# fabian-sp/GGLasso

Hardware: AMD Instinct MI355X
Metric: ADMM iters/sec on (K=32,p=500) GGL at 1/2/4/8 GPUs; eigh HBM GB/s vs peak (higher is better)
Workload: dtype f64

## Files before the change

gglasso_amd/_lib.py:

```python
import ctypes
import os

import numpy as np

_HERE = os.path.dirname(os.path.abspath(__file__))
LIB_PATH = os.path.join(_HERE, "lib", "libggl_hip.so")
DEV_LIB_PATH = os.path.join(_HERE, "lib", "libggl_hip_dev.so")

REG_SGL, REG_GGL, REG_FGL, REG_FSGL = 0, 1, 2, 3
EIG_AUTO, EIG_JACOBI, EIG_ROCSOLVER, EIG_NEWTON_SCHULZ = 0, 1, 2, 3
CTX_STREAM_GIVEN = 1 << 16
OPTIONS = {"speculate": 1, "spec_factor": 2, "ns_mode": 3, "ns_degrees": 4, "theta_flat": 5, "rank_eig": 6, "parts": 7,
           "parts_max_tiles": 8, "symm_variant": 9, "spin_wait": 10, "fused_bounds": 11, "pipeline": 12, "fused_start": 13, "parts_small": 14, "ns_tol": 15, "cw_warm": 16, "chain": 17, "rank_l0_coarse": 18, "isolate": 19, "rank_deflate": 20, "rank_l0_deflate": 21, "fused_cw": 22, "omega_lds": 23, "early_part": 24, "part_priority": 25, "fused_w": 26, "rank_cw": 27, "bound_side": 28, "lds_pinned": 29, "join_flag": 30, "cw_rider": 31, "copy_rider": 32, "reduce_rider": 33, "parts_bias": 34, "parts_order": 35, "download_threads": 36, "group_sched": 37, "omega_poly": 38}


def eig_flags(method=EIG_AUTO, ns_mode=0, ns_degrees=0):
    return int(method) | ((int(ns_mode) & 0x3) << 8) | ((int(ns_degrees) & 0xf) << 12)

JACOBI_MAX_P = 128
NS_MIN_P = 8
BUF_S, BUF_OMEGA, BUF_THETA, BUF_L, BUF_X, BUF_GROUPSQ, BUF_NORMS, BUF_OMEGA_PREV = range(8)
E_ARG, E_HIP, E_SOLVER, E_ALLOC, E_COMM = -1, -2, -3, -4, -5
PHASES = ("form_W", "eig_omega", "recon_omega", "theta", "eig_L", "recon_L", "dual", "reduce", "eig_omega2", "bound",
          "allreduce_groupsq", "allreduce_norms")

_dp = ctypes.POINTER(ctypes.c_double)
_vp = ctypes.c_void_p
_i = ctypes.c_int
_d = ctypes.c_double
_ubp = ctypes.POINTER(ctypes.c_ubyte)
_ip = ctypes.POINTER(ctypes.c_int)

_SIGNATURES = {
    "ggl_version": ([], _i),
    "ggl_last_error": ([], ctypes.c_char_p),
    "ggl_device_count": ([], _i),
    "ggl_theta_limits": ([ctypes.POINTER(_i)], _i),
    "ggl_ctx_create": ([_i, _i, _i, _i, _vp, ctypes.POINTER(_vp)], _i),
    "ggl_ctx_destroy": ([_vp], _i),
    "ggl_ctx_sync": ([_vp], _i),
    "ggl_device_ptr": ([_vp, _i], _vp),
    "ggl_ctx_set_option": ([_vp, _i, _d], _i),
    "ggl_ctx_get_option": ([_vp, _i, _dp], _i),
    "ggl_set_S": ([_vp, _dp], _i),
    "ggl_set_state": ([_vp, _dp, _dp, _dp, _dp], _i),
    "ggl_set_state_ex": ([_vp, _dp, _dp, _dp, _dp, ctypes.POINTER(_i)], _i),
    "ggl_set_S_ex": ([_vp, _dp, _i], _i),
    "ggl_get_state": ([_vp, _dp, _dp, _dp, _dp], _i),
    "ggl_state_snapshot": ([_vp, _i], _i),
    "ggl_set_lambda1_mask": ([_vp, _dp], _i),
    "ggl_set_lambda1_mask_k": ([_vp, _dp], _i),
    "ggl_set_instance_dims": ([_vp, ctypes.POINTER(_i)], _i),
    "ggl_set_block_size": ([_vp, _i], _i),
    "ggl_fsgl_stats": ([_vp, ctypes.POINTER(ctypes.c_longlong)], _i),
    "ggl_prox_sum_frob": ([_i, _i, _dp, _d, _dp], _i),
    "ggl_frob_norm_per_block": ([_i, _i, _dp, _i, _dp], _i),
    "ggl_admm_step": ([_vp, _d, _d, _d, _i, _i, _dp, _dp, _dp], _i),
    "ggl_hint_last_step": ([_vp], _i),
    "ggl_step_omega": ([_vp, _d, _i, _dp], _i),
    "ggl_step_omega_spec": ([_vp, _d, _i, _dp], _i),
    "ggl_step_group_partial": ([_vp, _d, _d], _i),
    "ggl_step_finish": ([_vp, _d, _d, _d, _i, _i, _dp, _i, _dp], _i),
    "ggl_norms_read": ([_vp, _dp], _i),
    "ggl_comm_unique_id": ([ctypes.c_char_p], _i),
    "ggl_comm_init": ([_vp, _i, _i, ctypes.c_char_p], _i),
    "ggl_comm_destroy": ([_vp], _i),
# ... 6 lines not shown
    "ggl_sgl_batch_step": ([_vp, _dp, _dp, _i, _dp, _dp], _i),
    "ggl_mgl_batch_step": ([_vp, _i, _dp, _dp, _dp, _i, _i, _dp, _dp, _dp], _i),
    "ggl_scale_X_batch": ([_vp, _dp], _i),
    "ggl_batch_decide": ([_i, _dp, _ubp, _ubp, _dp, _dp, _d, _d, _i, _dp, _dp, _ip], _i),
    "ggl_sgl_batch_run": ([_vp, _i, _dp, _dp, _i, _dp, _dp, _d, _d, _i, _dp, _ip, _ip, _i, _vp, _ip, _i], _i),
    "ggl_mgl_batch_run": ([_vp, _i, _i, _dp, _dp, _dp, _i, _i, _dp, _dp, _dp, _d, _d, _i, _dp, _ip, _ip, _i, _vp, _ip, _i], _i),
    "ggl_snapshot_state_from": ([_vp, _i, _vp, _i], _i),
    "ggl_get_snapshots": ([_vp, _dp, _dp, _dp, _dp], _i),
    "ggl_get_state_k": ([_vp, _i, _dp, _dp, _dp, _dp], _i),
    "ggl_exit_checks": ([_vp, _i, _dp], _i),
    "ggl_exit_checks_k": ([_vp, _i, _dp], _i),
    "ggl_exit_checks_fast_k": ([_vp, _i, _d, _d, _dp], _i),
    "ggl_ext_setup": ([_vp, ctypes.POINTER(_i), ctypes.POINTER(_i), _i], _i),
    "ggl_ext_set_state": ([_vp, _dp, _dp], _i),
    "ggl_ext_get_state": ([_vp, _dp, _dp], _i),
    "ggl_ext_admm_step": ([_vp, _d, _dp, _d, _i, _dp, _dp], _i),
    "ggl_ext_kkt_residual": ([_vp, _d, _dp, _d, _i, _dp, _dp], _i),
    "ggl_ext_setup_batch": ([_vp, _i, ctypes.POINTER(_i), ctypes.POINTER(_i), _i], _i),
    "ggl_ext_batch_step": ([_vp, _d, _dp, _dp, _i, _dp, _dp], _i),
    "ggl_objective": ([_vp, _d, _d, _i, _dp], _i),
    "ggl_kkt_residual": ([_vp, _d, _d, _d, _i, _i, _dp, _dp, _dp], _i),
    "ggl_profile_enable": ([_vp, _i], _i),
    "ggl_profile_read": ([_vp, _dp, ctypes.POINTER(ctypes.c_longlong), _i], _i),
    "ggl_dev_symm": ([_i, _i, _dp, _dp, _dp, _dp, _dp, _dp, _i], _i),
    "ggl_dev_symm_bench": ([_i, _i, _i, _i, _dp], _i),
    "ggl_lds_stats": ([_vp, ctypes.POINTER(ctypes.c_longlong)], _i),
    "ggl_group_stats": ([_vp, ctypes.POINTER(ctypes.c_longlong), _dp], _i),
    "ggl_spectral_bounds": ([_vp, _dp, _dp], _i),
    "ggl_pipeline_stats": ([_vp, ctypes.POINTER(ctypes.c_longlong)], _i),
    "ggl_trace_start": ([_vp, _i], _i),
    "ggl_trace_read": ([_vp, _dp, _i], _i),
    "ggl_dev_omega_lds": ([_i, _i, _dp, _dp, _dp, _dp, _dp, _d, _i, _dp, _dp, _i, _dp], _i),
    "ggl_dev_symm_bounds": ([_i, _i, _dp, _dp, _i, _dp, _dp, _dp, _dp], _i),
    "ggl_snapshot_k": ([_vp, _i], _i),
    "ggl_snapshot_from": ([_vp, _i, _vp, _i], _i),
    "ggl_selection_stats": ([_vp, _dp], _i),
    "ggl_threshold_scan": ([_vp, _dp, _i, _dp, ctypes.POINTER(_i)], _i),
    "ggl_selection_rank": ([_vp, _d, _dp], _i),
    "ggl_finalize_L": ([_vp, _i, ctypes.POINTER(_i)], _i),
    "ggl_failed_instances": ([_vp, ctypes.POINTER(_i)], _i),
    "ggl_failed_reason": ([_vp, _i, _dp], _i),
    "ggl_debug_poison": ([_i], _i),
    "ggl_set_odd_dl": ([_i], _i),
    "ggl_reset_instance": ([_vp, _i], _i),
    "ggl_ctx_create_subset": ([_vp, ctypes.POINTER(_i), _i, ctypes.POINTER(_vp)], _i),
    "ggl_get_snapshot_k": ([_vp, _i, _dp, _dp], _i),
    "ggl_get_snapshot_state_k": ([_vp, _i, _dp, _dp], _i),
    "ggl_dev_ns_schedule": ([_d, _i, _i, ctypes.POINTER(_i), _dp, ctypes.POINTER(_i)], _i),
    "ggl_dev_ns_schedule_tol": ([_d, _i, _d, _i, ctypes.POINTER(_i), _dp, ctypes.POINTER(_i)], _i),
    "ggl_dev_group_partition": ([ctypes.POINTER(_i), _i, _i, _i, ctypes.POINTER(_i)], _i),
    "ggl_dev_ns_units": ([_d, _i, _d], _i),
    "ggl_dev_omega_poly_plan": ([_d, _d, _i, ctypes.POINTER(_i), _dp, ctypes.POINTER(_i)], _i),
    "ggl_omega_poly_stats": ([_vp, ctypes.POINTER(ctypes.c_longlong)], _i),
    "ggl_ns_stats": ([_vp, ctypes.POINTER(ctypes.c_longlong)], _i),
    "ggl_rank_stats": ([_vp, ctypes.POINTER(ctypes.c_longlong)], _i),
    "ggl_deflate_stats": ([_vp, ctypes.POINTER(ctypes.c_longlong)], _i),
    "ggl_finalize_stats": ([_vp, ctypes.POINTER(ctypes.c_longlong)], _i),
    "ggl_eig_info": ([_vp, ctypes.POINTER(_i)], _i),
    "ggl_last_dispatch": ([_vp, ctypes.POINTER(ctypes.c_longlong)], _i),
    "ggl_eigh_batched": ([_i, _i, _dp, _dp, _dp, _i], _i),
    "ggl_phiplus": ([_i, _i, _dp, _dp, _dp, _dp], _i),
    "ggl_prox_rank_norm": ([_i, _i, _dp, _dp, _dp, _dp], _i),
    "ggl_phiplus_matrix": ([_i, _i, _dp, _dp, _dp, _i], _i),
    "ggl_rank_matrix": ([_i, _i, _dp, _dp, _dp, _i], _i),
    "ggl_rank_matrix_ex": ([_i, _i, _dp, _dp, _dp, _i, _d, ctypes.POINTER(ctypes.c_longlong)], _i),
    "ggl_rank_matrix_deflate": ([_i, _i, _dp, _dp, _dp, _i, _d, ctypes.POINTER(ctypes.c_longlong)], _i),
    "ggl_prox_od_1norm": ([_i, _dp, _d, _dp, _dp], _i),
    "ggl_prox_p": ([_i, _i, _dp, _d, _d, _i, _dp], _i),
    "ggl_prox_tv": ([_i, _i, _dp, _d, _dp], _i),
    "ggl_prox_2norm": ([_i, _i, _dp, _d, _dp], _i),
    "ggl_prox_phi": ([_i, _i, _dp, _d, _d, _i, _dp], _i),
}

_DEV_SIGNATURES = {
    "ggl_dev_i8_stages": ([_i], _i),
    "ggl_dev_symm_i8": ([_i, _i, _i, _i, _dp, _dp, _d, _d, _dp, _i, _dp], _i),
    "ggl_dev_omega_i8": ([_i, _i, _dp, _dp, _dp, ctypes.POINTER(_i), _d, _dp, _i, _dp], _i),
    "ggl_dev_mfma_f64_peak": ([_dp], _i),
    "ggl_dev_symm_timeline": ([_i, _i, ctypes.POINTER(ctypes.c_longlong), _i, ctypes.POINTER(_i)], _i),
    "ggl_dev_chain_probe": ([_i, _i, _i, _i, _i, _i, _dp], _i),
    "ggl_dev_coissue_probe": ([_dp], _i),
    "ggl_dev_mfma_lds_probe": ([_dp], _i),
    "ggl_dev_chain_run": ([_i, _i, _i, _i, _dp], _i),
    "ggl_dev_switch_bench": ([_i, _i, _i, _i, _i, _dp], _i),
    "ggl_dev_vendor_bench": ([_i, _i, _i, _i, _dp], _i),
    "ggl_dev_fill_copy_probe": ([_i, _i, _i, _i, _i, ctypes.POINTER(ctypes.c_longlong)], _i),
}

ABI_VERSION = 300
EXPORTS = tuple(_SIGNATURES)
_lib = None


def load():
    global _lib
    if _lib is not None:
        return _lib
    if not os.path.exists(LIB_PATH):
        raise RuntimeError(
            f"{LIB_PATH} is missing: build it with `python -m gglasso_amd.build` "
            "(gglasso_amd has no CPU fallback)")
    import sys
    if "torch" not in sys.modules and os.environ.get("GGL_TORCH_FIRST", "1") != "0":
        try:
            import torch
        except Exception:
# ... 59 lines not shown
```

gglasso_amd/csrc/capi_batch.hip:

```cpp
#include "capi_internal.hpp"

static int sgl_fused_finish(ggl_ctx* c, const double* rho, const double* lambda1, double* out_norms);

extern "C" int ggl_sgl_batch_step(ggl_ctx* c, const double* rho, const double* lambda1, int latent, const double* mu1,
                                  double* out_norms)
{
    ARGCHK(c && rho && lambda1 && out_norms, "ctx, rho, lambda1, out_norms");
    ARGCHK(!latent || mu1, "latent needs mu1");
    HIPCHK(hipSetDevice(c->device));
    DROP_PRE(c);
    return sgl_batch_step_impl(c, rho, lambda1, latent, mu1, out_norms);
}

static int sgl_fused_finish(ggl_ctx* c, const double* rho, const double* lambda1, double* out_norms)
{
    const int K = c->K;
    c->sgl_done = false;
    c->sgl_fused_calls += 1;
    c->norms_host = true;
    double* rows = c->norms_h;
    {
        const unsigned long long want = c->seq_wait;
        const volatile unsigned long long* sq = c->seq_h;
        const auto t0 = std::chrono::steady_clock::now();
// ... 433 lines not shown
    out[0] = f ? (double)c->fail_why[k] : 0.0;
    out[1] = f ? c->fail_value[k] : 0.0;
    return GGL_OK;
}

extern "C" int ggl_failed_instances(ggl_ctx* c, int* out)
{
    ARGCHK(c, "ctx");
    int n = 0;
    for (int k = 0; k < c->K; ++k) {
        const int f = (c->failed && c->failed[k]) ? 1 : 0;
        if (out) out[k] = f;
        n += f;
    }
    return n;
}

extern "C" int ggl_reset_instance(ggl_ctx* c, int k)
{
    ARGCHK(c && k >= 0 && k < c->K, "ctx, k");
    HIPCHK(hipSetDevice(c->device));
    DROP_PRE(c);
    const size_t pp = (size_t)c->p * c->p, off = (size_t)k * pp;
    double* ident[] = {c->S + off, c->Om[0] + off, c->Om[1] + off, c->Theta + off};
    double* zero[] = {c->L + off, c->X + off, c->W + off};
    for (double* z : zero) HIPCHK(hipMemsetAsync(z, 0, pp * sizeof(double), c->stream));
    for (double* a : ident) launch_set_identity(c->stream, a, 1, c->p);
    for (double* lam : c->Lam)
        if (lam) launch_set_identity(c->stream, lam + off, 1, c->p);
    if (c->X1) HIPCHK(hipMemsetAsync(c->X1 + off, 0, pp * sizeof(double), c->stream));
    HIPCHK(hipGetLastError());
    c->spec_have = false;
    c->cw_have = false;
    c->cwL_have = false;
    return GGL_OK;
}

extern "C" int ggl_ctx_create_subset(ggl_ctx* src, const int* idx, int m, ggl_ctx** out)
{
    ARGCHK(src && idx && out, "ctx, idx, out");
    ARGCHK(m >= 1 && m <= src->K, "1 <= m <= K");
    for (int i = 0; i < m; ++i) ARGCHK(idx[i] >= 0 && idx[i] < src->K, "instance index");
    HIPCHK(hipSetDevice(src->device));
    { int rc_ = drop_prelaunch(src); if (rc_) return rc_; }
    ggl_ctx* c = nullptr;
    int rc = ggl_ctx_create(src->device, m, src->p, src->flags & ~GGL_CTX_STREAM_GIVEN, nullptr, &c);
    if (rc) return rc;
    c->spec_enable = src->spec_enable; c->spec_factor = src->spec_factor; c->ns_force = src->ns_force;
    c->ns_degrees = src->ns_degrees; c->theta_flat = src->theta_flat; c->rank_eig = src->rank_eig;
    c->rank_ns = c->omega_ns && !c->rank_eig; c->ns_parts = src->ns_parts; c->parts_max_tiles = src->parts_max_tiles;
    c->symm_variant = src->symm_variant; c->spin_wait = src->spin_wait; c->fused_bounds = src->fused_bounds;
    c->pipeline = src->pipeline; c->fused_start = src->fused_start; c->parts_small = src->parts_small; c->download_threads = src->download_threads; c->ns_tol = src->ns_tol;
    c->cw_warm = src->cw_warm; c->rank_l0 = src->rank_l0; c->rank_l0_coarse = src->rank_l0_coarse;
    c->group_sched = src->group_sched; c->omega_poly = src->omega_poly;
    c->isolate = src->isolate; c->lds_omega = src->lds_omega; c->lds_waves = src->lds_waves; c->early_part = src->early_part; c->rank_deflate = src->rank_deflate; c->rank_l0_deflate = src->rank_l0_deflate;
    int* didx = nullptr;
    hipError_t e = hipMalloc(&didx, m * sizeof(int));
    if (e == hipSuccess) e = hipMemcpyAsync(didx, idx, m * sizeof(int), hipMemcpyHostToDevice, src->stream);
    if (e != hipSuccess) { ggl_ctx_destroy(c); return fail(GGL_E_HIP, "subset: %s", hipGetErrorString(e)); }
    const size_t pp = (size_t)src->p * src->p;
    const double* from[] = {src->S, src->Om[src->cur], src->Om[src->cur ^ 1], src->Theta, src->L, src->X};
    double* to[] = {c->S, c->Om[0], c->Om[1], c->Theta, c->L, c->X};
    for (int i = 0; i < 6; ++i) launch_copy_instances(src->stream, to[i], from[i], didx, m, pp, false);
    c->cur = 0;
    c->state_symmetric = src->state_symmetric;
    c->S_symmetric = src->S_symmetric;
    c->fused_w = src->fused_w;
#ifdef GGL_DEV
    c->parts_bias = src->parts_bias; c->parts_order = src->parts_order; c->chain_mode = src->chain_mode; c->fused_cw = src->fused_cw;
    c->rank_cw = src->rank_cw; c->bound_side = src->bound_side;
#endif
    c->lds_pinned = src->lds_pinned;
    c->join_flag = src->join_flag;
    c->cw_rider = src->cw_rider;
    c->copy_rider = src->copy_rider;
    c->red_rider = src->red_rider;
    c->step_latent = src->step_latent;
    c->nk_valid = false;
    if (src->l_ns && src->Ckeep && src->Ckeep_beta) {
        e = hipMalloc(&c->Ckeep_alloc, c->n * sizeof(double) + STACK_SLACK);
        if (e != hipSuccess) { (void)hipFree(didx); ggl_ctx_destroy(c); return fail(GGL_E_HIP, "subset: %s", hipGetErrorString(e)); }
        c->Ckeep = c->Ckeep_alloc;
        c->Ckeep_beta = (double*)malloc(m * sizeof(double));
        for (int i = 0; i < m; ++i) c->Ckeep_beta[i] = src->Ckeep_beta[idx[i]];
        launch_copy_instances(src->stream, c->Ckeep, src->Ckeep, didx, m, pp, false);
        c->l_ns = true;
    }
    if (src->has_mask) {
        e = hipMemcpyAsync(c->mask, src->mask, pp * sizeof(double), hipMemcpyDeviceToDevice, src->stream);
        c->has_mask = true;
    }
    if (e == hipSuccess && src->has_maskK && src->maskK) {
        e = hipMalloc(&c->maskK, c->n * sizeof(double));
        if (e == hipSuccess) launch_copy_instances(src->stream, c->maskK, src->maskK, didx, m, pp, false);
        c->has_maskK = true;
    }
    if (e == hipSuccess && src->has_dims && src->inst_pk) {
        std::vector<int> all(src->K), sub(m);
        e = hipMemcpyAsync(all.data(), src->inst_pk, src->K * sizeof(int), hipMemcpyDeviceToHost, src->stream);
        if (e == hipSuccess) e = hipStreamSynchronize(src->stream);
        for (int i = 0; i < m; ++i) sub[i] = all[idx[i]];
        if (e == hipSuccess) e = hipMalloc(&c->inst_pk, m * sizeof(int));
        if (e == hipSuccess) e = hipMemcpy(c->inst_pk, sub.data(), m * sizeof(int), hipMemcpyHostToDevice);
        c->has_dims = true;
    }
    if (e == hipSuccess) e = hipGetLastError();
    if (e == hipSuccess) e = hipStreamSynchronize(src->stream);
// ... 11 lines not shown
```

gglasso_amd/csrc/capi_ctx.hip:

```cpp
#include "capi_internal.hpp"

static thread_local char g_err[512] = "";

int fail(int code, const char* fmt, ...)
{
    va_list ap;
    va_start(ap, fmt);
    vsnprintf(g_err, sizeof(g_err), fmt, ap);
    va_end(ap);
    return code;
}

void prof_collect(ggl_ctx* c)
{
    if (!c->prof_on) return;
    for (int ph = 0; ph < GGL_NPHASE; ++ph) {
        if (!c->ev_used[ph]) continue;
        float ms = 0.f;
        if (hipEventElapsedTime(&ms, c->ev[ph][0], c->ev[ph][1]) == hipSuccess) {
            c->ph_ms[ph] += ms;
            c->ph_cnt[ph] += 1;
        }
        c->ev_used[ph] = false;
    }
// ... 278 lines not shown
    HIPCHK(hipMemsetAsync(c->X, 0, nb, c->stream));
    HIPCHK(hipMemsetAsync(c->Om[1], 0, nb, c->stream));
    if (c->omega_ns) {
        HIPCHK(hipMemsetAsync(c->cwmax, 0, c->K * sizeof(unsigned long long), c->stream));
        HIPCHK(hipMemsetAsync(c->cwcnt, 0, c->K * sizeof(unsigned), c->stream));
        *c->seq_h = 0;
        HIPCHK(hipMemsetAsync(c->spec_flag, 0, ggl_ctx::MAX_PARTS * sizeof(int), c->stream));
        memset(c->spec_flag_h, 0, ggl_ctx::MAX_PARTS * sizeof(int));
    }
    HIPCHK(hipStreamSynchronize(c->stream));
    return GGL_OK;
}



static int set_option(ggl_ctx* c, int opt, double v)
{
    int rcd = drop_prelaunch(c);
    if (rcd) return rcd;
    switch (opt) {
        case GGL_OPT_SPECULATE: c->spec_enable = v != 0.0; break;
        case GGL_OPT_SPEC_FACTOR:
            if (!(v > 0.0)) return fail(GGL_E_ARG, "bad argument: GGL_OPT_SPEC_FACTOR must be positive");
            c->spec_factor = v;
            break;
        case GGL_OPT_NS_MODE:
            if (v != 0.0 && v != 1.0 && v != 2.0) return fail(GGL_E_ARG, "bad argument: GGL_OPT_NS_MODE is 0, 1 or 2");
            c->ns_force = (int)v;
            break;
        case GGL_OPT_NS_DEGREES: c->ns_degrees = v >= 9 ? 9 : (v >= 5 ? 5 : 3); break;
        case GGL_OPT_THETA_FLAT: c->theta_flat = (v == 2.0) ? 2 : (v != 0.0 ? 1 : 0); break;
        case GGL_OPT_RANK_EIG: c->rank_eig = v != 0.0; c->rank_ns = c->omega_ns && !c->rank_eig; break;
        case GGL_OPT_PARTS: c->ns_parts = std::min(std::max((int)v, 1), (int)ggl_ctx::MAX_PARTS); break;
        case GGL_OPT_PARTS_MAX_TILES: c->parts_max_tiles = (long)v; break;
        case GGL_OPT_SYMM_VARIANT:
            if (v >= 0 && !symm_variant_built((int)v))
                return fail(GGL_E_ARG, "bad argument: product-kernel variant not in this build");
            c->symm_variant = (int)v;
            break;
        case GGL_OPT_SPIN_WAIT: c->spin_wait = v != 0.0; break;
        case GGL_OPT_FUSED_BOUNDS: c->fused_bounds = v != 0.0; break;
        case GGL_OPT_PIPELINE: c->pipeline = v != 0.0; break;
        case GGL_OPT_FUSED_START: c->fused_start = v != 0.0; break;
        case GGL_OPT_PARTS_SMALL: c->parts_small = (int)v; break;
        case GGL_OPT_GROUP_SCHED:
            if (v != 0.0 && v != 1.0 && v != 2.0 && v != 3.0 && v != 12.0 && v != 13.0)
                return fail(GGL_E_ARG, "bad argument: GGL_OPT_GROUP_SCHED is 0, 1, 2, 3, 12 or 13");
            c->group_sched = (int)v;
            break;
        case GGL_OPT_OMEGA_POLY:
            if (v != 0.0 && v != 1.0) return fail(GGL_E_ARG, "bad argument: GGL_OPT_OMEGA_POLY is 0 or 1");
            c->omega_poly = (int)v;
            break;
#ifdef GGL_DEV
        case GGL_OPT_PARTS_BIAS: c->parts_bias = (int)v; break;
        case GGL_OPT_PARTS_ORDER: c->parts_order = (int)v; break;
        case GGL_OPT_CHAIN: c->chain_mode = (v == 2.0) ? 2 : (v != 0.0 ? 1 : 0); break;
        case GGL_OPT_FUSED_CW: c->fused_cw = v != 0.0; break;
        case GGL_OPT_RANK_CW: c->rank_cw = v != 0.0; break;
        case GGL_OPT_BOUND_SIDE: c->bound_side = (int)v; break;
#else
        case GGL_OPT_PARTS_BIAS: case GGL_OPT_PARTS_ORDER: case GGL_OPT_CHAIN: case GGL_OPT_FUSED_CW: case GGL_OPT_RANK_CW:
        case GGL_OPT_BOUND_SIDE: case GGL_OPT_PART_PRIORITY:
            if (v == 0.0) break;
            return fail(GGL_E_ARG, "bad argument: option %d is a measured-and-rejected alternative that only the development "
                        "library (libggl_hip_dev.so, python -m gglasso_amd.build --dev) carries", opt);
#endif
        case GGL_OPT_DOWNLOAD_THREADS: c->download_threads = std::min(std::max((int)v, 1), 64); break;
        case GGL_OPT_CW_WARM: c->cw_warm = v != 0.0; break;
        case GGL_OPT_ISOLATE: c->isolate = v != 0.0; break;
        case GGL_OPT_OMEGA_LDS: c->lds_omega = v != 0.0; c->lds_waves = (v == 4.0 || v == 8.0) ? (int)v : 0; break;
        case GGL_OPT_EARLY_PART: c->early_part = v != 0.0; break;
        case GGL_OPT_FUSED_W: c->fused_w = v != 0.0; break;
        case GGL_OPT_LDS_PINNED: c->lds_pinned = v != 0.0; break;
        case GGL_OPT_JOIN_FLAG: c->join_flag = v != 0.0; break;
        case GGL_OPT_CW_RIDER: c->cw_rider = (int)v; break;
        case GGL_OPT_COPY_RIDER: c->copy_rider = (int)v; break;
        case GGL_OPT_REDUCE_RIDER: c->red_rider = (int)v; break;
#ifdef GGL_DEV
        case GGL_OPT_PART_PRIORITY: {
            if (v != 0.0 && v != 1.0 && v != 2.0) return fail(GGL_E_ARG, "bad argument: GGL_OPT_PART_PRIORITY is 0, 1 or 2");
            if (!c->omega_ns || (int)v == c->part_priority) break;
            int lo = 0, hi = 0;
            HIPCHK(hipSetDevice(c->device));
            HIPCHK(hipDeviceGetStreamPriorityRange(&lo, &hi));
            HIPCHK(hipStreamSynchronize(c->stream));
            for (int i = 0; i < ggl_ctx::MAX_PARTS - 1; ++i) {
                HIPCHK(hipStreamSynchronize(c->streamx[i]));
                HIPCHK(hipStreamDestroy(c->streamx[i]));
                c->streamx[i] = nullptr;
                if (v == 0.0) HIPCHK(hipStreamCreateWithFlags(&c->streamx[i], hipStreamNonBlocking));
                else HIPCHK(hipStreamCreateWithPriority(&c->streamx[i], hipStreamNonBlocking, v == 1.0 ? hi : lo));
            }
            c->part_priority = (int)v;
            c->parts_probed = false;
            break;
        }
#endif
        case GGL_OPT_RANK_DEFLATE: c->rank_deflate = v != 0.0; break;
        case GGL_OPT_RANK_L0_DEFLATE:
            if (!(v > 0.0) || v > 0.1) return fail(GGL_E_ARG, "bad argument: GGL_OPT_RANK_L0_DEFLATE is in (0, 0.1]");
            c->rank_l0_deflate = v;
            break;
        case GGL_OPT_RANK_L0_COARSE:
            if (!(v >= 0.0) || v > 0.1) return fail(GGL_E_ARG, "bad argument: GGL_OPT_RANK_L0_COARSE is in [0, 0.1]");
            c->rank_l0_coarse = v;
            break;
        case GGL_OPT_NS_TOL:
            if (!(v >= 0.0) || v > 1e-6) return fail(GGL_E_ARG, "bad argument: GGL_OPT_NS_TOL is in [0, 1e-6]");
            c->ns_tol = std::max(v, NS_TOL_EXACT);
            break;
        default: return fail(GGL_E_ARG, "bad argument: unknown ctx option %d", opt);
    }
    c->spec_have = false;
    c->cw_have = false;
    c->cwL_have = false;
    return GGL_OK;
}

extern "C" int ggl_ctx_set_option(ggl_ctx* c, int opt, double value)
{
    ARGCHK(c, "ctx");
    return set_option(c, opt, value);
}

extern "C" int ggl_ctx_get_option(ggl_ctx* c, int opt, double* value)
{
    ARGCHK(c && value, "ctx, value");
    switch (opt) {
        case GGL_OPT_SPECULATE: *value = c->spec_enable; break;
        case GGL_OPT_SPEC_FACTOR: *value = c->spec_factor; break;
        case GGL_OPT_NS_MODE: *value = c->ns_force; break;
        case GGL_OPT_NS_DEGREES: *value = c->ns_degrees; break;
        case GGL_OPT_THETA_FLAT: *value = c->theta_flat; break;
        case GGL_OPT_RANK_EIG: *value = c->rank_eig; break;
        case GGL_OPT_PARTS: *value = c->ns_parts; break;
        case GGL_OPT_PARTS_MAX_TILES: *value = (double)c->parts_max_tiles; break;
        case GGL_OPT_SYMM_VARIANT: *value = c->symm_variant; break;
        case GGL_OPT_SPIN_WAIT: *value = c->spin_wait; break;
        case GGL_OPT_FUSED_BOUNDS: *value = c->fused_bounds; break;
        case GGL_OPT_PIPELINE: *value = c->pipeline; break;
        case GGL_OPT_FUSED_START: *value = c->fused_start; break;
        case GGL_OPT_PARTS_SMALL: *value = c->parts_small; break;
        case GGL_OPT_GROUP_SCHED: *value = c->group_sched; break;
        case GGL_OPT_OMEGA_POLY: *value = c->omega_poly; break;
        case GGL_OPT_PARTS_BIAS: *value = c->parts_bias; break;
        case GGL_OPT_PARTS_ORDER: *value = c->parts_order; break;
        case GGL_OPT_DOWNLOAD_THREADS: *value = c->download_threads; break;
        case GGL_OPT_NS_TOL: *value = c->ns_tol; break;
        case GGL_OPT_CW_WARM: *value = c->cw_warm; break;
        case GGL_OPT_CHAIN: *value = c->chain_mode; break;
        case GGL_OPT_RANK_L0_COARSE: *value = c->rank_l0_coarse; break;
        case GGL_OPT_ISOLATE: *value = c->isolate; break;
        case GGL_OPT_FUSED_CW: *value = c->fused_cw; break;
        case GGL_OPT_OMEGA_LDS: *value = c->lds_omega ? (c->lds_waves ? c->lds_waves : 1) : 0; break;
        case GGL_OPT_EARLY_PART: *value = c->early_part; break;
        case GGL_OPT_FUSED_W: *value = c->fused_w; break;
        case GGL_OPT_RANK_CW: *value = c->rank_cw; break;
        case GGL_OPT_BOUND_SIDE: *value = c->bound_side; break;
        case GGL_OPT_LDS_PINNED: *value = c->lds_pinned; break;
        case GGL_OPT_JOIN_FLAG: *value = c->join_flag; break;
        case GGL_OPT_CW_RIDER: *value = c->cw_rider; break;
        case GGL_OPT_COPY_RIDER: *value = c->copy_rider; break;
        case GGL_OPT_REDUCE_RIDER: *value = c->red_rider; break;
        case GGL_OPT_PART_PRIORITY: *value = c->part_priority; break;
        case GGL_OPT_RANK_DEFLATE: *value = c->rank_deflate; break;
        case GGL_OPT_RANK_L0_DEFLATE: *value = c->rank_l0_deflate; break;
        default: return fail(GGL_E_ARG, "bad argument: unknown ctx option %d", opt);
    }
    return GGL_OK;
}

#ifdef GGL_DEV
static void dev_env_options(ggl_ctx* c)
{
    static const struct { const char* name; int opt; } tab[] = {
        {"GGL_SPECULATE", GGL_OPT_SPECULATE}, {"GGL_SPEC_FACTOR", GGL_OPT_SPEC_FACTOR}, {"GGL_NS_MODE", GGL_OPT_NS_MODE},
        {"GGL_NS_DEGREES", GGL_OPT_NS_DEGREES}, {"GGL_THETA_FLAT", GGL_OPT_THETA_FLAT}, {"GGL_RANK_EIG", GGL_OPT_RANK_EIG},
        {"GGL_TWO_STREAM", GGL_OPT_PARTS}, {"GGL_PARTS_MAX_TILES", GGL_OPT_PARTS_MAX_TILES},
        {"GGL_SYMM_VARIANT", GGL_OPT_SYMM_VARIANT}, {"GGL_SPIN_WAIT", GGL_OPT_SPIN_WAIT},
        {"GGL_FUSED_BOUNDS", GGL_OPT_FUSED_BOUNDS}, {"GGL_PIPELINE", GGL_OPT_PIPELINE},
        {"GGL_FUSED_START", GGL_OPT_FUSED_START}, {"GGL_PARTS_SMALL", GGL_OPT_PARTS_SMALL}, {"GGL_CHAIN", GGL_OPT_CHAIN}};
    for (const auto& t : tab)
        if (const char* v = getenv(t.name)) (void)set_option(c, t.opt, atof(v));
    if (const char* v = getenv("GGL_ROCSOLVER_SYEVJ")) c->use_syevj = atoi(v) != 0;
}
#endif

extern "C" int ggl_ctx_create(int device, int K, int p, int flags, void* stream, ggl_ctx** out)
{
    ARGCHK(out != nullptr, "out");
    ARGCHK(K >= 1 && p >= 1, "K, p must be positive");
    const int eig = flags & 0xff;
    ARGCHK(eig == GGL_EIG_AUTO || eig == GGL_EIG_JACOBI || eig == GGL_EIG_ROCSOLVER || eig == GGL_EIG_NEWTON_SCHULZ,
           "eigensolver selector");
    ARGCHK(eig != GGL_EIG_JACOBI || jacobi_fits(p), "GGL_EIG_JACOBI needs p <= GGL_JACOBI_MAX_P");
    const int nsm = (flags >> 8) & 0x3, nsd = (flags >> 12) & 0xf;
    ARGCHK(nsm <= 2, "GGL_EIG_NS_MODE is 0, 1 or 2");
// ... 339 lines not shown
```

gglasso_amd/csrc/capi_internal.hpp:

```cpp
#pragma once
#include <hip/hip_runtime.h>
#include <rocblas/rocblas.h>
#include <rocsolver/rocsolver.h>

#include <algorithm>
#include <cmath>
#include <cstdarg>
#include <cstdio>
#include <cstring>
#include <numeric>
#include <atomic>
#include <thread>
#include <mutex>
#include <chrono>
#include <vector>

#include "../../include/ggl_hip.h"
#include "kernels.hpp"
#include "ggl_comm.hpp"

using namespace ggl;


#define HIPCHK(expr)                                                                                   \
// ... 60 lines not shown
    bool par0_stale = false;
    int* sgl_fail_h = nullptr;
    long long sgl_fused_calls = 0, sgl_fallback_instances = 0;
    bool nk_valid = false;
    bool omega_ns = false;
    bool dvo_valid = false;
    int symm_variant = -1;
    double *nsYP[2] = {nullptr, nullptr}, *nsT = nullptr;
#ifdef GGL_DEV
#define GGL_DEV_OPT(type, name) type name = 0
#else
#define GGL_DEV_OPT(type, name) static constexpr type name = 0
#endif
    GGL_DEV_OPT(int, chain_mode);
    double* nsNX = nullptr;
    unsigned* chain_cnt = nullptr;
    long long chain_calls = 0;
    bool flags_dirty = false;
    int step_latent = 0;
    int ns_force = 0;
    bool use_syevj = false;
    static constexpr int MAX_PARTS = 4;
    hipStream_t streamx[MAX_PARTS - 1] = {};
    hipEvent_t ev_fork = nullptr, ev_join[MAX_PARTS - 1] = {};
    GGL_DEV_OPT(int, bound_side);
    bool join_flag = true;
    int red_rider = 2;
    long long red_rides = 0;
    RedRider red_pending;
    int copy_rider = 1;
    long long copy_rides = 0;
    std::vector<double> pre0_beta;
    int cw_rider = 1;
    long long cw_rides = 0;
    bool parts_serial = false;
    unsigned long long* join_words = nullptr;
    unsigned long long join_seq = 0;
    hipEvent_t ev_bfork[MAX_PARTS] = {}, ev_bjoin[MAX_PARTS] = {};
    bool pipeline = true, pre_valid = false, pre_spec_pending = false;
    bool last_step_hint = false;
    double* pre_beta = nullptr;
    long long pre_launched = 0, pre_dropped = 0;
    int download_threads = 8;
    GGL_DEV_OPT(int, parts_order);
    GGL_DEV_OPT(int, parts_bias);
    int group_sched = 1;
    long long group_steps = 0;
    long long group_changes = 0;
    int last_groups = 1, last_group_len[MAX_PARTS] = {}, last_group_units[MAX_PARTS] = {};
    double group_units_sum[MAX_PARTS] = {};
    int omega_poly = 1;
    long long poly_seqs = 0, poly_seqs_total = 0;
    int poly_last_deg = 0;
    int parts_small = 8;
    bool fused_start = true;
    bool fused_bounds = true;
    bool lds_omega = true;
    int lds_waves = 0;
    double* lds_tab = nullptr;
    int lds_ntab = 0, lds_tab_deg = -1;
    double lds_lnq = 0.0, lds_tab_tol = -1.0;
    long long lds_calls = 0, lds_misses = 0;
    int lds_cool = 0, lds_cool_next = 4;
    bool lds_last = false;
    GGL_DEV_OPT(bool, fused_cw);
    int theta_flat = 2;
    bool state_symmetric = true;
    bool S_symmetric = false;
    bool fused_w = true, wf_ready = false;
    double* wf_beta = nullptr;
    long long wf_written = 0, wf_used = 0;
    bool spec_enable = true, spec_have = false, spec_pending = false;
    double *spec_c = nullptr, *spec_beta = nullptr;
    double *cuse = nullptr, *cuse_h = nullptr;
    double *coef_hh[2] = {nullptr, nullptr}, *cuse_hh[2] = {nullptr, nullptr};
    int plan_par = 0;
    struct EarlyA {
        bool valid = false;
        NsPlan plans[4];
        double* fused[4] = {nullptr, nullptr, nullptr, nullptr};
        double* beta = nullptr;
        int nh = 0, Kh[4] = {}, k0h[4] = {};
        bool grouped = false;
        int var_parts = -1;
    } early;
    bool early_part = true;
    GGL_DEV_OPT(int, part_priority);
    bool parts_probed = false;
    int parts_replaced = 0;
    bool early_caller = false;
    bool early_request = false;
    bool ratio_calm = false;
    long long early_launched = 0, early_used = 0;
    int *spec_flag = nullptr, *spec_flag_h = nullptr;
    long long spec_calls = 0, spec_misses = 0;
    double spec_factor = 1.02;
    unsigned long long* seq_h = nullptr;
    unsigned long long seq_next = 0, seq_wait = 0;
    unsigned long long stamp_want = 0;
    bool spin_wait = true;
    long long spin_timeouts = 0;
    bool sharded_check = false;
    bool info_dirty = true;
    bool norms_host = false;
    int spec_cool = 0;
    int ns_degrees = 9;
// ... 151 lines not shown
```

gglasso_amd/csrc/capi_omega.hip:

```cpp
#include "capi_internal.hpp"

int eig_recon(ggl_ctx* c, double* A, double* out, double* Dv, int map, const double* betaK, int ph_eig,
                     int ph_recon)
{
    c->info_dirty = true;
    if (use_jacobi(c)) {
        if (ph_eig >= 0) PB(c, ph_eig);
        HIPCHK(launch_jacobi(c->stream, A, Dv, nullptr, out, map, betaK, c->info, c->K, c->p));
        if (ph_eig >= 0) PE(c, ph_eig);
        return GGL_OK;
    }
    if (ph_eig >= 0) PB(c, ph_eig);
    {
        int rcb = blas_handle(c, &c->blas);
        if (rcb) return rcb;
    }
    if (c->use_syevj) {
        rocblas_status sj = rocsolver_dsyevj_strided_batched(c->blas, rocblas_esort_none, rocblas_evect_original,
                                                             rocblas_fill_upper, c->p, A, c->p,
                                                             (rocblas_stride)c->p * c->p, 0.0, c->E, 100,
                                                             (rocblas_int*)c->sweeps, Dv, c->p, c->info, c->K);
        if (sj != rocblas_status_success) return fail(GGL_E_SOLVER, "rocsolver_dsyevj_strided_batched: status %d", (int)sj);
        if (ph_eig >= 0) PE(c, ph_eig);
        if (ph_recon >= 0) PB(c, ph_recon);
// ... 161 lines not shown
        HIPCHK(hipMalloc(&c->lds_tab, (nt + 2) * sizeof(double)));
        HIPCHK(hipMemsetAsync(c->lds_tab + nt, 0, 2 * sizeof(double), c->stream));
    }
    std::vector<double> tab(nt, 0.0);
    c->lds_ntab = omega_lds_build_table(c->ns_tol, c->ns_degrees, tab.data(), OMEGA_LDS_MAXTAB, &c->lds_lnq);
    if (c->lds_ntab < 1) return fail(GGL_E_SOLVER, "LDS Omega-step: empty schedule table");
    HIPCHK(hipStreamSynchronize(c->stream));
    HIPCHK(hipMemcpy(c->lds_tab, tab.data(), nt * sizeof(double), hipMemcpyHostToDevice));
    c->lds_tab_tol = c->ns_tol;
    c->lds_tab_deg = c->ns_degrees;
    return GGL_OK;
}

void lds_missed(ggl_ctx* c)
{
    c->lds_misses += 1;
    c->lds_cool = c->lds_cool_next;
    c->lds_cool_next = std::min(2 * c->lds_cool_next, 64);
    c->lds_last = false;
}

int trace_lane(const ggl_ctx* c, hipStream_t st)
{
    if (st == c->stream) return 0;
    for (int i = 0; i < ggl_ctx::MAX_PARTS - 1; ++i)
        if (st == c->streamx[i]) return i + 1;
    return -1;
}
void trace_mark(ggl_ctx* c, hipStream_t st, int tag)
{
    ggl_ctx::Trace& t = c->trace;
    if (!t.on || t.n >= t.cap) return;
    if (hipEventRecord(t.ev[t.n], st) != hipSuccess) return;
    t.tag[t.n] = tag;
    t.lane[t.n] = trace_lane(c, st);
    t.n += 1;
}
void trace_host(ggl_ctx* c, int tag)
{
    ggl_ctx::Trace& t = c->trace;
    if (!t.on || t.nhost >= t.cap) return;
    t.host_us[t.nhost] = std::chrono::duration<double, std::micro>(std::chrono::steady_clock::now() - t.t0).count();
    t.host_tag[t.nhost] = tag;
    t.nhost += 1;
}
void trace_symm_hook(hipStream_t st, int kind, void* arg) { trace_mark((ggl_ctx*)arg, st, 10 + kind); }

static void note_family(ggl_ctx* c, const NsPlan& pl)
{
    c->poly_seqs_total += 1;
    if (pl.direct) { c->poly_seqs += 1; c->poly_last_deg = pl.direct; }
}

static int omega_groups(const ggl_ctx* c, const double* cb, const double* beta_h, int K, int* Kh, int* k0h, int* gunits)
{
    if (!c->group_sched || K < 2 || c->ns_force == 2 || c->chain_mode || c->comm) return 1;
    {
        const double I = 2.5e-14 * (double)c->p * c->p * c->p, F = 6.5e-6;
        if (c->group_sched < 10 && (double)K * 1e-7 > 0.01 * 7.0 * (F + K * I)) return 1;
    }
    std::vector<int> u(K);
    for (int k = 0; k < K; ++k) {
        double ck = cb[k] * (1.0 + 1e-10);
        if (!(ck > 0.0) || !std::isfinite(ck) || !(beta_h[k] > 0.0)) return 1;
        if (ck < 4.0 * beta_h[k]) ck = 4.0 * beta_h[k];
        u[k] = ns_units_query(std::sqrt(4.0 * beta_h[k] / ck), c->ns_degrees, c->ns_tol);
        if (u[k] < 0) return 1;
    }
    int len[ggl_ctx::MAX_PARTS];
    const bool force = c->group_sched >= 10;
    const int gmax = force ? c->group_sched - 10 : (c->group_sched >= 2 ? c->group_sched : 3);
    const int G = ns_group_partition(u.data(), K, force ? 20000 : c->p, std::min(gmax, (int)ggl_ctx::MAX_PARTS - 1), len);
    if (G <= 1) return 1;
    for (int g = 0, k0 = 0; g < G; ++g) {
        Kh[g] = len[g];
        k0h[g] = k0;
        gunits[g] = 0;
        for (int k = k0; k < k0 + len[g]; ++k) gunits[g] = std::max(gunits[g], u[k]);
        k0 += len[g];
    }
    return G;
}

static void note_groups(ggl_ctx* c, int G, const int* Kh, const NsPlan* plans)
{
    const int G_prev = c->last_groups;
    c->last_groups = G;
    if (G <= 1) return;
    bool same = (G_prev == G);
    for (int g = 0; same && g < G; ++g) same = (c->last_group_len[g] == Kh[g]);
    if (c->group_steps > 0 && !same) c->group_changes += 1;
    c->group_steps += 1;
    for (int g = 0; g < ggl_ctx::MAX_PARTS; ++g) {
        c->last_group_len[g] = g < G ? Kh[g] : 0;
        c->last_group_units[g] = g < G ? plans[g].units : 0;
        if (g < G) c->group_units_sum[g] += plans[g].units;
    }
}

int omega_step(ggl_ctx* c, int latent, CopySegs* pending, bool allow_spec, bool only_spec)
{
    int rc;
    const double* beta = c->par;
    const int nxt = c->cur ^ 1;
    c->step_latent = latent;
    if (latent && !c->pre0_beta.empty()) std::fill(c->pre0_beta.begin(), c->pre0_beta.end(), std::nan(""));
// ... 14 lines not shown
        if (!resume) {
            c->plan_par ^= 1;
            c->coef_h = c->coef_hh[c->plan_par];
            c->cuse_h = c->cuse_hh[c->plan_par];
        }
        double* pre = c->coef_h + (size_t)(NS_MAX_LAUNCHES - 2) * NS_SLOT(K);
        for (int k = 0; !resume && k < K; ++k) {
            double* o0 = pre + (size_t)k * NS_NCOEF;
            double* o1 = pre + NS_SLOT(K) + (size_t)k * NS_NCOEF;
            o0[0] = 4.0 * c->par_h[k]; o0[1] = 1.0; o0[2] = o0[3] = o0[4] = o0[5] = o0[6] = o0[7] = 0.0;
            o1[0] = 0.0; o1[1] = 1.0; o1[2] = o1[3] = o1[4] = o1[5] = o1[6] = o1[7] = 0.0;
        }
        double* pre_d = c->coef + (size_t)(NS_MAX_LAUNCHES - 2) * NS_SLOT(K);
        const long t64 = (c->p + 63) / 64;
        const long ntile = t64 * (t64 + 1) / 2 * K;
        int nh = (K >= 16 && ntile >= 600 && ntile <= c->parts_max_tiles) ? std::min(c->ns_parts, K / 8) : 1;
        if (nh == 1 && c->parts_small && K >= c->parts_small && K < 16 && c->p >= 384 && c->ns_parts >= 2) nh = 2;
        nh = std::max(nh, 1);
        bool spec = allow_spec && c->spec_enable && c->spec_have && !latent && c->spec_cool == 0;
        if (allow_spec && !only_spec && c->spec_cool > 0) c->spec_cool -= 1;
        for (int k = 0; spec && k < K; ++k) spec = (c->par_h[k] == c->spec_beta[k]);
        if (resume) spec = true;
        int Kh[ggl_ctx::MAX_PARTS], k0h[ggl_ctx::MAX_PARTS];
        bool grouped = false;
        int gunits[ggl_ctx::MAX_PARTS] = {};
        if (resume) {
            nh = c->early.nh;
            grouped = c->early.grouped;
            for (int h = 0; h < nh; ++h) { Kh[h] = c->early.Kh[h]; k0h[h] = c->early.k0h[h]; }
        } else {
            for (int h = 0, k0 = 0; h < nh; ++h) {
                Kh[h] = K / nh + (h < K % nh ? 1 : 0);
                if (nh == 2 && c->parts_bias && std::abs(c->parts_bias) < K / 2) Kh[h] += h == 0 ? c->parts_bias : -c->parts_bias;
                k0h[h] = k0;
                k0 += Kh[h];
            }
            if (spec && nh == 1) {
                std::vector<double> cb(K);
                for (int k = 0; k < K; ++k) cb[k] = c->spec_c[k] * c->spec_factor;
                const int G = omega_groups(c, cb.data(), c->par_h, K, Kh, k0h, gunits);
                if (G > 1) { nh = G; grouped = true; }
            }
        }
        const size_t pp = (size_t)c->p * c->p;
        const int nbb = norm_bounds_blocks(c->p);
        const int var_grouped = c->symm_variant >= 0 ? c->symm_variant : (symm_auto_variant(K, c->p) == 16 ? 17 : symm_auto_variant(K, c->p));
        const int var_parts = resume ? c->early.var_parts
                            : grouped ? var_grouped
                                      : ((c->symm_variant < 0 && nh > 1 && K >= 16) ? 17 : c->symm_variant);
        c->last_parts = nh;
        c->last_variant = symm_effective_variant(var_parts >= 0 ? var_parts : symm_auto_variant(Kh[0], c->p), c->p);
        const size_t region = (size_t)(NS_MAX_LAUNCHES - 4) / nh * NS_SLOT(K);
        NsPlan plans[ggl_ctx::MAX_PARTS];
        double* start_base_h = c->coef_h + (size_t)(NS_MAX_LAUNCHES - 3) * NS_SLOT(K);
        double* start_base_d = c->coef + (size_t)(NS_MAX_LAUNCHES - 3) * NS_SLOT(K);
        double* fused[ggl_ctx::MAX_PARTS] = {};
        bool cw_written = false;
        if (c->flags_dirty) {
            HIPCHK(hipMemsetAsync(c->spec_flag, 0, ggl_ctx::MAX_PARTS * sizeof(int), c->stream));
            for (int h = 0; h < ggl_ctx::MAX_PARTS; ++h) c->spec_flag_h[h] = 0;
            c->flags_dirty = false;
        }
        c->lds_last = false;
        const LdsSgl* sgl_req = c->sgl_req;
        c->sgl_req = nullptr;
        c->sgl_done = false;
        if (c->lds_omega && c->p <= omega_lds_max_p() && c->ns_force == 0 && c->symm_variant < 0 && !c->chain_mode && !want_A && !resume) {
            const bool as_spec = allow_spec && c->spec_enable && !latent;
            if (c->lds_cool > 0) {
                if (!only_spec) c->lds_cool -= 1;
            } else if (as_spec || !only_spec) {
                rc = lds_table(c);
                if (rc) return rc;
                LdsSgl sgl;
                const bool fused = sgl_req && as_spec && c->seq_h && c->spin_wait && !c->prof_on;
                const bool no_copy = c->lds_pinned && !c->info_dirty && ((fused && pending != nullptr) || (!sgl_req && (pending == nullptr || c->pending_beta_only || c->pending_pinned_ok)));
                CopySegs sg = first;
                sg.add(c->spec_flag, nullptr, sizeof(int));
                sg.add(c->spec_flag + ggl_ctx::MAX_PARTS - 1, nullptr, sizeof(int));
                c->spec_flag_h[0] = c->spec_flag_h[ggl_ctx::MAX_PARTS - 1] = 0;
                if (c->info_dirty) sg.add(c->info, nullptr, K * sizeof(int));
                if (!no_copy) launch_copy_small(c->stream, sg);
                PB(c, GGL_PH_EIG_OMEGA);
                unsigned long long* cnt = (unsigned long long*)(c->lds_tab + (size_t)OMEGA_LDS_MAXTAB * OMEGA_LDS_ENT);
                if (fused) {
                    sgl = *sgl_req;
                    sgl.Theta = c->Theta; sgl.X = c->X; sgl.OmegaPrev = c->Om[c->cur];
                    sgl.norms = c->norms_h; sgl.fail = c->sgl_fail_h;
                    sgl.seq = c->seq_h; sgl.seq_val = c->seq_wait = ++c->seq_next; sgl.arrive = c->arrive;
                    memset(c->sgl_fail_h, 0, K * sizeof(int));
                    if (no_copy) {
                        sgl.l1K = c->par_h + K;
                        sgl.invrhoK = c->par_h + 4 * (size_t)K;
                    }
                }
                if (no_copy && first.n > 0) { beta = c->par_h; c->par0_stale = true; }
                if (!launch_omega_lds(c->stream, c->Theta, latent ? c->L : nullptr, c->X, c->S, beta, c->Om[nxt], c->lds_tab,
                                      c->lds_ntab, c->lds_lnq, K, c->p, c->spec_flag, c->spec_flag_h, 0, cnt, c->bounds_h, nullptr,
                                      c->lds_waves, fused ? &sgl : nullptr))
                    return fail(GGL_E_HIP, "k_omega_lds: p = %d outside the kernel's range, or the LDS attribute was refused", c->p);
                PE(c, GGL_PH_EIG_OMEGA);
                c->sgl_done = fused;
                HIPCHK(hipGetLastError());
                c->last_parts = 1;
                c->last_variant = 41;
                c->lds_calls += 1;
// ... 53 lines not shown
                c->spec_flag_h[0] = c->spec_flag_h[1] = c->spec_flag_h[ggl_ctx::MAX_PARTS - 1] = 0;
                const int nb_launch = pl.products - 2;
                if (nb_launch > 0) sg.add(c->coef, c->coef_h, (size_t)nb_launch * NS_SLOT(K) * sizeof(double));
                sg.add(c->cuse, c->cuse_h, (size_t)K * sizeof(double));
                if (c->info_dirty) sg.add(c->info, nullptr, K * sizeof(int));
                sg.add(c->chain_cnt, nullptr, (size_t)K * CHAIN_CNT_STRIDE * sizeof(unsigned));
                launch_copy_small(c->stream, sg);
                PB(c, GGL_PH_FORM_W);
                launch_form_W_sym(c->stream, c->W, c->Theta, nullptr, c->X, c->S, beta, K, c->p);
                PE(c, GGL_PH_FORM_W);
                PB(c, GGL_PH_EIG_OMEGA);
                ChainProg P;
                P.nops = nops; P.K = K; P.p = c->p; P.ntiles = bT * (bT + 1) / 2;
                P.begin[0] = 0;
                for (int i = 0; i < nops; ++i) { P.op[i] = ops[i]; P.begin[i + 1] = P.begin[i] + P.ntiles * (ops[i].pair ? 2 : 1); }
                if (launch_omega_chain(c->stream, P, c->chain_cnt, c->spec_flag + 1, c->spec_flag_h + 1) < 0)
                    return fail(GGL_E_HIP, "k_omega_chain: launch failed (%s)", hipGetErrorString(hipGetLastError()));
                launch_bound_rows(c->stream, c->rowpart, bT, K, c->p, c->nbrow, c->infpart);
                launch_cw_final(c->stream, c->nsYP[0] + c->n, c->nbrow, K, c->p, c->infpart, c->fropart, bT * (bT + 1) / 2,
                                c->cwmax, c->cwcnt, c->bounds_h, c->cuse, c->spec_flag, c->spec_flag_h, 0,
                                (c->cw_warm && c->cw_have) ? c->cwvec[c->cw_cur] : nullptr,
                                c->cw_warm ? c->cwvec[c->cw_cur ^ 1] : nullptr);
                PE(c, GGL_PH_EIG_OMEGA);
                HIPCHK(hipGetLastError());
                c->last_parts = 1;
                c->last_variant = 40;
                c->chain_calls += 1;
                c->ns_launches_total += pl.products;
                note_family(c, pl);
                c->ns_units_frac += pl.units;
                c->ns_steps_frac += pl.steps;
                c->ns_units_total = (long long)(c->ns_units_frac + 0.5);
                c->ns_steps_total = (long long)(c->ns_steps_frac + 0.5);
                c->ns_calls += 1;
                c->spec_calls += 1;
                c->spec_pending = true;
                c->cw_pending = c->cw_warm;
                if (c->info_dirty) { memset(c->info_h, 0, K * sizeof(int)); c->info_dirty = false; }
                c->dvo_valid = false;
                c->cur = nxt;
                return GGL_OK;
            }
        }
#endif
        if (resume) {
            for (int h = 0; h < nh; ++h) { plans[h] = c->early.plans[h]; fused[h] = c->early.fused[h]; }
            c->early_used += 1;
        } else if (spec) {
            for (int k = 0; k < K; ++k) c->cuse_h[k] = c->spec_c[k] * c->spec_factor;
            sanitize_bounds(c, c->cuse_h, c->par_h, 4.0);
            for (int h = 0; spec && h < nh; ++h) {
                const int k0 = k0h[h];
                const int prc = ns_plan(c->cuse_h + k0, c->par_h + k0, Kh[h], c->coef_h + h * region,
                                        start_base_h + 5 * k0, &plans[h], c->ns_force, c->ns_degrees, c->ns_tol, c->omega_poly);
                spec = (prc == 0) && !plans[h].stable;
                for (int k = k0; spec && c->fused_start && k < k0 + Kh[h]; ++k) {
                    fused[h] = ns_fused_start(plans[h], start_base_h + 5 * (size_t)k, c->nsYP[1] + k0 * pp, c->nsT + k0 * pp,
                                              nh > 1 ? c->n : (size_t)K * pp, pre + NS_SLOT(K) + (size_t)k * NS_NCOEF);
                }
            }
        }
        if (only_spec && !spec) return GGL_NOT_LAUNCHED;
        if (nh > 1 && !c->parts_probed) {
            rc = probe_part_streams(c);
            if (rc) return rc;
        }
        if (nh > 1 && !resume) {
            HIPCHK(hipEventRecord(c->ev_fork, c->stream));
            for (int h = 1; h < nh; ++h) HIPCHK(hipStreamWaitEvent(c->streamx[h - 1], c->ev_fork, 0));
        }
        for (int hh = 0; hh < nh; ++hh) {
            const int h = (c->parts_order && nh == 2 && c->prof_on == 0) ? nh - 1 - hh : hh;
            hipStream_t sh = h == 0 ? c->stream : c->streamx[h - 1];
            const int k0 = k0h[h];
            if (!want_A) {
                c->spec_flag_h[h] = 0;
                if (h == 0 && nh < ggl_ctx::MAX_PARTS) c->spec_flag_h[ggl_ctx::MAX_PARTS - 1] = 0;
            }
            double* Ap = c->nsYP[0] + k0 * pp;
            double* Bp = c->nsYP[0] + c->n + k0 * pp;
            const int btile = c->fused_bounds ? symm_bounds_tile(Kh[h], c->p, var_parts) : 0;
            const int bT = btile ? (c->p + btile - 1) / btile : 0;
            double* rowp = btile ? c->rowpart + (size_t)k0 * bT * c->p : nullptr;
            double* frop = btile ? c->fropart + (size_t)k0 * (bT * (bT + 1) / 2) : nullptr;
            if (!resume) {
            bool ride_copy = (c->copy_rider == 2 || (c->copy_rider == 1 && nh == 1)) && first.n == 0 && !latent && btile != 0 &&
                             !c->chain_mode && c->prof_on != 1;
            for (int k = k0; ride_copy && k < k0 + Kh[h]; ++k) ride_copy = (c->pre0_beta[k] == c->par_h[k]);
            CopySegs sg = first;
            if (!ride_copy) {
                sg.add(pre_d + NS_NCOEF * (size_t)k0, pre + NS_NCOEF * (size_t)k0, (size_t)Kh[h] * NS_NCOEF * sizeof(double));
                for (int k = k0; k < k0 + Kh[h]; ++k) c->pre0_beta[k] = c->par_h[k];
            }
            sg.add(pre_d + NS_SLOT(K) + NS_NCOEF * (size_t)k0, pre + NS_SLOT(K) + NS_NCOEF * (size_t)k0,
                   (size_t)Kh[h] * NS_NCOEF * sizeof(double));
            sg.add(c->spec_flag + h, nullptr, sizeof(int));
            if (h == 0 && nh < ggl_ctx::MAX_PARTS) sg.add(c->spec_flag + ggl_ctx::MAX_PARTS - 1, nullptr, sizeof(int));
            if (spec) {
                sg.add(start_base_d + 5 * (size_t)k0, start_base_h + 5 * (size_t)k0, (size_t)Kh[h] * 5 * sizeof(double));
                const int nb_launch = plans[h].products - 2;
                if (nb_launch > 0)
                    sg.add(c->coef + h * region, c->coef_h + h * region, (size_t)nb_launch * NS_SLOT(Kh[h]) * sizeof(double));
                sg.add(c->cuse + k0, c->cuse_h + k0, (size_t)Kh[h] * sizeof(double));
                if (h == 0 && c->info_dirty) sg.add(c->info, nullptr, K * sizeof(int));
            }
            if (h == 0 && c->red_pending.nblk > 0) {
                if (w_ready && (c->red_rider == 2 || nh == 1)) {
// ... 45 lines not shown
                }
                sb = c->streamx[side_slot];
                HIPCHK(hipEventRecord(c->ev_bfork[h], sh));
                HIPCHK(hipStreamWaitEvent(sb, c->ev_bfork[h], 0));
                bfree = c->ev_bjoin[h];
            }
            const bool ride = c->cw_rider && spec && btile && !c->fused_cw && sb == sh && c->cw_warm && c->cw_have;
            if (ride) {
                CwRider r;
                r.B = Bp; r.rowpart = rowp; r.fropart = frop;
                r.dprev = c->cwvec[c->cw_cur] + (size_t)k0 * c->p;
                r.dnext = c->cwvec[c->cw_cur ^ 1] + (size_t)k0 * c->p;
                r.d_out = c->nbrow + (size_t)k0 * c->p;
                r.cwmax = c->cwmax + k0; r.cnt = c->cwcnt + k0; r.out = c->bounds_h + k0; r.cuse = c->cuse + k0;
                r.flag = c->spec_flag; r.flag_host = c->spec_flag_h; r.flag_slot = h;
                r.T = bT; r.ntile = bT * (bT + 1) / 2; r.p = c->p; r.K = Kh[h]; r.nbx = (c->p + 15) / 16;
                symm_set_rider(r);
                if (c->cw_rider == 2) symm_flush_rider(sh);
                c->cw_rides += 1;
                cw_written = true;
            } else if (btile) {
                if (c->fused_cw) {
                    launch_bound_cw(sh, Bp, rowp, bT, Kh[h], c->p, c->nbrow + (size_t)k0 * c->p, frop, bT * (bT + 1) / 2,
                                    c->cwmax + k0, c->cwcnt + k0, c->bounds_h + k0, spec ? c->cuse + k0 : nullptr,
                                    spec ? c->spec_flag : nullptr, spec ? c->spec_flag_h : nullptr, h,
                                    (c->cw_warm && c->cw_have) ? c->cwvec[c->cw_cur] + (size_t)k0 * c->p : nullptr,
                                    c->cw_warm ? c->cwvec[c->cw_cur ^ 1] + (size_t)k0 * c->p : nullptr);
                } else {
                const int nib = bound_rows_blocks(c->p);
                launch_bound_rows(sb, rowp, bT, Kh[h], c->p, c->nbrow + (size_t)k0 * c->p, c->infpart + (size_t)k0 * nib);
                trace_mark(c, sb, 3);
                launch_cw_final(sb, Bp, c->nbrow + (size_t)k0 * c->p, Kh[h], c->p, c->infpart + (size_t)k0 * nib, frop,
                                bT * (bT + 1) / 2, c->cwmax + k0, c->cwcnt + k0, c->bounds_h + k0, spec ? c->cuse + k0 : nullptr,
                                spec ? c->spec_flag : nullptr, spec ? c->spec_flag_h : nullptr, h,
                                (c->cw_warm && c->cw_have) ? c->cwvec[c->cw_cur] + (size_t)k0 * c->p : nullptr,
                                c->cw_warm ? c->cwvec[c->cw_cur ^ 1] + (size_t)k0 * c->p : nullptr);
                trace_mark(c, sb, 4);
                }
                cw_written = c->cw_warm;
            } else {
                double* nb2 = c->nbpart + 2 * (size_t)k0 * nbb;
                double* nbc = c->nbpart + 2 * (size_t)K * nbb + (size_t)k0 * nbb;
                launch_norm_bounds(sh, Bp, Kh[h], c->p, nb2, c->nbrow + (size_t)k0 * c->p);
                launch_cw_bounds(sh, Bp, c->nbrow + (size_t)k0 * c->p, Kh[h], c->p, nbc);
                launch_bound_final(sh, nb2, nbc, nbb, Kh[h], c->bounds_h + k0, 0, spec ? c->cuse + k0 : nullptr,
                                   spec ? c->spec_flag + h : nullptr, spec ? c->spec_flag_h + h : nullptr);
            }
            if (bfree) HIPCHK(hipEventRecord(bfree, sb));
            if (spec) {
                ns_run(sh, plans[h], c->coef + h * region, start_base_d + 5 * k0, c->W + k0 * pp, c->nsYP[0] + k0 * pp,
                       c->nsYP[1] + k0 * pp, c->nsT + k0 * pp, c->Om[nxt] + k0 * pp, Kh[h], c->p,
                       var_parts, nh > 1 ? c->n : 0, fused[h] != nullptr, bfree);
                symm_flush_rider(sh);
                c->ns_launches_total += plans[h].products;
                note_family(c, plans[h]);
                const double frac = (double)Kh[h] / K;
                c->ns_units_frac += frac * plans[h].units;
                c->ns_steps_frac += frac * plans[h].steps;
            }
            if (h == 0 && !spec) PE(c, GGL_PH_EIG_OMEGA);
        }
        HIPCHK(hipGetLastError());
        if (want_A) {
            for (int h = 0; h < nh; ++h) { c->early.plans[h] = plans[h]; c->early.fused[h] = fused[h]; c->early.Kh[h] = Kh[h]; c->early.k0h[h] = k0h[h]; }
            c->early.nh = nh;
            c->early.grouped = grouped;
            c->early.var_parts = var_parts;
            memcpy(c->early.beta, c->par_h, K * sizeof(double));
            c->early.valid = true;
            c->early_launched += 1;
            return GGL_OK;
        }
        if (spec) {
            if (nh > 1 && c->join_flag && !c->parts_serial) {
                c->join_seq += 1;
                for (int h = 1; h < nh; ++h) launch_set_flag(c->streamx[h - 1], c->join_words + h, c->join_seq);
                launch_wait_flags(c->stream, c->join_words + 1, nh - 1, c->join_seq, c->spec_flag, c->spec_flag_h, 0, 200.0);
                HIPCHK(hipGetLastError());
            } else {
                for (int h = 1; h < nh; ++h) {
                    HIPCHK(hipEventRecord(c->ev_join[h - 1], c->streamx[h - 1]));
                    HIPCHK(hipStreamWaitEvent(c->stream, c->ev_join[h - 1], 0));
                }
            }
            PE(c, GGL_PH_EIG_OMEGA);
            c->ns_units_total = (long long)(c->ns_units_frac + 0.5);
            c->ns_steps_total = (long long)(c->ns_steps_frac + 0.5);
            c->ns_calls += 1;
            c->spec_calls += 1;
            note_groups(c, grouped ? nh : 1, Kh, plans);
            c->spec_pending = true;
            c->cw_pending = cw_written;
            if (c->info_dirty) { memset(c->info_h, 0, K * sizeof(int)); c->info_dirty = false; }
            c->dvo_valid = false;
            c->cur = nxt;
            return GGL_OK;
        }
        for (int h = 0; h < nh; ++h) HIPCHK(hipStreamSynchronize(h == 0 ? c->stream : c->streamx[h - 1]));
        sanitize_bounds(c, c->bounds_h, c->par_h, 4.0);
        for (int k = 0; k < K; ++k) { c->spec_c[k] = c->bounds_h[k]; c->spec_beta[k] = c->par_h[k]; }
        c->spec_have = true;
        if (cw_written) { c->cw_cur ^= 1; c->cw_have = true; }
        bool any_stable = false;
        size_t region_b = region;
        int var_b = var_parts;
        if (nh == 1) {
            const int G = omega_groups(c, c->bounds_h, c->par_h, K, Kh, k0h, gunits);
            if (G > 1) {
                nh = G;
                grouped = true;
                region_b = (size_t)(NS_MAX_LAUNCHES - 4) / nh * NS_SLOT(K);
                var_b = var_grouped;
                if (!c->parts_probed) {
                    rc = probe_part_streams(c);
                    if (rc) return rc;
                }
            }
        }
        for (int h = 0; h < nh; ++h) {
            const int k0 = k0h[h];
            const int prc = ns_plan(c->bounds_h + k0, c->par_h + k0, Kh[h], c->coef_h + h * region_b, start_base_h + 5 * k0,
                                    &plans[h], c->ns_force, c->ns_degrees, c->ns_tol, c->omega_poly);
            if (prc == -1) return fail(GGL_E_SOLVER, "Newton-Schulz Omega-step: non-finite W (diverged iterate?)");
            if (prc == -2) {
                c->ns_eigh_fallbacks += 1;
                rc = eig_recon(c, c->W, c->Om[nxt], c->DvO, MAP_PHIPLUS, beta, -1, GGL_PH_RECON_OMEGA);
                if (rc) return rc;
                c->dvo_valid = true;
                c->cur = nxt;
                return GGL_OK;
            }
            any_stable = any_stable || plans[h].stable;
        }
        if (nh > 1 && any_stable) {
            const int prc = ns_plan(c->bounds_h, c->par_h, K, c->coef_h, start_base_h, &plans[0], c->ns_force, c->ns_degrees, c->ns_tol,
                                    c->omega_poly);
            if (prc != 0) return fail(GGL_E_SOLVER, "Newton-Schulz Omega-step: plan failed (%d)", prc);
        }
        const int nrun = (nh > 1 && !any_stable) ? nh : 1;
        if (nrun == 1) { Kh[0] = K; k0h[0] = 0; }
        c->last_parts = nrun;
        c->last_variant = symm_effective_variant((nrun > 1 && var_b >= 0) ? var_b
                          : (c->symm_variant >= 0 ? c->symm_variant : symm_auto_variant(Kh[0], c->p)), c->p);
        note_groups(c, (grouped && nrun > 1) ? nrun : 1, Kh, plans);
        PB(c, GGL_PH_EIG_OMEGA2);
        for (int h = 0; h < nrun; ++h) {
            const int Kr = Kh[h], k0 = k0h[h];
            hipStream_t sh = h == 0 ? c->stream : c->streamx[h - 1];
            CopySegs up;
            up.add(start_base_d + 5 * (size_t)k0, start_base_h + 5 * (size_t)k0, (size_t)Kr * 5 * sizeof(double));
            const int nb_launch = plans[h].products - 2;
            if (nb_launch > 0)
                up.add(c->coef + h * region_b, c->coef_h + h * region_b, (size_t)nb_launch * NS_SLOT(Kr) * sizeof(double));
            if (h == 0 && c->info_dirty) up.add(c->info, nullptr, K * sizeof(int));
            launch_copy_small(sh, up);
            ns_run(sh, plans[h], c->coef + h * region_b, start_base_d + 5 * k0,
                   c->W + k0 * pp, c->nsYP[0] + k0 * pp, c->nsYP[1] + k0 * pp, c->nsT + k0 * pp, c->Om[nxt] + k0 * pp, Kr,
                   c->p,
                   nrun > 1 ? var_b : c->symm_variant, nrun > 1 ? c->n : 0);
            c->ns_stable_calls += plans[h].stable ? 1 : 0;
            c->ns_launches_total += plans[h].products;
            note_family(c, plans[h]);
            const double frac = (double)Kr / K;
            c->ns_units_frac += frac * plans[h].units;
            c->ns_steps_frac += frac * plans[h].steps;
        }
        for (int h = 1; h < nrun; ++h) {
            HIPCHK(hipEventRecord(c->ev_join[h - 1], c->streamx[h - 1]));
            HIPCHK(hipStreamWaitEvent(c->stream, c->ev_join[h - 1], 0));
        }
        PE(c, GGL_PH_EIG_OMEGA2);
        HIPCHK(hipGetLastError());
        c->ns_units_total = (long long)(c->ns_units_frac + 0.5);
        c->ns_steps_total = (long long)(c->ns_steps_frac + 0.5);
        c->ns_calls += 1;
        c->dvo_valid = false;
        if (c->info_dirty) { memset(c->info_h, 0, K * sizeof(int)); c->info_dirty = false; }
        c->cur = nxt;
        return GGL_OK;
    }
    if (only_spec) return GGL_NOT_LAUNCHED;
    launch_copy_small(c->stream, first);
    PB(c, GGL_PH_FORM_W);
    launch_form_W(c->stream, c->W, c->Theta, latent ? c->L : nullptr, c->X, c->S, beta, c->K, c->p);
    PE(c, GGL_PH_FORM_W);
    HIPCHK(hipGetLastError());
    rc = eig_recon(c, c->W, c->Om[nxt], c->DvO, MAP_PHIPLUS, beta, GGL_PH_EIG_OMEGA, GGL_PH_RECON_OMEGA);
    if (rc) return rc;
    c->dvo_valid = true;
    c->cur = nxt;
    return GGL_OK;
}

extern "C" int ggl_step_group_partial(ggl_ctx* c, double rho, double lambda1)
{
    ARGCHK(c, "ctx");
    ARGCHK(rho > 0, "rho must be positive");
    HIPCHK(hipSetDevice(c->device));
    launch_group_sums_packed(c->stream, c->groupsq, c->sqwork, c->Om[c->cur], c->step_latent ? c->L : nullptr, c->X,
                             (1.0 / rho) * lambda1, c->K, c->p, c->spec_pending ? c->spec_flag : nullptr);
    HIPCHK(hipGetLastError());
    return GGL_OK;
}

int validate_spec(ggl_ctx* c)
{
    if (c->spec_pending || c->sharded_check) {
        const bool mine = c->spec_pending, sharded = c->sharded_check;
        c->spec_pending = false;
        c->sharded_check = false;
        bool bad = false;
        for (int h = 0; h < ggl_ctx::MAX_PARTS; ++h) bad = bad || (c->spec_flag_h[h] != 0);
        if (sharded) bad = bad || (*c->gflag_h > 0.5);
        if (bad) {
            if (mine && c->lds_last) lds_missed(c);
            else if (mine) c->spec_misses += 1;
            c->flags_dirty = true;
            c->cw_pending = false;
// ... 342 lines not shown
```

gglasso_amd/csrc/capi_ops.hip:

```cpp
#include "capi_internal.hpp"

static int eig_common(int K, int p, const double* A, const double* beta, double* D, double* Q, double* out, int map,
                      int eig_method)
{
    ARGCHK(K >= 1 && p >= 1 && A, "K, p, A");
    ARGCHK(eig_method != GGL_EIG_JACOBI || jacobi_fits(p), "GGL_EIG_JACOBI needs p <= GGL_JACOBI_MAX_P");
    const bool jac = (eig_method == GGL_EIG_JACOBI) || (eig_method == GGL_EIG_AUTO && jacobi_fits(p));
    const size_t n = (size_t)K * p * p, kp = (size_t)K * p;
    DevBuf dA, dD, dR, dO, dB, dE, dS;
    int* dinfo = nullptr;
    HIPCHK(dA.alloc(n));
    HIPCHK(dD.alloc(kp));
    HIPCHK(dB.alloc(K));
    HIPCHK(hipMalloc(&dinfo, K * sizeof(int)));
    struct InfoFree { int* p; ~InfoFree() { (void)hipFree(p); } } infofree{dinfo};
    UP(dA.p, A, n);
    if (beta) UP(dB.p, beta, K);
    if (out) HIPCHK(dO.alloc(n));
    std::vector<int> info(K);
    if (jac) {
        if (Q) HIPCHK(dR.alloc(n));
        HIPCHK(launch_jacobi(nullptr, dA.p, dD.p, dR.p, dO.p, map, beta ? dB.p : nullptr, dinfo, K, p));
        HIPCHK(hipDeviceSynchronize());
        HIPCHK(hipMemcpy(info.data(), dinfo, K * sizeof(int), hipMemcpyDeviceToHost));
// ... 14 lines not shown
        rocblas_destroy_handle(h);
        if (st != rocblas_status_success) return fail(GGL_E_SOLVER, "rocsolver_dsyevd_strided_batched: status %d", (int)st);
        HIPCHK(hipGetLastError());
        HIPCHK(hipMemcpy(info.data(), dinfo, K * sizeof(int), hipMemcpyDeviceToHost));
        for (int k = 0; k < K; ++k)
            if (info[k] != 0) return fail(GGL_E_SOLVER, "rocSOLVER syevd did not converge (instance %d)", k);
    }
    if (out) DOWN(out, dO.p, n);
    if (D || Q) {
        std::vector<double> hd(kp), hr;
        DOWN(hd.data(), dD.p, kp);
        if (Q) { hr.resize(n); DOWN(hr.data(), jac ? dR.p : dA.p, n); }
        std::vector<int> idx(p);
        for (int k = 0; k < K; ++k) {
            std::iota(idx.begin(), idx.end(), 0);
            const double* dk = hd.data() + (size_t)k * p;
            std::stable_sort(idx.begin(), idx.end(), [dk](int a, int b) { return dk[a] < dk[b]; });
            for (int m = 0; m < p; ++m) {
                if (D) D[(size_t)k * p + m] = dk[idx[m]];
                if (Q) {
                    const double* row = hr.data() + (size_t)k * p * p + (size_t)idx[m] * p;
                    for (int i = 0; i < p; ++i) Q[(size_t)k * p * p + (size_t)i * p + m] = row[i];
                }
            }
        }
    }
    return GGL_OK;
}

extern "C" int ggl_dev_symm(int K, int p, const double* A, const double* B, const double* E, const double* coef5K,
                            double* C, double* C2, int variant)
{
    ARGCHK(K >= 1 && p >= 1 && A && B && coef5K && C, "arguments");
    ARGCHK(variant < 0 || symm_variant_built(variant), "product-kernel variant not in this build");
    const size_t n = (size_t)K * p * p;
    DevBuf dA, dB, dE, dC, dC2, dcoef;
    HIPCHK(dA.alloc(n));
    HIPCHK(dB.alloc(n));
    HIPCHK(dC.alloc(n));
    std::vector<double> cw((size_t)K * NS_NCOEF, 0.0);
    for (int k = 0; k < K; ++k) std::copy(coef5K + (size_t)k * 5, coef5K + (size_t)k * 5 + 5, cw.begin() + (size_t)k * NS_NCOEF);
    HIPCHK(dcoef.alloc(cw.size()));
    UP(dA.p, A, n);
    UP(dB.p, B, n);
    UP(dcoef.p, cw.data(), cw.size());
    if (E) { HIPCHK(dE.alloc(n)); UP(dE.p, E, n); }
    if (C2) HIPCHK(dC2.alloc(n));
    launch_symm(nullptr, dA.p, dB.p, dC.p, C2 ? dC2.p : nullptr, E ? dE.p : nullptr, dcoef.p, K, p, variant);
    HIPCHK(hipGetLastError());
    HIPCHK(hipDeviceSynchronize());
    DOWN(C, dC.p, n);
    if (C2) DOWN(C2, dC2.p, n);
    return GGL_OK;
}

extern "C" int ggl_dev_symm_bounds(int K, int p, const double* A, const double* B, int variant, double* C,
                                   double* rowsum_out, double* fro2_out, double* bound_out)
{
    ARGCHK(K >= 1 && p >= 1 && A && B && C && rowsum_out && fro2_out && bound_out, "arguments");
    ARGCHK(variant < 0 || symm_variant_built(variant), "product-kernel variant not in this build");
    const int tile = symm_bounds_tile(K, p, variant);
    ARGCHK(tile != 0, "this variant / p has no bound partials (direct-to-LDS kernels, even p)");
    const int T = (p + tile - 1) / tile, ntile = T * (T + 1) / 2, nib = bound_rows_blocks(p);
    const size_t n = (size_t)K * p * p;
    DevBuf dA, dB, dC, dcoef, drow, dfro, dd, dinf, dout;
    unsigned long long* cw = nullptr;
    unsigned* cnt = nullptr;
    HIPCHK(dA.alloc(n)); HIPCHK(dB.alloc(n)); HIPCHK(dC.alloc(n));
    HIPCHK(drow.alloc((size_t)K * T * p)); HIPCHK(dfro.alloc((size_t)K * ntile)); HIPCHK(dd.alloc((size_t)K * p));
    HIPCHK(dinf.alloc((size_t)K * nib)); HIPCHK(dout.alloc(K));
    HIPCHK(hipMalloc(&cw, K * sizeof(unsigned long long)));
    HIPCHK(hipMalloc(&cnt, K * sizeof(unsigned)));
    struct Free2 { void *a, *b; ~Free2() { (void)hipFree(a); (void)hipFree(b); } } free2{cw, cnt};
    HIPCHK(hipMemset(cw, 0, K * sizeof(unsigned long long)));
    HIPCHK(hipMemset(cnt, 0, K * sizeof(unsigned)));
    HIPCHK(hipMemset(drow.p, 0xff, (size_t)K * T * p * sizeof(double)));
    HIPCHK(hipMemset(dfro.p, 0xff, (size_t)K * ntile * sizeof(double)));
    std::vector<double> coef((size_t)K * NS_NCOEF, 0.0);
    for (int k = 0; k < K; ++k) coef[(size_t)k * NS_NCOEF + 1] = 1.0;
    HIPCHK(dcoef.alloc(coef.size()));
    UP(dA.p, A, n);
    UP(dB.p, B, n);
    UP(dcoef.p, coef.data(), coef.size());
    launch_symm(nullptr, dA.p, dB.p, dC.p, nullptr, nullptr, dcoef.p, K, p, variant, nullptr, drow.p, dfro.p);
    launch_bound_rows(nullptr, drow.p, T, K, p, dd.p, dinf.p);
    launch_cw_final(nullptr, dC.p, dd.p, K, p, dinf.p, dfro.p, ntile, cw, cnt, dout.p, nullptr, nullptr, nullptr, 0);
    HIPCHK(hipGetLastError());
    HIPCHK(hipDeviceSynchronize());
    DOWN(C, dC.p, n);
    DOWN(rowsum_out, dd.p, (size_t)K * p);
    DOWN(bound_out, dout.p, K);
    std::vector<double> fr((size_t)K * ntile);
    DOWN(fr.data(), dfro.p, fr.size());
    for (int k = 0; k < K; ++k) {
        double sq = 0.0;
        for (int t = 0; t < ntile; ++t) sq += fr[(size_t)k * ntile + t];
        fro2_out[k] = sq;
    }
    return GGL_OK;
}

extern "C" int ggl_dev_symm_bench(int K, int p, int variant, int iters, double* ms_out)
{
    ARGCHK(K >= 1 && p >= 1 && iters >= 1 && ms_out, "arguments");
    ARGCHK(variant < 0 || symm_variant_built(variant), "product-kernel variant not in this build");
    const size_t n = (size_t)K * p * p;
// ... 552 lines not shown
}

extern "C" int ggl_dev_symm_timeline(int K, int p, long long* out, int max_blocks, int* nblocks_out)
{
    ARGCHK(K >= 1 && p >= 1 && out && nblocks_out, "arguments");
    const size_t n = (size_t)K * p * p;
    std::vector<double> h(n, 0.25), coef((size_t)K * NS_NCOEF, 0.0);
    for (int k = 0; k < K; ++k) coef[(size_t)k * NS_NCOEF + 1] = 1.0 / p;
    const int T = (p + 63) / 64;
    const int nb = (K >= 8 ? 8 * ((K + 7) / 8) : K) * (T * (T + 1) / 2);
    ARGCHK(nb <= max_blocks, "max_blocks too small");
    DevBuf dA, dB, dC, dcoef, dT;
    HIPCHK(dA.alloc(n));
    HIPCHK(dB.alloc(n));
    HIPCHK(dC.alloc(n));
    HIPCHK(dcoef.alloc(coef.size()));
    HIPCHK(dT.alloc((size_t)nb * 5));
    UP(dA.p, h.data(), n);
    UP(dB.p, h.data(), n);
    UP(dcoef.p, coef.data(), coef.size());
    HIPCHK(hipMemset(dT.p, 0, (size_t)nb * 5 * sizeof(double)));
    for (int i = 0; i < 3; ++i) launch_symm(nullptr, dA.p, dB.p, dC.p, nullptr, nullptr, dcoef.p, K, p, 0);
    launch_symm(nullptr, dA.p, dB.p, dC.p, nullptr, nullptr, dcoef.p, K, p, 10, dT.p);
    HIPCHK(hipGetLastError());
    HIPCHK(hipDeviceSynchronize());
    HIPCHK(hipMemcpy(out, dT.p, (size_t)nb * 5 * sizeof(long long), hipMemcpyDeviceToHost));
    *nblocks_out = nb;
    return GGL_OK;
}

#endif

extern "C" int ggl_dev_ns_schedule(double l, int degrees, int max_steps, int* deg_out, double* coef_out, int* units_out)
{
    ARGCHK(deg_out && coef_out && units_out, "output pointers");
    ARGCHK(l > 0.0 && l <= 1.0, "l must be in (0,1]");
    const int n = ns_schedule_query(l, degrees, max_steps, deg_out, coef_out, units_out);
    if (n < 0) return fail(GGL_E_ARG, "no schedule within %d steps", max_steps);
    return n;
}

extern "C" int ggl_dev_group_partition(const int* units, int K, int p, int max_groups, int* len_out)
{
    ARGCHK(units && len_out && K >= 1 && p >= 1 && max_groups >= 1 && max_groups <= 3, "units, len_out, K, p, 1 <= max_groups <= 3");
    return ns_group_partition(units, K, p, max_groups, len_out);
}
extern "C" int ggl_dev_ns_units(double l, int degrees, double tol) { return ns_units_query(l, degrees, tol); }
extern "C" int ggl_dev_omega_poly_plan(double a, double tol, int degrees, int* deg, double* out, int* units)
{
    ARGCHK(deg && out && units && a > 0.0 && a < 1.0, "deg, out, units, 0 < a < 1");
    return ns_poly_query(std::sqrt(a), degrees, tol, deg, out, units, out + 16, out + 17);
}

extern "C" int ggl_dev_ns_schedule_tol(double l, int degrees, double tol, int max_steps, int* deg_out, double* coef_out,
                                       int* units_out)
{
    ARGCHK(deg_out && coef_out && units_out, "output pointers");
    ARGCHK(l > 0.0 && l <= 1.0, "l must be in (0,1]");
    ARGCHK(tol >= 0.0 && tol <= 1e-6, "tol in [0, 1e-6]");
    const int n = ns_schedule_query(l, degrees, max_steps, deg_out, coef_out, units_out, std::max(tol, NS_TOL_EXACT));
    if (n < 0) return fail(GGL_E_ARG, "no schedule within %d steps", max_steps);
    return n;
}

#ifdef GGL_DEV
extern "C" int ggl_dev_coissue_probe(double* out12)
{
    ARGCHK(out12, "out");
    DevBuf d;
    HIPCHK(d.alloc((size_t)512 * 512));
    coissue_probe(nullptr, d.p, out12);
    HIPCHK(hipGetLastError());
    return GGL_OK;
}

extern "C" int ggl_dev_mfma_lds_probe(double* out6)
{
    ARGCHK(out6, "out");
    DevBuf d;
    HIPCHK(d.alloc((size_t)2048 * 256));
    mfma_lds_probe(nullptr, d.p, out6);
    HIPCHK(hipGetLastError());
    return GGL_OK;
}

extern "C" int ggl_dev_mfma_f64_peak(double* tflops_out)
{
    ARGCHK(tflops_out, "tflops_out");
    const int blocks = 256 * 8;
    DevBuf d;
    HIPCHK(d.alloc((size_t)blocks * 256));
    double best = 0.0;
    for (int r = 0; r < 3; ++r) best = std::max(best, mfma_f64_peak_tflops(nullptr, d.p, blocks, 2000, 8));
    HIPCHK(hipGetLastError());
    if (getenv("GGL_MFMA_PROBE_VERBOSE")) {
        for (int layers : {1, 2, 4, 8})
            for (int nacc : {1, 2, 4, 8})
                fprintf(stderr, "mfma f64 probe: %d wave(s)/SIMD, %d accumulators: %.1f TF/s\n", layers, nacc,
                        mfma_f64_peak_tflops(nullptr, d.p, 256 * layers, 4000, nacc));
    }
    if (getenv("GGL_MFMA_MIX_VERBOSE")) {
        for (int layers : {1, 4})
            for (int nv : {0, 2, 4, 8, 16})
                fprintf(stderr, "mfma+valu mix: %d wave(s)/SIMD, %2d VALU per MFMA: %.1f TF/s\n", layers, nv,
                        mfma_valu_mix_tflops(nullptr, d.p, 256 * layers, 4000, nv));
    }
// ... 238 lines not shown
```

gglasso_amd/csrc/capi_stats.hip:

```cpp
#include "capi_internal.hpp"

extern "C" int ggl_scale_X(ggl_ctx* c, double factor)
{
    ARGCHK(c, "ctx");
    HIPCHK(hipSetDevice(c->device));
    DROP_PRE(c);
    launch_scale(c->stream, c->X, factor, c->n);
    HIPCHK(hipGetLastError());
    return GGL_OK;
}

extern "C" int ggl_profile_enable(ggl_ctx* c, int on)
{
    ARGCHK(c, "ctx");
    HIPCHK(hipSetDevice(c->device));
    if (on && !c->ev[0][0]) {
        for (int ph = 0; ph < GGL_NPHASE; ++ph)
            for (int e = 0; e < 2; ++e) HIPCHK(hipEventCreate(&c->ev[ph][e]));
        for (int q = 0; q < 2; ++q)
            for (int e = 0; e < 2; ++e) HIPCHK(hipEventCreate(&c->ev_early[q][e]));
    }
    c->prof_on = (on == 2) ? 2 : (on != 0 ? 1 : 0);
    return GGL_OK;
}

extern "C" int ggl_ns_stats(ggl_ctx* c, long long out[16])
{
    ARGCHK(c && out, "ctx, out");
    long long lds[4] = {0, 0, 0, 0};
    if (c->lds_calls) { int rc_ = ggl_lds_stats(c, lds); if (rc_) return rc_; }
    out[0] = c->ns_calls;
    out[1] = c->ns_steps_total + (lds[3] + c->K / 2) / c->K;
    out[2] = c->ns_stable_calls;
    out[3] = c->ns_units_total + (lds[2] + c->K / 2) / c->K;
    out[4] = c->ns_launches_total;
    out[5] = c->rank_calls;
    out[6] = c->rank_retries;
    out[7] = c->rank_fallbacks;
    out[8] = c->rank_launches;
    out[9] = c->spec_calls;
    out[10] = c->spec_misses;
    out[11] = c->spin_timeouts;
    out[12] = c->last_parts;
    out[13] = c->last_variant;
    out[14] = c->ns_eigh_fallbacks;
    out[15] = c->pre_dropped;
    return GGL_OK;
}

extern "C" int ggl_omega_poly_stats(ggl_ctx* c, long long out[3])
{
    ARGCHK(c && out, "ctx, out");
    out[0] = c->poly_seqs;
    out[1] = c->poly_seqs_total;
    out[2] = c->poly_last_deg;
    return GGL_OK;
}

extern "C" int ggl_group_stats(ggl_ctx* c, long long out[11], double* units_sum)
{
    ARGCHK(c && out, "ctx, out");
    out[10] = c->group_changes;
    out[0] = c->group_steps;
    out[1] = c->last_groups;
    for (int g = 0; g < 4; ++g) {
        out[2 + g] = c->last_groups > 1 ? c->last_group_len[g] : 0;
        out[6 + g] = c->last_groups > 1 ? c->last_group_units[g] : 0;
        if (units_sum) units_sum[g] = c->group_units_sum[g];
    }
    return GGL_OK;
}

extern "C" int ggl_spectral_bounds(ggl_ctx* c, double* c_out, double* beta_out)
{
    ARGCHK(c && c_out && beta_out, "ctx, c_out, beta_out");
    if (!c->omega_ns || !c->spec_have) return 0;
    for (int k = 0; k < c->K; ++k) { c_out[k] = c->spec_c[k]; beta_out[k] = c->spec_beta[k]; }
    return 1;
}

extern "C" int ggl_lds_stats(ggl_ctx* c, long long out[4])
{
    ARGCHK(c && out, "ctx, out");
    out[0] = c->lds_calls;
    out[1] = c->lds_misses;
    out[2] = out[3] = 0;
    if (c->lds_tab) {
        HIPCHK(hipSetDevice(c->device));
        unsigned long long cnt[2] = {0, 0};
        HIPCHK(hipStreamSynchronize(c->stream));
        HIPCHK(hipMemcpy(cnt, c->lds_tab + (size_t)OMEGA_LDS_MAXTAB * OMEGA_LDS_ENT, sizeof(cnt), hipMemcpyDeviceToHost));
        out[2] = (long long)cnt[0];
        out[3] = (long long)cnt[1];
    }
    return GGL_OK;
}

extern "C" int ggl_pipeline_stats(ggl_ctx* c, long long out[10])
{
    ARGCHK(c && out, "ctx, out");
    out[0] = c->pre_launched;
    out[1] = c->pre_dropped;
    out[2] = c->early_launched;
    out[3] = c->early_used;
    out[4] = c->parts_probed ? c->parts_replaced : -1;
    out[5] = c->wf_written;
    out[6] = c->wf_used;
    out[7] = c->cw_rides;
    out[8] = c->copy_rides;
    out[9] = c->red_rides;
    return GGL_OK;
// ... 116 lines not shown
```

gglasso_amd/csrc/gemm_sym.hip:

```cpp
#include <algorithm>
#include <initializer_list>
#include <mutex>
#include <unordered_map>
#include <type_traits>

#include "common.hpp"
#include "kernels.hpp"

namespace ggl {

typedef double v4d __attribute__((ext_vector_type(4)));

__device__ __forceinline__ double c2val(double dC, double v, double dE, double e) { return __builtin_fma(dE, e, dC * v); }
__device__ __forceinline__ double c2val2(double dC, double v, double dE, double e, bool has2, double dE2, double f)
{
    const double w = c2val(dC, v, dE, e);
    return has2 ? __builtin_fma(dE2, f, w) : w;
}

template <int BM, int BK, int WM, int WN, bool LM>
struct SymCfg {
    static constexpr int NWR = BM / WM, NWC = BM / WN, NW = NWR * NWC, NT = NW * 64;
    static constexpr int TI = WM / 16, TJ = WN / 16;
    static constexpr int LDS_LD = BM + 16;
// ... 7 lines not shown

constexpr int sym_nt(int BM, int WM, int WN) { return (BM / WM) * (BM / WN) * 64; }

static constexpr int NXCD = 8;
__host__ __device__ inline int xcd_share(int K) { return (K == 1 || K == 2 || K == 4) ? NXCD / K : 0; }
__host__ __device__ inline int xcd_grid_small(int ntiles, int K)
{
    const int g = xcd_share(K);
    return g ? NXCD * ((ntiles + g - 1) / g) : NXCD * ((ntiles * K + NXCD - 1) / NXCD);
}
__host__ __device__ inline int xcd_grid(int ntiles, int K)
{
    if (K < NXCD) return xcd_grid_small(ntiles, K);
    const int r = K % NXCD;
    return NXCD * (K / NXCD) * ntiles + (r ? xcd_grid_small(ntiles, r) : 0);
}
__device__ __forceinline__ bool decode_block_small(int ntiles, int K, int& k, int& tile, int L)
{
    const int g = xcd_share(K);
    if (g) {
        const int xcd = L % NXCD, slot = L / NXCD;
        k = xcd / g;
        tile = slot * g + xcd % g;
        return tile < ntiles;
    }
    k = L / ntiles;
    tile = L % ntiles;
    return k < K;
}
__device__ __forceinline__ bool decode_block_xcd(int ntiles, int K, int& k, int& tile, int L)
{
    if (K < NXCD) return decode_block_small(ntiles, K, k, tile, L);
    const int nfull = NXCD * (K / NXCD) * ntiles;
    if (L < nfull) {
        const int xcd = L % NXCD, slot = L / NXCD;
        k = (slot / ntiles) * NXCD + xcd;
        tile = slot % ntiles;
        return true;
    }
    const bool ok = decode_block_small(ntiles, K % NXCD, k, tile, L - nfull);
    k += (K / NXCD) * NXCD;
    return ok;
}
__device__ __forceinline__ bool decode_block_xcd(int ntiles, int K, int& k, int& tile)
{
    return decode_block_xcd(ntiles, K, k, tile, (int)blockIdx.x);
}

template <int BM, int BK, int WM, int WN, bool LM, int ABL = 0>
__global__ __launch_bounds__(sym_nt(BM, WM, WN)) void k_symm_tn(
    const double* __restrict__ A, const double* __restrict__ B, double* __restrict__ C, double* __restrict__ C2,
    const double* __restrict__ E, const double* __restrict__ coef, int K, int p, const double* __restrict__ A1,
    const double* __restrict__ B1, double* __restrict__ C1, int K1, double* __restrict__ maxdev,
    const double* __restrict__ E2)
{
    using Cfg = SymCfg<BM, BK, WM, WN, LM>;
    __shared__ __attribute__((aligned(16))) double smem[Cfg::LDS_DOUBLES];
    double* As = smem;
    double* Bs = smem + Cfg::SLAB;
    const int T = (p + BM - 1) / BM;
    int k, b;
    if (!decode_block_xcd(T * (T + 1) / 2, K + K1, k, b)) return;
    const bool second = k >= K;
    const int kk = second ? k - K : k;
    int I = 0;
    while (b >= T - I) { b -= T - I; ++I; }
    const int J = I + b;
    const int I0 = I * BM, J0 = J * BM;
    const int tid = threadIdx.x, lane = tid & 63, wave = tid >> 6;
    const int wr = (wave / Cfg::NWC) * WM, wc = (wave % Cfg::NWC) * WN;
    const size_t pp = (size_t)p * p;
    const double* Ak = (second ? A1 : A) + (size_t)kk * pp;
    const double* Bk = (second ? B1 : B) + (size_t)kk * pp;

#ifdef GGL_DEV
    long long t_start = 0, t_loop = 0, t_loop_end = 0;
    if (ABL == 3) t_start = clock64();
#endif

    v4d acc[Cfg::TI][Cfg::TJ];
#pragma unroll
    for (int i = 0; i < Cfg::TI; ++i)
#pragma unroll
        for (int j = 0; j < Cfg::TJ; ++j) acc[i][j] = (v4d){0.0, 0.0, 0.0, 0.0};

    constexpr int RSTEP = Cfg::NT / BM;
    constexpr int NST = 1;
    const int lcol = tid % BM, lrow = tid / BM;
    const bool aok = (I0 + lcol) < p, bok = (J0 + lcol) < p;
    double ra[NST][Cfg::LPT], rb[NST][Cfg::LPT];

    const unsigned pu = (unsigned)p, pm1 = (unsigned)(p - 1);
    const unsigned ca = min((unsigned)(I0 + lcol), pm1), cb = min((unsigned)(J0 + lcol), pm1);
    auto fetch = [&](int m0, double (&xa)[Cfg::LPT], double (&xb)[Cfg::LPT]) {
#pragma unroll
        for (int q = 0; q < Cfg::LPT; ++q) {
            if (ABL == 1 || ABL == 4 || ABL == 5) { xa[q] = 1.0 + q; xb[q] = 2.0 + q; continue; }
            const unsigned ro = min((unsigned)(m0 + lrow + q * RSTEP), pm1) * pu;
            xa[q] = Ak[ro + ca];
            xb[q] = Bk[ro + cb];
        }
    };
    auto stage = [&](int m0, const double (&xa)[Cfg::LPT], const double (&xb)[Cfg::LPT]) {
#pragma unroll
        for (int q = 0; q < Cfg::LPT; ++q) {
            const int row = lrow + q * RSTEP;
            const bool in = (m0 + row) < p;
            As[row * Cfg::LDS_LD + lcol] = (in && aok) ? xa[q] : 0.0;
            Bs[row * Cfg::LDS_LD + lcol] = (in && bok) ? xb[q] : 0.0;
        }
    };
    auto compute = [&](int nq) {
        double af[BK / 4][Cfg::TI], bf[BK / 4][Cfg::TJ];
#pragma unroll
        for (int kk = 0; kk < BK / 4; ++kk) {
            if (kk >= nq) break;
// ... 72 lines not shown
                }
                if (LM && I != J) smem[row * Cfg::CLD + col] = v;
            }
    if (maxdev && ABL != 3) {
        double dev = 0.0;
#pragma unroll
        for (int ti = 0; ti < Cfg::TI; ++ti)
#pragma unroll
            for (int tj = 0; tj < Cfg::TJ; ++tj)
#pragma unroll
                for (int r = 0; r < 4; ++r) {
                    const int gi = I0 + wr + ti * 16 + (lane >> 4) + 4 * r;
                    const int gj = J0 + wc + tj * 16 + (lane & 15);
                    if (gi < p && gj < p && (I != J || gi <= gj)) {
                        double v = cAcc * acc[ti][tj][r] + (gi == gj ? cI - 1.0 : 0.0);
                        if (Ek) v += cE * Ek[(size_t)gi * p + gj];
                        if (E2k) v += cE2 * E2k[(size_t)gi * p + gj];
                        dev = fmax(dev, fabs(v));
                    }
                }
        dev = wave_max(dev);
        if (lane == 0 && dev > 0.0)
            atomicMax(reinterpret_cast<unsigned long long*>(maxdev + k), (unsigned long long)__double_as_longlong(dev));
    }
    if (LM && I != J) {
        __syncthreads();
        for (int e = tid; e < BM * BM; e += Cfg::NT) {
            const int a = e / BM, c = e % BM;
            if (J0 + a < p && I0 + c < p) {
                const double v = smem[c * Cfg::CLD + a];
                Ck[(size_t)(J0 + a) * p + I0 + c] = v;
                if (C2k) {
                    const double e0 = (dE != 0.0 && Ek) ? Ek[(size_t)(J0 + a) * p + I0 + c] : 0.0;
                    const double f0 = E2k ? E2k[(size_t)(J0 + a) * p + I0 + c] : 0.0;
                    C2k[(size_t)(J0 + a) * p + I0 + c] = c2val2(dC, v, dE, e0, E2k != nullptr, dE2, f0);
                }
            }
        }
    }
#ifdef GGL_DEV
    if (ABL == 3 && tid == 0) {
        asm volatile("s_waitcnt vmcnt(0)" ::: "memory");
        long long* tl = reinterpret_cast<long long*>(maxdev) + (size_t)blockIdx.x * 5;
        unsigned xcc = 0;
        asm volatile("s_getreg_b32 %0, hwreg(HW_REG_XCC_ID)" : "=s"(xcc));
        tl[0] = t_start; tl[1] = t_loop; tl[2] = t_loop_end; tl[3] = clock64(); tl[4] = (long long)xcc;
    }
#endif
}

template <int BM, int BK, int WM, int WN, bool LM>
static void launch_cfg(hipStream_t st, const double* A, const double* B, double* C, double* C2, const double* E,
                       const double* coef, int K, int p, const double* A1 = nullptr, const double* B1 = nullptr,
                       double* C1 = nullptr, int K1 = 0, double* maxdev = nullptr, const double* E2 = nullptr)
{
    using Cfg = SymCfg<BM, BK, WM, WN, LM>;
    const int T = (p + BM - 1) / BM;
    hipLaunchKernelGGL((k_symm_tn<BM, BK, WM, WN, LM>), dim3(xcd_grid(T * (T + 1) / 2, K + K1)), dim3(Cfg::NT), 0, st, A,
                       B, C, C2, E, coef, K, p, A1, B1, C1, K1, maxdev, E2);
}

typedef __attribute__((address_space(1))) const void* gptr_t;
typedef __attribute__((address_space(3))) void* lptr_t;

template <int N> __device__ __forceinline__ void wait_vmcnt()
{
    static_assert(N >= 0 && N <= 63, "vmcnt range");
    if constexpr (N == 0) asm volatile("s_waitcnt vmcnt(0)" ::: "memory");
    else if constexpr (N == 2) asm volatile("s_waitcnt vmcnt(2)" ::: "memory");
    else if constexpr (N == 4) asm volatile("s_waitcnt vmcnt(4)" ::: "memory");
    else if constexpr (N == 6) asm volatile("s_waitcnt vmcnt(6)" ::: "memory");
    else if constexpr (N == 8) asm volatile("s_waitcnt vmcnt(8)" ::: "memory");
    else if constexpr (N == 12) asm volatile("s_waitcnt vmcnt(12)" ::: "memory");
    else if constexpr (N == 16) asm volatile("s_waitcnt vmcnt(16)" ::: "memory");
    else if constexpr (N == 24) asm volatile("s_waitcnt vmcnt(24)" ::: "memory");
    else static_assert(N == 0, "add the immediate");
}

template <int AUX> __device__ __forceinline__ double ld_pol(const double* p)
{
    if constexpr (AUX == 0) return *p;
    else return __hip_atomic_load(p, __ATOMIC_RELAXED, __HIP_MEMORY_SCOPE_AGENT);
}

template <int BK, int NSTG, int ABL, int BM, int NW, int AUX = 0>
__device__ __forceinline__ void symm_dl_tile(const double* __restrict__ A, const double* __restrict__ B,
                                             double* __restrict__ C, double* __restrict__ C2,
                                             const double* __restrict__ E, const double* __restrict__ E2,
                                             const double* __restrict__ coef, int K,
                                             int p, const double* __restrict__ A1, const double* __restrict__ B1,
                                             double* __restrict__ C1, int K1, double* __restrict__ maxdev,
                                             double* __restrict__ rowpart, double* __restrict__ fropart, int k, int b,
                                             double* smem)
{
    constexpr int NT = NW * 64;
    constexpr int WM = BM / (NW / 2), WN = BM / 2, TI = WM / 16, TJ = WN / 16;
    constexpr int RPI = 128 / BM;
    constexpr int LPR = 64 / RPI;
    constexpr int SLAB = BK * BM;
    constexpr int IPW = BK / (NW * RPI);
    constexpr int RPW = BK / NW;
    static_assert(NW == 4 || NW == 8, "waves per workgroup");
    static_assert(TI >= 1 && TJ >= 1, "wave tile");
    static_assert(BM == 64 || BM == 32, "tile edge");
    static_assert(IPW >= 1, "k-slab too shallow for this tile");
    static_assert(NSTG * 2 * SLAB >= BM * BM, "the mirror tile reuses the slab storage");
    const int T = (p + BM - 1) / BM;
    const int blockTile = b;
    const bool second = k >= K;
    const int kk = second ? k - K : k;
    int I = 0;
    while (b >= T - I) { b -= T - I; ++I; }
// ... 440 lines not shown
    const int lane = threadIdx.x & 63, wid = threadIdx.x >> 6;
    const int nblk = r.nblk, nv = r.nv;
    double acc[8] = {0, 0, 0, 0, 0, 0, 0, 0};
    const double* base = r.partials;
    for (int b = threadIdx.x; b < nblk; b += 512) {
        double t[2][8];
#pragma unroll
        for (int u = 0; u < 2; ++u) {
            const int bb = b + 256 * u;
#pragma unroll
            for (int v = 0; v < 8; ++v) t[u][v] = (v < nv && bb < nblk) ? base[(size_t)bb * nv + v] : 0.0;
        }
#pragma unroll
        for (int u = 0; u < 2; ++u) {
            if (b + 256 * u < nblk) {
#pragma unroll
                for (int v = 0; v < 8; ++v)
                    if (v < nv) acc[v] += t[u][v];
            }
        }
    }
#pragma unroll
    for (int v = 0; v < 8; ++v) {
        if (v < nv) {
            const double s = wave_sum(acc[v]);
            if (lane == 0) sh[wid][v] = s;
        }
    }
    __syncthreads();
    if ((int)threadIdx.x <= nv) {
        const double s = (int)threadIdx.x == nv ? (double)r.seq_val
                                                : (sh[0][threadIdx.x] + sh[1][threadIdx.x]) + (sh[2][threadIdx.x] + sh[3][threadIdx.x]);
        __hip_atomic_store(r.out + threadIdx.x, s, __ATOMIC_RELAXED, __HIP_MEMORY_SCOPE_SYSTEM);
        asm volatile("s_waitcnt vmcnt(0)" ::: "memory");
    }
    __syncthreads();
    if (threadIdx.x == 0) __hip_atomic_store(r.seq, r.seq_val, __ATOMIC_RELAXED, __HIP_MEMORY_SCOPE_SYSTEM);
}

__global__ __launch_bounds__(256) void k_cw_rider(const CwRider rider)
{
    __shared__ __attribute__((aligned(16))) double sh[8 + 256];
    cw_rider_body(rider, (int)blockIdx.x, sh);
}

template <int BK, int NSTG, int ABL = 0, int BM = 64, int NW = 4>
__global__ __launch_bounds__(NW * 64) void k_symm_dl(const double* __restrict__ A, const double* __restrict__ B,
                                                 double* __restrict__ C, double* __restrict__ C2,
                                                 const double* __restrict__ E, const double* __restrict__ E2,
                                                 const double* __restrict__ coef, int K,
                                                 int p, const double* __restrict__ A1, const double* __restrict__ B1,
                                                 double* __restrict__ C1, int K1, double* __restrict__ maxdev,
                                                 double* __restrict__ rowpart, double* __restrict__ fropart, const CwRider rider,
                                                 const CopySegs cps, const RedRider red)
{
    __shared__ __attribute__((aligned(16))) double smem[NSTG * 2 * BK * BM];
    const int T = (p + BM - 1) / BM;
    int bid = (int)blockIdx.x;
    if constexpr (NW == 4) {
        if (red.nblk > 0) {
            if (bid < NXCD) {
                if (bid == 0) red_rider_body(red, smem);
                return;
            }
            bid -= NXCD;
        }
        const int base = xcd_grid(T * (T + 1) / 2, K + K1);
        if (bid >= base) {
            const int idx = bid - base, ncw = rider.K * rider.nbx;
            if (idx < ncw) cw_rider_body(rider, idx, smem);
            else {
                int blk = idx - ncw;
                for (int sgi = 0; sgi < cps.n; ++sgi) {
                    const int nb = (int)((cps.words[sgi] + 1023u) / 1024u);
                    if (blk < nb) {
                        unsigned* d = (unsigned*)cps.dst[sgi];
                        const unsigned* src = (const unsigned*)cps.src[sgi];
                        const unsigned i0 = (unsigned)blk * 1024u + threadIdx.x;
#pragma unroll
                        for (int e = 0; e < 4; ++e) {
                            const unsigned i = i0 + 256u * e;
                            if (i < cps.words[sgi]) d[i] = src ? src[i] : 0u;
                        }
                        break;
                    }
                    blk -= nb;
                }
            }
            return;
        }
    }
    int k, b;
    if (!decode_block_xcd(T * (T + 1) / 2, K + K1, k, b, bid)) return;
    symm_dl_tile<BK, NSTG, ABL, BM, NW>(A, B, C, C2, E, E2, coef, K, p, A1, B1, C1, K1, maxdev, rowpart, fropart, k, b, smem);
}

#ifdef GGL_DEV
template <int SPLIT> __device__ __forceinline__ bool sk_decode(int ntiles, int K, int L, int& k, int& tile, int& part)
{
    auto small = [&](int Ks, int Ls) {
        const int g = xcd_share(Ks);
        if (g) {
            const int xcd = Ls % NXCD, slot = Ls / NXCD;
            k = xcd / g;
            tile = (slot / SPLIT) * g + xcd % g;
            part = slot % SPLIT;
            return tile < ntiles;
        }
        const int u = Ls % (ntiles * SPLIT);
        k = Ls / (ntiles * SPLIT);
        tile = u / SPLIT;
        part = u % SPLIT;
        return k < Ks;
    };
    if (K < NXCD) return small(K, L);
    const int nfull = NXCD * (K / NXCD) * ntiles * SPLIT;
    if (L < nfull) {
        const int xcd = L % NXCD, slot = L / NXCD, u = slot % (ntiles * SPLIT);
        k = (slot / (ntiles * SPLIT)) * NXCD + xcd;
        tile = u / SPLIT;
        part = u % SPLIT;
        return true;
    }
    const bool ok = small(K % NXCD, L - nfull);
    k += (K / NXCD) * NXCD;
    return ok;
}
inline int sk_grid_small(int ntiles, int K, int split)
{
    const int g = xcd_share(K);
    return g ? NXCD * ((ntiles + g - 1) / g) * split : NXCD * ((ntiles * split * K + NXCD - 1) / NXCD);
}
inline int sk_grid(int ntiles, int K, int split)
{
    if (K < NXCD) return sk_grid_small(ntiles, K, split);
    const int r = K % NXCD;
    return NXCD * (K / NXCD) * ntiles * split + (r ? sk_grid_small(ntiles, r, split) : 0);
}

template <int BK, int NSTG, int SPLIT>
__global__ __launch_bounds__(256) void k_symm_sk(const double* __restrict__ A, const double* __restrict__ B,
                                                 double* __restrict__ C, double* __restrict__ C2,
                                                 const double* __restrict__ E, const double* __restrict__ coef, int K,
                                                 int p, double* __restrict__ maxdev, double* __restrict__ rowpart,
                                                 double* __restrict__ fropart, double* __restrict__ scratch,
                                                 unsigned* __restrict__ arrivals)
{
// ... 421 lines not shown
}

int launch_chain_probe(hipStream_t st, double* X0, double* X1, const double* coef, int K, int p, int nprod, int variant,
                       unsigned* bar, unsigned* err, int two_level)
{
    const void* fn = nullptr;
    int BM = 64;
    if (variant == 16) fn = (const void*)k_symm_chain_probe<16, 2, 64>;
    else if (variant == 17) fn = (const void*)k_symm_chain_probe<16, 3, 64>;
    else if (variant == 20) { fn = (const void*)k_symm_chain_probe<32, 2, 32>; BM = 32; }
    else return 0;
    int per_cu = 0, dev = 0;
    hipDeviceProp_t prop;
    if (hipGetDevice(&dev) != hipSuccess || hipGetDeviceProperties(&prop, dev) != hipSuccess) return -1;
    if (hipOccupancyMaxActiveBlocksPerMultiprocessor(&per_cu, fn, 256, 0) != hipSuccess || per_cu < 1) return -1;
    const int T = (p + BM - 1) / BM;
    const int total = xcd_grid(T * (T + 1) / 2, K);
    if (per_cu > 4) per_cu = 4;
    int grid = per_cu * prop.multiProcessorCount;
    if (grid > total) grid = total;
    grid -= grid % NXCD;
    if (grid < NXCD) return -1;
    void* args[] = {&X0, &X1, &coef, &K, &p, &nprod, &bar, &err, &two_level};
    if (hipLaunchCooperativeKernel(fn, dim3(grid), dim3(256), args, 0, st) != hipSuccess) return -1;
    return grid;
}
#endif

static thread_local CwRider g_rider;
static thread_local CopySegs g_copy_rider;
static thread_local RedRider g_red_rider;
void symm_set_reduce_rider(const RedRider& r) { g_red_rider = r; }
void symm_set_rider(const CwRider& r) { g_rider = r; }
void symm_set_copy_rider(const CopySegs& sg) { g_copy_rider = sg; }
void symm_flush_rider(hipStream_t st)
{
    if (g_red_rider.nblk > 0) {
        launch_reduce_partials(st, g_red_rider.partials, 1, g_red_rider.nblk, g_red_rider.nv, g_red_rider.out, g_red_rider.seq,
                               g_red_rider.seq_val);
        g_red_rider = RedRider{};
    }
    if (g_copy_rider.n > 0) {
        launch_copy_small(st, g_copy_rider);
        g_copy_rider = CopySegs{};
    }
    if (g_rider.K <= 0) return;
    hipLaunchKernelGGL(k_cw_rider, dim3(g_rider.K * g_rider.nbx), dim3(256), 0, st, g_rider);
    g_rider = CwRider{};
}

static void launch_dl(hipStream_t st, const double* A, const double* B, double* C, double* C2, const double* E,
                      const double* coef, int K, int p, const double* A1, const double* B1, double* C1, int K1,
                      double* maxdev, int dl_cfg = 0, double* rowpart = nullptr, double* fropart = nullptr,
                      const double* E2 = nullptr)
{
    const bool eight = dl_cfg == 6 || dl_cfg == 7;
    const CwRider rider = (g_rider.K > 0 && !eight) ? g_rider : CwRider{};
    if (rider.K > 0) g_rider = CwRider{};
    const CopySegs cps = (g_copy_rider.n > 0 && !eight) ? g_copy_rider : CopySegs{};
    if (cps.n > 0) g_copy_rider = CopySegs{};
    const RedRider red = (g_red_rider.nblk > 0 && !eight) ? g_red_rider : RedRider{};
    if (red.nblk > 0) g_red_rider = RedRider{};
    int ncopy = red.nblk > 0 ? NXCD : 0;
    for (int i = 0; i < cps.n; ++i) ncopy += (int)((cps.words[i] + 1023u) / 1024u);
    const int nride = rider.K * rider.nbx + ncopy;
#define GGL_DL(...) hipLaunchKernelGGL((k_symm_dl<__VA_ARGS__>), grid, dim3(256), 0, st, A, B, C, C2, E, E2, coef, K, p, A1, B1, C1, K1, maxdev, rowpart, fropart, rider, cps, red)
    if (dl_cfg == 4 || (dl_cfg >= 8 && dl_cfg <= 13) || (dl_cfg >= 18 && dl_cfg <= 21)) {
        const int T32 = (p + 31) / 32;
        const dim3 grid(xcd_grid(T32 * (T32 + 1) / 2, K + K1) + nride);
        if (dl_cfg == 4) GGL_DL(32, 2, 0, 32);
#ifdef GGL_DEV
        else if (dl_cfg == 8) GGL_DL(16, 4, 0, 32);
        else if (dl_cfg == 9) GGL_DL(32, 3, 0, 32);
        else if (dl_cfg == 10) GGL_DL(16, 6, 0, 32);
        else if (dl_cfg == 11) GGL_DL(32, 4, 0, 32);
        else if (dl_cfg == 12) GGL_DL(16, 2, 0, 32);
        else if (dl_cfg == 13) GGL_DL(16, 3, 0, 32);
        else if (dl_cfg == 18) GGL_DL(32, 2, 2, 32);
        else if (dl_cfg == 19) GGL_DL(32, 2, 3, 32);
        else if (dl_cfg == 20) GGL_DL(32, 2, 4, 32);
        else if (dl_cfg == 21) GGL_DL(32, 2, 5, 32);
#endif
        return;
    }
    const int T = (p + 63) / 64;
    const dim3 grid(xcd_grid(T * (T + 1) / 2, K + K1) + nride);
#ifdef GGL_DEV
    if (dl_cfg == 6 || dl_cfg == 7) {
#define GGL_DL8(...) hipLaunchKernelGGL((k_symm_dl<__VA_ARGS__>), grid, dim3(512), 0, st, A, B, C, C2, E, E2, coef, K, p, A1, B1, C1, K1, maxdev, rowpart, fropart, rider, cps, red)
        if (dl_cfg == 6) GGL_DL8(16, 4, 0, 64, 8);
        else GGL_DL8(32, 3, 0, 64, 8);
#undef GGL_DL8
        return;
    }
#endif
    if (dl_cfg == 1) GGL_DL(16, 3);
#ifdef GGL_DEV
    else if (dl_cfg == 2) GGL_DL(16, 4);
    else if (dl_cfg == 3) GGL_DL(32, 2);
    else if (dl_cfg == 5) GGL_DL(16, 2, 1);
    else if (dl_cfg == 14) GGL_DL(16, 3, 2);
    else if (dl_cfg == 15) GGL_DL(16, 3, 3);
    else if (dl_cfg == 16) GGL_DL(16, 3, 4);
    else if (dl_cfg == 17) GGL_DL(16, 3, 5);
    else if (dl_cfg == 22) GGL_DL(8, 4);
    else if (dl_cfg == 23) GGL_DL(8, 6);
#endif
    else GGL_DL(16, 2);
#undef GGL_DL
}

template <int BM, int BK, int WM, int WN>
__global__ __launch_bounds__(sym_nt(BM, WM, WN)) void k_gemm_nt_right(const double* __restrict__ A,
                                                                      const double* __restrict__ T,
                                                                      double* __restrict__ C,
                                                                      const double* __restrict__ scal, int nbatch, int K, int p)
{
    constexpr int NWC = BM / WN, NT = sym_nt(BM, WM, WN), TI = WM / 16, TJ = WN / 16;
    constexpr int LDA = BK + 2;
    constexpr int LDB = BM + 16;
    __shared__ __attribute__((aligned(16))) double smem[BM * LDA + BK * LDB];
    double* As = smem;
    double* Bs = smem + BM * LDA;
    const int Tn = (p + BM - 1) / BM;
    int b, tile;
    if (!decode_block_xcd(Tn * Tn, nbatch, b, tile)) return;
    const int kt = b % K;
    const int I0 = (tile / Tn) * BM, J0 = (tile % Tn) * BM;
    const int tid = threadIdx.x, lane = tid & 63, wave = tid >> 6;
    const int wr = (wave / NWC) * WM, wc = (wave % NWC) * WN;
    const size_t pp = (size_t)p * p;
    const double* Ab = A + (size_t)b * pp;
    const double* Tb = T + (size_t)kt * pp;

    v4d acc[TI][TJ];
#pragma unroll
    for (int i = 0; i < TI; ++i)
#pragma unroll
        for (int j = 0; j < TJ; ++j) acc[i][j] = (v4d){0.0, 0.0, 0.0, 0.0};

    constexpr int LPT = (BM * BK) / NT;
    static_assert((BM * BK) % NT == 0 && NT % BK == 0 && NT % BM == 0, "tile/thread mismatch");
// ... 255 lines not shown
}

int symm_auto_variant(int nprod, int p)
{
    const long T64 = (p + 63) / 64;
    return (T64 * (T64 + 1) / 2 * nprod <= SMALL_BATCH_TILES) ? (p >= SMALL_DL_MIN_P ? 20 : 9) : 16;
}

static void (*g_symm_hook)(hipStream_t, int, void*) = nullptr;
static void* g_symm_hook_arg = nullptr;
void symm_set_launch_hook(void (*fn)(hipStream_t, int, void*), void* arg) { g_symm_hook = fn; g_symm_hook_arg = arg; }
struct SymmHookAtExit {
    hipStream_t st; int kind;
    ~SymmHookAtExit() { if (g_symm_hook) g_symm_hook(st, kind, g_symm_hook_arg); }
};

void launch_symm_pair(hipStream_t st, const double* A, const double* B, double* C, const double* A1, const double* B1,
                      double* C1, const double* coef2K, int K, int p, int variant)
{
    SymmHookAtExit hook{st, 1};
    if (variant < 0) variant = symm_auto_variant(2 * K, p);
    if (variant >= 41 && variant <= 50) variant = 20;
    switch (variant) {
        case 16: case 17: case 18: case 19: case 20: case 22: case 23: case 24: case 25: case 26: case 27: case 28: case 29: case 30: case 31: case 32: case 33: case 34: case 35: case 36: case 37: case 38: case 39:
            if (symm_dl_serves(p)) {
                launch_dl(st, A, B, C, nullptr, nullptr, coef2K, K, p, A1, B1, C1, K, nullptr, variant - 16);
                break;
            }
            if (variant == 20 || variant >= 24) launch_cfg<32, 32, 16, 16, true>(st, A, B, C, nullptr, nullptr, coef2K, K, p, A1, B1, C1, K);
            else launch_cfg<64, 16, 32, 32, true>(st, A, B, C, nullptr, nullptr, coef2K, K, p, A1, B1, C1, K);
            break;
        case 9: launch_cfg<32, 32, 16, 16, true>(st, A, B, C, nullptr, nullptr, coef2K, K, p, A1, B1, C1, K); break;
#ifdef GGL_DEV
        case 1: launch_cfg<64, 32, 32, 32, true>(st, A, B, C, nullptr, nullptr, coef2K, K, p, A1, B1, C1, K); break;
        case 3: launch_cfg<128, 16, 32, 64, false>(st, A, B, C, nullptr, nullptr, coef2K, K, p, A1, B1, C1, K); break;
        case 4: launch_cfg<64, 16, 32, 32, false>(st, A, B, C, nullptr, nullptr, coef2K, K, p, A1, B1, C1, K); break;
        case 8: launch_cfg<32, 16, 16, 16, true>(st, A, B, C, nullptr, nullptr, coef2K, K, p, A1, B1, C1, K); break;
#endif
        default: launch_cfg<64, 16, 32, 32, true>(st, A, B, C, nullptr, nullptr, coef2K, K, p, A1, B1, C1, K); break;
    }
}

int symm_bounds_tile(int K, int p, int variant)
{
    if (variant < 0) variant = symm_auto_variant(K, p);
    if (!symm_dl_serves(p)) return 0;
    if (variant == 20 || (variant >= 24 && variant <= 29) || (variant >= 34 && variant <= 37) || (variant >= 41 && variant <= 50)) return 32;
    if ((variant >= 16 && variant <= 19) || variant == 22 || variant == 23 || (variant >= 30 && variant <= 33) || variant == 38 || variant == 39) return 64;
    return 0;
}

void launch_symm(hipStream_t st, const double* A, const double* B, double* C, double* C2, const double* E,
                 const double* coef, int K, int p, int variant, double* maxdev, double* rowpart, double* fropart,
                 const double* E2)
{
    SymmHookAtExit hook{st, 0};
    if (variant < 0) variant = symm_auto_variant(K, p);
#define GGL_TN(BM, BK, WM, WN, LM) \
    launch_cfg<BM, BK, WM, WN, LM>(st, A, B, C, C2, E, coef, K, p, nullptr, nullptr, nullptr, 0, maxdev, E2)
#ifdef GGL_DEV
    if (E2 && variant >= 41 && variant <= 50) variant = 20;
    if (variant >= 41 && variant <= 50) {
        if ((p & 1) == 0 && p >= 2) { launch_sk(st, A, B, C, C2, E, coef, K, p, maxdev, rowpart, fropart, variant); return; }
        variant = 9;
    }
#endif
    switch (variant) {
        case 16: case 17: case 18: case 19: case 20: case 21: case 22: case 23: case 24: case 25: case 26: case 27: case 28: case 29: case 30: case 31: case 32: case 33: case 34: case 35: case 36: case 37: case 38: case 39:
            if (symm_dl_serves(p)) {
                launch_dl(st, A, B, C, C2, E, coef, K, p, nullptr, nullptr, nullptr, 0, maxdev, variant - 16, rowpart, fropart, E2);
                break;
            }
            if (variant == 20 || variant >= 24) GGL_TN(32, 32, 16, 16, true);
            else GGL_TN(64, 16, 32, 32, true);
            break;
        case 9: GGL_TN(32, 32, 16, 16, true); break;
#ifdef GGL_DEV
        case 1: GGL_TN(64, 32, 32, 32, true); break;
        case 2: GGL_TN(128, 16, 64, 64, false); break;
        case 3: GGL_TN(128, 16, 32, 64, false); break;
        case 4: GGL_TN(64, 16, 32, 32, false); break;
        case 5: GGL_TN(128, 32, 64, 64, false); break;
        case 8: GGL_TN(32, 16, 16, 16, true); break;
        case 11: GGL_TN(64, 16, 16, 32, true); break;
        case 12: GGL_TN(64, 32, 16, 32, true); break;
        case 13: GGL_TN(64, 16, 32, 16, true); break;
        case 6: case 7: case 10: case 14: case 15: {
            const int T = (p + 63) / 64;
            const dim3 grid(xcd_grid(T * (T + 1) / 2, K));
            double* md = (variant == 10) ? maxdev : nullptr;
#define GGL_ABL(N) hipLaunchKernelGGL((k_symm_tn<64, 16, 32, 32, true, N>), grid, dim3(256), 0, st, A, B, C, C2, E, coef, K, p, nullptr, nullptr, nullptr, 0, md, E2)
            if (variant == 6) GGL_ABL(1); else if (variant == 7) GGL_ABL(2); else if (variant == 10) GGL_ABL(3);
            else if (variant == 14) GGL_ABL(4); else GGL_ABL(5);
#undef GGL_ABL
            break;
        }
#endif
        default: GGL_TN(64, 16, 32, 32, true); break;
    }
#undef GGL_TN
}

}
```

gglasso_amd/csrc/kernels.hpp:

```cpp
#pragma once
#include <hip/hip_runtime.h>
#include <stddef.h>

#define GGL_NNORM 5

namespace ggl {

enum EigMap {
    MAP_PHIPLUS = 0,
    MAP_RANK = 1,
    MAP_IDENT = 2
};

int elementwise_blocks(int p);
void launch_form_W(hipStream_t st, double* W, const double* Theta, const double* L, const double* X,
                   const double* S, const double* betaK, int K, int p);
void launch_theta_sgl(hipStream_t st, double* Theta, double* X, double* C, const double* Omega,
                      const double* OmegaPrev, const double* L, const double* l1K,
                      const double* mask, const double* invrhoK, int latent, double* partials, int K, int p, const int* skip = nullptr,
                      const int* pk = nullptr, size_t mask_stride = 0);
void launch_dual_update(hipStream_t st, double* X, const double* Omega, const double* OmegaPrev,
                        const double* Theta, const double* L, double* partials, int K, int p);
void launch_reduce_partials(hipStream_t st, const double* partials, int K, int nblk, int nv, double* out,
                            unsigned long long* seq = nullptr, unsigned long long seq_val = 0, unsigned* arrive = nullptr);
// ... 120 lines not shown
struct I8Op {
    const int8_t* As = nullptr;
    const int8_t* Bs = nullptr;
    size_t sstrideA = 0, sstrideB = 0;
    const double* par = nullptr;
    const double* E1 = nullptr;
    const double* E2 = nullptr;
    double* C1 = nullptr;
    double* C2 = nullptr;
    int8_t* S1 = nullptr;
    int8_t* S2 = nullptr;
    int nS1 = 0, nS2 = 0;
    size_t sstride1 = 0, sstride2 = 0;
    int* flag = nullptr;
    int K = 0, p = 0, P = 0;
};
bool launch_symm_i8_op(hipStream_t st, const I8Op& op, int SA, int SB, int dmax);
static constexpr int I8_NSLICES = 59;
static constexpr int I8_MAXPROD = 8;
struct I8Omega {
    int K = 0, p = 0, P = 0;
    size_t sl = 0;
    int8_t* slab = nullptr;
    double *par = nullptr, *par_h = nullptr;
    double *wscale = nullptr, *wscale_h = nullptr;
    int* flag = nullptr;
};
struct I8Cfg { int s_full = 7, s_f2 = 4, s_gf2 = 3, s_ye = 5, d_ye = 4; };
struct I8Bufs { const double* W; double *Ap, *Bp, *Y1, *F, *F2, *Om; };
struct I8Prog {
    struct Prod { I8Op op; int SA, SB, dmax; } prod[I8_MAXPROD];
    int nprod = 0, units = 0, k0 = 0, Kp = 0, S_W = 7;
};
int i8_omega_alloc(I8Omega* w, int K, int p);
void i8_omega_free(I8Omega* w);
int i8_omega_plan(I8Omega* w, const double* cuse_h, const double* beta_h, int k0, int Kp, double tol, int degrees,
                  const I8Cfg& cfg, const I8Bufs& bufs, I8Prog* prog);
bool i8_omega_run(hipStream_t st, I8Omega* w, const I8Prog& prog, const double* W);
hipError_t launch_jacobi(hipStream_t st, const double* A, double* D, double* R, double* out, int map,
                         const double* betaK, int* info, int K, int p);

void launch_recon(hipStream_t st, double* out, const double* R, const double* D, const double* betaK,
                  int map, int K, int p, double* scale_work);

static constexpr int NS_NCOEF = 8;
int symm_variants();
bool symm_variant_built(int v);
bool symm_dl_serves(int p);
void symm_set_odd_dl(bool on);
int symm_effective_variant(int variant, int p);
int symm_auto_variant(int nprod, int p);
void launch_symm(hipStream_t st, const double* A, const double* B, double* C, double* C2, const double* E,
                 const double* coef, int K, int p, int variant, double* maxdev = nullptr, double* rowpart = nullptr,
                 double* fropart = nullptr, const double* E2 = nullptr);
int symm_bounds_tile(int K, int p, int variant);
void symm_release_workspace(hipStream_t st);

struct SymmOp {
    const double *A, *B, *E, *A1, *B1, *E2;
    double *C, *C2, *C1;
    const double* coef;
    double *rowpart, *fropart;
    int pair, pad_;
};
static constexpr int CHAIN_MAX_OPS = 16;
struct ChainProg {
    int nops, K, p, ntiles;
    int begin[CHAIN_MAX_OPS + 1];
    SymmOp op[CHAIN_MAX_OPS];
    long long* prof = nullptr;
};
int chain_tile(int K, int p, bool force = false);
static constexpr int CHAIN_CNT_STRIDE = 32;
static constexpr int CHAIN_MAX_INST = 64;
static_assert(CHAIN_MAX_OPS + 1 <= CHAIN_CNT_STRIDE, "one line holds the completion word and the ticket words");
int launch_omega_chain(hipStream_t st, const ChainProg& P, unsigned* state, int* flag, int* flag_h, int aux = 16);

#ifdef GGL_DEV
int launch_chain_probe(hipStream_t st, double* X0, double* X1, const double* coef, int K, int p, int nprod, int variant,
                       unsigned* bar, unsigned* err, int two_level);
#endif
#ifdef GGL_DEV
void coissue_probe(hipStream_t st, double* scratch, double* out);
void mfma_lds_probe(hipStream_t st, double* scratch, double* out);
#endif
double mfma_f64_peak_tflops(hipStream_t st, double* scratch, int blocks, int iters, int nacc);
double mfma_valu_mix_tflops(hipStream_t st, double* scratch, int blocks, int iters, int nv);
void launch_gemm_right(hipStream_t st, const double* A, const double* T, double* C, const double* scal,
                       int nbatch, int K, int p, int variant);


struct CwRider {
    const double* B = nullptr;
    const double* rowpart = nullptr;
    const double* fropart = nullptr;
    const double* dprev = nullptr;
    double* dnext = nullptr;
    double* d_out = nullptr;
    unsigned long long* cwmax = nullptr;
    unsigned* cnt = nullptr;
    double* out = nullptr;
    const double* cuse = nullptr;
    int* flag = nullptr;
    int* flag_host = nullptr;
    int flag_slot = 0;
    int T = 0, ntile = 0, p = 0, K = 0;
    int nbx = 0;
};
void symm_set_copy_rider(const CopySegs& sg);
struct RedRider {
    const double* partials = nullptr;
    double* out = nullptr;
    unsigned long long* seq = nullptr;
    unsigned long long seq_val = 0;
    int nblk = 0, nv = 0;
};
void symm_set_reduce_rider(const RedRider& r);
void symm_set_rider(const CwRider& r);
void symm_flush_rider(hipStream_t st);
void symm_set_launch_hook(void (*fn)(hipStream_t, int, void*), void* arg);
void launch_symm_pair(hipStream_t st, const double* A, const double* B, double* C, const double* A1, const double* B1,
                      double* C1, const double* coef2K, int K, int p, int variant);

static constexpr double NS_TOL_EXACT = 4e-16;
static constexpr double NS_TOL_DEFAULT = 2e-12;
static constexpr int NS_MAX_STEPS = 24;
static constexpr int NS_RANK_MAX_STEPS = 40;
static constexpr int NS_MAX_LAUNCHES = 2 * NS_RANK_MAX_STEPS + 1 + 3;
static inline size_t NS_SLOT(int K) { return (size_t)K * 2 * NS_NCOEF; }
static constexpr double NS_SYM_KAPPA_MAX = 300.0;
static constexpr double NS_KAPPA_LIMIT = 1e12;
struct NsPlan {
    int steps = 0; int products = 0; bool stable = false; double kappa = 0.0; int units = 0; int direct = 0;
    double check = 5e-5;
    unsigned char deg[NS_RANK_MAX_STEPS] = {};
};
int form_W_tiles(int p);
void launch_form_W_sym(hipStream_t st, double* W, const double* Theta, const double* L, const double* X,
                       const double* S, const double* betaK, int K, int p);
int ns_plan(const double* cbound_h, const double* beta_h, int K, double* coef_h, double* start_h, NsPlan* plan,
            int force_mode, int degrees = 9, double tol = NS_TOL_EXACT, int poly = 0);
int ns_poly_query(double l, int degrees, double tol, int* deg, double* coef, int* units, double* a_out, double* err_out);
int ns_schedule_query(double l, int degrees, int max_steps, int* deg, double* coef, int* units, double tol = NS_TOL_EXACT);
int ns_units_query(double l, int degrees, double tol);
int ns_group_partition(const int* units, int K, int p, int max_groups, int* len_out);
void ns_prepare(hipStream_t st, const double* pre0_d, const double* pre1_d, const double* W, double* Ap, double* Bp,
                int K, int p, int variant, double* start2 = nullptr, double* rowpart = nullptr, double* fropart = nullptr,
                bool start_w = false);
void ns_run(hipStream_t st, const NsPlan& plan, const double* coef_d, const double* start_d, const double* W,
            double* AB, double* YP, double* Tb, double* out, int K, int p, int variant, size_t pstride = 0,
            bool fused_start = false, hipEvent_t bprime_free = nullptr);
int ns_chain_ops(const NsPlan& plan, const double* pre0_d, const double* pre1_d, const double* coef_d, const double* W,
                 double* AB, double* YP, double* NX, double* Tb, double* out, int K, int p, size_t pstride, double* start2,
                 double* rowpart, double* fropart, SymmOp* ops, int max_ops);
double* ns_fused_start(const NsPlan& plan, const double* start_hk, double* YP, double* Tb, size_t n1, double* row);

int norm_bounds_blocks(int p);
void launch_norm_bounds(hipStream_t st, const double* W, int K, int p, double* part, double* rowsum = nullptr);
void launch_cw_bounds(hipStream_t st, const double* W, const double* rowsum, int K, int p, double* part);
void launch_bound_final(hipStream_t st, const double* part2, const double* cwpart, int nbb, int K, double* out, int mode,
                        const double* cuse = nullptr, int* flag = nullptr, int* flag_host = nullptr);
int bound_rows_blocks(int p);
void launch_bound_rows(hipStream_t st, const double* rowpart, int T, int K, int p, double* d, double* infpart);
void launch_bound_cw(hipStream_t st, const double* B, const double* rowpart, int T, int K, int p, double* d_out,
                     const double* fropart, int ntile, unsigned long long* cwmax, unsigned* cnt, double* out,
                     const double* cuse, int* flag, int* flag_host, int flag_slot, const double* dprev, double* dnext);
void launch_cw_final(hipStream_t st, const double* B, const double* d, int K, int p, const double* infpart,
                     const double* fropart, int ntile, unsigned long long* cwmax, unsigned* cnt, double* out,
                     const double* cuse, int* flag, int* flag_host, int flag_slot, const double* dprev = nullptr,
                     double* dnext = nullptr);
int rank_ns_plan(const double* cnorm_h, const double* mu_h, int K, double l0, double* coef_h, NsPlan* plan,
                 int degrees = 9);
double rank_ns_image(double l0, int degrees, double x);
double rank_trace_tolerance(double l0, int p);
int rank_ns_plan_continue(const double* mu_h, int m, double lp, double* coef_h, NsPlan* plan, int degrees, size_t slot);
void rank_ns_steps(hipStream_t st, const NsPlan& plan, const double* coef_d, const double* C, double* X, double* Xn, double* Tb,
                   double* P2, double* out, double* maxdev, int K, int p, int variant, size_t cs);
void rank_ns_run(hipStream_t st, const NsPlan& plan, const double* coef_d, const double* C, double* Xa, double* Xb,
                 double* Tb, double* P2, double* out, double* maxdev, int K, int p, int variant, size_t cslot = 0,
                 bool t0_ready = false);
void launch_bound_sqrt_inf_fro(hipStream_t st, const double* infpart, int ninf, const double* fropart, int ntile, int K,
                               double* out);
void launch_rank_t0(hipStream_t st, double* P, const double* C, const double* coef_d, int K, int p);

}
```

gglasso_amd/csrc/newton_schulz.hip:

```cpp
#include <cmath>
#include <vector>
#include <unordered_map>

#include <functional>
#include "common.hpp"
#include "kernels.hpp"

namespace ggl {

static constexpr int FT = 32, FTY = 8, FQ = FT / FTY;

template <bool HAS_L>
__global__ __launch_bounds__(256) void k_form_W_sym(double* __restrict__ W, const double* __restrict__ Theta,
                                                    const double* __restrict__ L, const double* __restrict__ X,
                                                    const double* __restrict__ S, const double* __restrict__ betaK,
                                                    int p)
{
    __shared__ double tile[FT][FT + 1];
    const int k = blockIdx.y;
    const int T = (p + FT - 1) / FT;
    int I = 0, b = blockIdx.x;
    while (b >= T - I) { b -= T - I; ++I; }
    const int J = I + b;
    const int I0 = I * FT, J0 = J * FT;
// ... 523 lines not shown
    for (int g = gbest; g >= 1; --g) {
        const int i = from[(size_t)g * (K + 1) + j];
        len_out[g - 1] = j - i;
        j = i;
    }
    return gbest;
}

__global__ __launch_bounds__(256) void k_ns_start(double* __restrict__ Y1, double* __restrict__ Z1,
                                                  const double* __restrict__ Ap, const double* __restrict__ Bp,
                                                  const double* __restrict__ W, const double* __restrict__ st, int p,
                                                  int mode)
{
    const int k = blockIdx.y;
    const size_t pp = (size_t)p * p, base = (size_t)k * pp;
    const double y1a = st[k * 5 + 0], y1b = st[k * 5 + 1], z1i = st[k * 5 + 2], z1a = st[k * 5 + 3], h = st[k * 5 + 4];
    size_t i = (size_t)blockIdx.x * 1024 + threadIdx.x;
#pragma unroll
    for (int e = 0; e < 4; ++e, i += 256) {
        if (i < pp) {
            const double a = Ap[base + i], b2 = Bp[base + i];
            const int r = (int)(i / p), c = (int)(i - (size_t)r * p);
            if (mode == 2) {
                Z1[base + i] = __builtin_fma(z1a, a, y1b * b2) + (r == c ? z1i : 0.0);
                continue;
            }
            if (mode == 3) {
                Y1[base + i] = __builtin_fma(y1a, a, y1b * b2) + (r == c ? z1i : 0.0);
                continue;
            }
            if (mode == 4) {
                Y1[base + i] = __builtin_fma(0.5, W[base + i], __builtin_fma(y1a, a, y1b * b2)) + (r == c ? z1i : 0.0);
                continue;
            }
            const double y = y1a * a + y1b * b2;
            if (mode == 1) {
                Y1[base + i] = 0.5 * W[base + i] + h * y;
            } else {
                Y1[base + i] = y;
                Z1[base + i] = z1a * a + (r == c ? z1i : 0.0);
            }
        }
    }
}

static void launch_ns_start(hipStream_t st, double* Y1, double* Z1, const double* Ap, const double* Bp, const double* W,
                            const double* stt, int K, int p, int mode)
{
    dim3 grid((unsigned)(((size_t)p * p + 1023) / 1024), K);
    hipLaunchKernelGGL(k_ns_start, grid, dim3(256), 0, st, Y1, Z1, Ap, Bp, W, stt, p, mode);
}

int ns_plan(const double* cbound_h, const double* beta_h, int K, double* coef_h, double* start_h, NsPlan* plan,
            int force_mode, int degrees, double tol, int poly)
{
    std::vector<double> c(K);
    double kappa = 1.0;
    for (int k = 0; k < K; ++k) {
        c[k] = cbound_h[k] * (1.0 + 1e-10);
        if (!(c[k] > 0.0) || !std::isfinite(c[k]) || !(beta_h[k] > 0.0)) return -1;
        if (c[k] < 4.0 * beta_h[k]) c[k] = 4.0 * beta_h[k];
        kappa = std::fmax(kappa, c[k] / (4.0 * beta_h[k]));
    }
    const bool stable = (force_mode == 2) || (force_mode == 0 && kappa > NS_SYM_KAPPA_MAX);
    if (kappa > NS_KAPPA_LIMIT) return -2;
    const double lmin = 1.0 / std::sqrt(kappa);
    plan->stable = stable;
    plan->kappa = kappa;
    plan->direct = 0;
    auto put = [&](int g, int k, double cI, double cAcc, double cE, double dI = 0.0, double dC = 0.0, double dE = 0.0,
                   double cE2 = 0.0, double dE2 = 0.0) {
        double* o = coef_h + (size_t)g * NS_SLOT(K) + (size_t)k * NS_NCOEF;
        o[0] = cI; o[1] = cAcc; o[2] = cE; o[3] = dI; o[4] = dC; o[5] = dE; o[6] = cE2; o[7] = dE2;
    };
    const int pd = (!stable && poly) ? ns_poly_choice(lmin, degrees, tol) : 0;
    if (pd) {
        const NsPoly pp = ns_poly_plan(lmin, tol, pd);
        const int J = pd / 3;
        const double a = pp.a, m = 0.5 * (1.0 + a), h = 0.5 * (1.0 - a), u = 1.0 / (h * h * h);
        plan->direct = pd;
        plan->steps = 1;
        plan->deg[0] = 0;
        plan->units = pp.units;
        plan->products = J + 2;
        for (int k = 0; k < K; ++k) {
            const double ck = c[k], hc = 0.5 * std::sqrt(ck);
            auto digit = [&](int j, double* o3) {
                const double a0 = pp.co[3 * j], a1 = pp.co[3 * j + 1], a2 = pp.co[3 * j + 2];
                o3[0] = a0 - a1 * (m / h) + a2 * (m / h) * (m / h);
                o3[1] = a1 / (ck * h) - 2.0 * a2 * m / (ck * h * h);
                o3[2] = a2 / (ck * ck * h * h);
            };
            double dg[3];
            digit(0, dg);
            double* s = start_h + (size_t)k * 5;
            s[0] = hc * dg[1]; s[1] = hc * dg[2]; s[2] = hc * dg[0]; s[3] = 0.0; s[4] = 0.0;
            int g = 0;
            digit(J - 1, dg);
            put(g++, k, -m * m * m * u, u / (ck * ck * ck), -3.0 * m * u / (ck * ck), dg[0], pp.co[3 * J], dg[2],
                3.0 * m * m * u / ck, dg[1]);
            for (int j = J - 2; j >= 1; --j) {
                digit(j, dg);
                put(g++, k, dg[0], 1.0, dg[2], 0.0, 0.0, 0.0, dg[1]);
            }
            put(g++, k, 0.0, hc, 1.0);
        }
        return 0;
    }
    if (!stable) {
        const NsSeq& sq = ns_mixed_schedule(lmin, degrees, tol);
        if (sq.n < 1 || sq.n > NS_MAX_STEPS || sq.cost >= (1 << 29)) return -2;
        const int n = sq.n;
        plan->steps = n;
        plan->units = 2 + sq.cost;
        int g = 0;
        for (int it = 0; it < n; ++it) plan->deg[it] = sq.deg[it];
        for (int k = 0; k < K; ++k) {
            const double ck = c[k], sc = std::sqrt(ck);
            double* s = start_h + (size_t)k * 5;
            const double* t = sq.st[0].t;
            g = 0;
            if (sq.deg[0] == 3) {
                s[0] = t[0] / ck; s[1] = t[1] / (ck * ck); s[2] = t[0]; s[3] = t[1] / ck; s[4] = 0.5 * sc;
            } else {
                if (sq.deg[0] == 5) {
                    s[0] = 0.0; s[1] = t[2] / (ck * ck); s[2] = t[0]; s[3] = t[1] / ck; s[4] = 0.0;
                } else {
                    s[0] = t[3] / ck; s[1] = t[4] / (ck * ck); s[2] = t[2]; s[3] = 0.0; s[4] = 0.0;
                    put(g++, k, t[0], 1.0 / (ck * ck), t[1] / ck);
                }
                if (n == 1) put(g++, k, 0.0, 0.5 * sc / ck, 0.5);
                else put(g++, k, 0.0, 1.0 / ck, 0.0);
            }
            for (int it = 1; it < n; ++it) {
                t = sq.st[it].t;
                if (sq.deg[it] == 3) {
                    put(g++, k, t[0], t[1], 0.0);
                } else if (sq.deg[it] == 5) {
                    put(g++, k, 0.0, 1.0, 0.0);
                    put(g++, k, t[0], t[2], t[1]);
                } else {
                    const double a = t[3] / (2.0 * t[4]), d = t[2] / t[4] - a * a, e = t[1] - t[4] * d * a;
                    put(g++, k, 0.0, 1.0, 0.0);
                    put(g++, k, 0.0, 1.0, a, d, 1.0);
                    put(g++, k, t[0], t[4], e);
                }
                if (it == n - 1) put(g++, k, 0.0, 0.5 * sc, 0.5);
                else {
                    put(g, k, 0.0, 1.0, 0.0);
                    put(g, K + k, 0.0, 1.0, 0.0);
                    ++g;
                }
            }
        }
        plan->products = 2 + g;
        return 0;
    }
    std::vector<std::vector<double>> al(K);
    int n = 1;
// ... 21 lines not shown
            put(g++, k, 1.5, -0.5 * a * a, 0.0);
            if (it == n - 1) put(g++, k, 0.0, 0.5 * sc * a, 0.5);
            else {
                double* o = coef_h + (size_t)g * NS_SLOT(K);
                o[k] = a;
                o[K + k] = a;
                ++g;
            }
        }
    }
    return 0;
}

void ns_prepare(hipStream_t st, const double* pre0_d, const double* pre1_d, const double* W, double* Ap, double* Bp, int K,
                int p, int variant, double* start2, double* rowpart, double* fropart, bool start_w)
{
    launch_symm(st, W, W, Ap, nullptr, nullptr, pre0_d, K, p, variant);
    symm_flush_rider(st);
    launch_symm(st, Ap, Ap, Bp, start2, start2 ? Ap : nullptr, pre1_d, K, p, variant, nullptr, rowpart, fropart,
                start2 && start_w ? W : nullptr);
}

double* ns_fused_start(const NsPlan& plan, const double* start_hk, double* YP, double* Tb, size_t n1, double* row)
{
    double* out3 = row + 3;
    row[7] = 0.0;
    if (plan.direct) {
        out3[0] = start_hk[2]; out3[1] = start_hk[1]; out3[2] = start_hk[0]; row[7] = 0.5;
        return Tb;
    }
    if (plan.stable || plan.deg[0] < 5) return nullptr;
    if (plan.deg[0] == 5) { out3[0] = start_hk[2]; out3[1] = start_hk[1]; out3[2] = start_hk[3]; return YP + n1; }
    out3[0] = start_hk[2]; out3[1] = start_hk[1]; out3[2] = start_hk[0];
    return Tb;
}

void ns_run(hipStream_t st, const NsPlan& plan, const double* coef_d, const double* start_d, const double* W,
            double* AB, double* YP, double* Tb, double* out, int K, int p, int variant, size_t pstride, bool fused_start,
            hipEvent_t bprime_free)
{
    bool bwaited = bprime_free == nullptr;
    const double* bprime = AB + (pstride ? pstride : (size_t)K * p * p);
    auto before_write = [&](const double* o1, const double* o2) {
        if (!bwaited && (o1 == bprime || o2 == bprime)) { (void)hipStreamWaitEvent(st, bprime_free, 0); bwaited = true; }
    };
    struct AtExit { std::function<void()> f; ~AtExit() { f(); } } at_exit{[&]() { before_write(bprime, nullptr); }};
    const size_t cs = NS_SLOT(K), n1 = pstride ? pstride : (size_t)K * p * p;
    const int n = plan.steps;
    int g = 0;
    if (plan.direct) {
        if (!fused_start) launch_ns_start(st, Tb, nullptr, AB, AB + n1, W, start_d, K, p, 4);
        const int J = plan.direct / 3;
        auto hbuf = [&](int j) { return (j & 1) ? YP + n1 : out; };
        launch_symm(st, AB, AB + n1, YP, hbuf(J - 1), AB + n1, coef_d + cs * g++, K, p, variant, nullptr, nullptr, nullptr, AB);
        for (int j = J - 2; j >= 1; --j)
            launch_symm(st, hbuf(j + 1), YP, hbuf(j), nullptr, AB + n1, coef_d + cs * g++, K, p, variant, nullptr, nullptr,
                        nullptr, AB);
        launch_symm(st, hbuf(1), YP, out, nullptr, Tb, coef_d + cs * g++, K, p, variant);
        return;
    }
    double *cur = YP, *nxt = AB;
    if (plan.deg[0] >= 5 && !plan.stable) {
        if (plan.deg[0] == 5) {
            if (!fused_start)
                launch_ns_start(st, nullptr, YP + n1, AB, AB + n1, W, start_d, K, p, 2);
        } else {
            if (!fused_start)
                launch_ns_start(st, Tb, nullptr, AB, AB + n1, W, start_d, K, p, 3);
            launch_symm(st, Tb, AB + n1, YP + n1, nullptr, AB, coef_d + cs * g++, K, p, variant);
        }
        if (n == 1) {
            launch_symm(st, AB, YP + n1, out, nullptr, W, coef_d + cs * g++, K, p, variant);
            return;
        }
        launch_symm(st, AB, YP + n1, YP, nullptr, nullptr, coef_d + cs * g++, K, p, variant);
    } else {
        if (n == 1) {
            launch_ns_start(st, out, nullptr, AB, AB + n1, W, start_d, K, p, 1);
            return;
        }
        launch_ns_start(st, YP, YP + n1, AB, AB + n1, W, start_d, K, p, 0);
    }
    for (int it = 1; it < n; ++it) {
        if (plan.deg[it] == 5 && !plan.stable) {
            launch_symm(st, cur + n1, cur, nxt, nullptr, nullptr, coef_d + cs * g++, K, p, variant);
            launch_symm(st, nxt, nxt, Tb, nullptr, nxt, coef_d + cs * g++, K, p, variant);
        } else if (plan.deg[it] == 9 && !plan.stable) {
            launch_symm(st, cur + n1, cur, out, nullptr, nullptr, coef_d + cs * g++, K, p, variant);
            before_write(nxt, nxt + n1);
            launch_symm(st, out, out, nxt, nxt + n1, out, coef_d + cs * g++, K, p, variant);
            launch_symm(st, nxt, nxt + n1, Tb, nullptr, out, coef_d + cs * g++, K, p, variant);
        } else {
            launch_symm(st, cur + n1, cur, Tb, nullptr, nullptr, coef_d + cs * g++, K, p, variant);
        }
        if (it == n - 1) {
            launch_symm(st, cur, Tb, out, nullptr, W, coef_d + cs * g++, K, p, variant);
        } else if (plan.stable) {
            before_write(nxt + n1, nullptr);
            launch_gemm_right(st, cur, Tb, nxt, coef_d + cs * g++, 2 * K, K, p, 0);
            std::swap(cur, nxt);
        } else {
            before_write(nxt, nxt + n1);
            launch_symm_pair(st, cur, Tb, nxt, Tb, cur + n1, nxt + n1, coef_d + cs * g++, K, p, variant);
            std::swap(cur, nxt);
        }
    }
// ... 606 lines not shown
```

gglasso_amd/solver.py:

```python
import math
import time
import warnings

import numpy as np

from . import _lib
from ._lib import as_c, check, ptr

_REG = {"SGL": _lib.REG_SGL, "GGL": _lib.REG_GGL, "FGL": _lib.REG_FGL, "FSGL": _lib.REG_FSGL}


ENGINE_OPTIONS = {}


RANK_REL_TOL = 1e-9


def latent_rank(L, rel_tol=0.0):
    a = np.abs(np.linalg.eigvalsh(L))
    return int(np.count_nonzero(a > a.max() * max(rel_tol, L.shape[0] * np.finfo(np.float64).eps)))


def _host_period(A, K=None, p=None):
    if K is not None:
# ... 351 lines not shown

    def ext_set_state(self, Lambda, X1):
        check(self.lib.ggl_ext_set_state(self.h, ptr(as_c(Lambda)), ptr(None if X1 is None else as_c(X1))))

    def ext_state(self):
        shape = (self.K, self.p, self.p)
        Lam, X1 = np.empty(shape), np.empty(shape)
        check(self.lib.ggl_ext_get_state(self.h, ptr(Lam), ptr(X1)))
        return {'Lambda': Lam, 'X1': X1}

    def ext_step(self, rho, lambda1K, lambda2, latent, mu1):
        rc = self.lib.ggl_ext_admm_step(self.h, rho, self._cptr(lambda1K), lambda2, int(latent), self._cptr(mu1),
                                        self._norms_p)
        if rc != 0:
            if rc > 0:
                raise RuntimeError(f"ggl_ext_admm_step: unexpected return code {rc} (speculative step rejected twice)")
            check(rc)
        return self._norms

    def ext_kkt(self, rho, lambda1K, lambda2, latent, mu1):
        out = np.zeros(1)
        check(self.lib.ggl_ext_kkt_residual(self.h, rho, ptr(lambda1K), lambda2, int(latent), ptr(mu1), ptr(out)))
        return float(out[0])

    def state(self):
        shape = (self.K, self.p, self.p)
        Om, Th, L, X = (np.empty(shape) for _ in range(4))
        check(self.lib.ggl_get_state(self.h, ptr(Om), ptr(Th), ptr(L), ptr(X)))
        return {'Omega': Om, 'Theta': Th, 'L': L, 'X': X}

    def profile(self, on=1):
        check(self.lib.ggl_profile_enable(self.h, int(on)))

    def profile_read(self, reset=True):
        import ctypes
        ms = np.zeros(len(_lib.PHASES))
        cnt = (ctypes.c_longlong * len(_lib.PHASES))()
        check(self.lib.ggl_profile_read(self.h, ptr(ms), cnt, int(reset)))
        return {name: (float(ms[i]), int(cnt[i])) for i, name in enumerate(_lib.PHASES)}

    def ns_stats(self):
        import ctypes
        out = (ctypes.c_longlong * 16)()
        check(self.lib.ggl_ns_stats(self.h, out))
        return dict(zip(("calls", "steps", "stable_calls", "units", "launches", "rank_calls", "rank_retries",
                         "rank_fallbacks", "rank_launches", "spec_calls", "spec_misses", "spin_timeouts", "last_parts",
                         "last_variant", "eigh_fallbacks", "pre_dropped"), (int(v) for v in out)))

    def poly_stats(self):
        import ctypes
        out = (ctypes.c_longlong * 3)()
        check(self.lib.ggl_omega_poly_stats(self.h, out))
        return dict(zip(("seqs", "seqs_total", "last_deg"), (int(v) for v in out)))

    def rank_stats(self):
        import ctypes
        out = (ctypes.c_longlong * 4)()
        check(self.lib.ggl_rank_stats(self.h, out))
        st = dict(zip(("calls", "continued_calls", "continued_instances", "eigh_fallbacks"), (int(v) for v in out)))
        d = (ctypes.c_longlong * 2)()
        check(self.lib.ggl_deflate_stats(self.h, d))
        st["deflated_calls"], st["deflated_instances"] = int(d[0]), int(d[1])
        return st

    def group_stats(self):
        import ctypes
        out = (ctypes.c_longlong * 11)()
        us = np.zeros(4)
        check(self.lib.ggl_group_stats(self.h, out, ptr(us)))
        g = int(out[1])
        return {'steps': int(out[0]), 'groups': g, 'changes': int(out[10]), 'len': [int(out[2 + i]) for i in range(g)] if g > 1 else [],
                'units': [int(out[6 + i]) for i in range(g)] if g > 1 else [], 'units_sum': us.tolist()}

    def spectral_bounds(self):
        cb, be = np.zeros(self.K), np.zeros(self.K)
        if check(self.lib.ggl_spectral_bounds(self.h, ptr(cb), ptr(be))) == 0:
            return None
        return cb, be

    def lds_stats(self):
        import ctypes
        out = (ctypes.c_longlong * 4)()
        check(self.lib.ggl_lds_stats(self.h, out))
        return dict(zip(("calls", "misses", "products", "steps"), (int(v) for v in out)))

    def pipeline_stats(self):
        import ctypes
        out = (ctypes.c_longlong * 10)()
        check(self.lib.ggl_pipeline_stats(self.h, out))
        return dict(zip(("prelaunched", "dropped", "early_launched", "early_used", "part_streams_tried", "w_fused", "w_fused_used",
                         "bound_rides", "copy_rides", "reduce_rides"),
                        (int(v) for v in out)))

    def eig_info(self):
        import ctypes
        out = np.zeros(self.K, dtype=np.int32)
        check(self.lib.ggl_eig_info(self.h, out.ctypes.data_as(ctypes.POINTER(ctypes.c_int))))
        return out

    def last_dispatch(self):
        import ctypes
        out = (ctypes.c_longlong * 4)()
        check(self.lib.ggl_last_dispatch(self.h, out))
        return dict(zip(("parts", "variant", "theta_kernel", "finalize_calls"), (int(v) for v in out)))

    def device_ptr(self, which):
# ... 384 lines not shown
```

include/ggl_hip.h:

```cpp
#ifndef GGL_HIP_H
#define GGL_HIP_H

#ifdef __cplusplus
extern "C" {
#endif

#define GGL_VERSION 300

#define GGL_OK 0
#define GGL_E_ARG (-1)
#define GGL_E_HIP (-2)
#define GGL_E_SOLVER (-3)
#define GGL_E_ALLOC (-4)
#define GGL_E_COMM (-5)

#define GGL_REG_SGL 0
#define GGL_REG_GGL 1
#define GGL_REG_FGL 2
#define GGL_REG_FSGL 3

#define GGL_EIG_AUTO 0
#define GGL_EIG_JACOBI 1
#define GGL_EIG_ROCSOLVER 2
#define GGL_EIG_NEWTON_SCHULZ 3
// ... 8 lines not shown
#define GGL_BUF_THETA 2
#define GGL_BUF_L 3
#define GGL_BUF_X 4
#define GGL_BUF_GROUPSQ 5
#define GGL_BUF_NORMS 6
#define GGL_BUF_OMEGA_PREV 7

typedef struct ggl_ctx ggl_ctx;

int ggl_version(void);
const char *ggl_last_error(void);
int ggl_device_count(void);

int ggl_ctx_create(int device, int K, int p, int flags, void *stream, ggl_ctx **out);
int ggl_ctx_destroy(ggl_ctx *ctx);
int ggl_ctx_sync(ggl_ctx *ctx);
void *ggl_device_ptr(ggl_ctx *ctx, int which);

#define GGL_OPT_SPECULATE 1
#define GGL_OPT_SPEC_FACTOR 2
#define GGL_OPT_NS_MODE 3
#define GGL_OPT_NS_DEGREES 4
#define GGL_OPT_THETA_FLAT 5
#define GGL_OPT_RANK_EIG 6
#define GGL_OPT_PARTS 7
#define GGL_OPT_PARTS_MAX_TILES 8
#define GGL_OPT_SYMM_VARIANT 9
#define GGL_OPT_SPIN_WAIT 10
#define GGL_OPT_FUSED_BOUNDS 11
#define GGL_OPT_PIPELINE 12
#define GGL_OPT_FUSED_START 13
#define GGL_OPT_PARTS_SMALL 14
#define GGL_OPT_NS_TOL 15
#define GGL_OPT_CW_WARM 16
#define GGL_OPT_CHAIN 17
#define GGL_OPT_RANK_DEFLATE 20
#define GGL_OPT_RANK_L0_DEFLATE 21
#define GGL_OPT_FUSED_CW 22
#define GGL_OPT_OMEGA_LDS 23
#define GGL_OPT_EARLY_PART 24
#define GGL_OPT_FUSED_W 26
#define GGL_OPT_RANK_CW 27
#define GGL_OPT_BOUND_SIDE 28
#define GGL_OPT_LDS_PINNED 29
#define GGL_OPT_JOIN_FLAG 30
#define GGL_OPT_CW_RIDER 31
#define GGL_OPT_COPY_RIDER 32
#define GGL_OPT_REDUCE_RIDER 33
#define GGL_OPT_PARTS_BIAS 34
#define GGL_OPT_PARTS_ORDER 35
#define GGL_OPT_DOWNLOAD_THREADS 36
#define GGL_OPT_GROUP_SCHED 37
#define GGL_OPT_OMEGA_POLY 38
#define GGL_OPT_PART_PRIORITY 25
#define GGL_OPT_ISOLATE 19
#define GGL_OPT_RANK_L0_COARSE 18
int ggl_ctx_set_option(ggl_ctx *ctx, int option, double value);
int ggl_ctx_get_option(ggl_ctx *ctx, int option, double *value);

int ggl_set_S(ggl_ctx *ctx, const double *S_host);
int ggl_set_state(ggl_ctx *ctx, const double *Omega, const double *Theta, const double *L,
                  const double *X);
int ggl_set_S_ex(ggl_ctx *ctx, const double *S_host, int period);
int ggl_set_state_ex(ggl_ctx *ctx, const double *Omega, const double *Theta, const double *L, const double *X,
                     const int *periods);
int ggl_get_state(ggl_ctx *ctx, double *Omega, double *Theta, double *L, double *X);
int ggl_state_snapshot(ggl_ctx *ctx, int restore);
int ggl_set_lambda1_mask(ggl_ctx *ctx, const double *lam_pp_host);

int ggl_admm_step(ggl_ctx *ctx, double rho, double lambda1, double lambda2, int reg, int latent,
                  const double *mu1, const double *nk, double out_norms[5]);
int ggl_hint_last_step(ggl_ctx *ctx);

int ggl_step_omega(ggl_ctx *ctx, double rho, int latent, const double *nk);
int ggl_step_group_partial(ggl_ctx *ctx, double rho, double lambda1);
int ggl_step_omega_spec(ggl_ctx *ctx, double rho, int latent, const double *nk);
int ggl_step_finish(ggl_ctx *ctx, double rho, double lambda1, double lambda2, int reg, int latent,
                    const double *mu1, int groupsq_ready, double out_norms[5]);
int ggl_norms_read(ggl_ctx *ctx, double out_norms[5]);

int ggl_comm_unique_id(char id_out[128]);
int ggl_comm_init(ggl_ctx *ctx, int rank, int nranks, const char id[128]);
int ggl_comm_destroy(ggl_ctx *ctx);
int ggl_comm_count(ggl_ctx *ctx, int *nranks_out);
int ggl_allreduce_groupsq(ggl_ctx *ctx);
int ggl_allreduce_norms(ggl_ctx *ctx);
int ggl_admm_step_sharded(ggl_ctx *ctx, double rho, double lambda1, double lambda2, const double *nk,
                          double out_norms[5]);
int ggl_admm_step_sharded_latent(ggl_ctx *ctx, double rho, double lambda1, double lambda2, int latent,
                                 const double *mu1, const double *nk, double out_norms[5]);

int ggl_sgl_batch_step(ggl_ctx *ctx, const double *rho, const double *lambda1, int latent,
                       const double *mu1, double *out_norms);
int ggl_set_instance_dims(ggl_ctx *ctx, const int *pk);
int ggl_set_block_size(ggl_ctx *ctx, int M);
int ggl_set_lambda1_mask_k(ggl_ctx *ctx, const double *lam_Kpp_host);
int ggl_scale_X_batch(ggl_ctx *ctx, const double *factor);
int ggl_get_state_k(ggl_ctx *ctx, int k, double *Omega, double *Theta, double *L, double *X);

int ggl_mgl_batch_step(ggl_ctx *ctx, int G, const double *rho, const double *lambda1, const double *lambda2,
                       int reg, int latent, const double *mu1, const double *nk, double *out_norms);

int ggl_batch_decide(int n, const double *sq, const unsigned char *live, const unsigned char *marked, double *rho,
                     const double *dims, double tol, double rtol, int update_rho, double *last, double *fac, int *status);
int ggl_sgl_batch_run(ggl_ctx *ctx, int n_iters, double *rho, const double *lambda1, int latent, const double *mu1,
                      const double *dims, double tol, double rtol, int update_rho, double *last, int *status,
// ... 13 lines not shown

int ggl_exit_checks_k(ggl_ctx *ctx, int latent, double *out);
int ggl_exit_checks_fast_k(ggl_ctx *ctx, int latent, double shift_tl, double shift_l, double *out);

int ggl_ext_setup(ggl_ctx *ctx, const int *pk, const int *G, int L);
int ggl_ext_set_state(ggl_ctx *ctx, const double *Lambda, const double *X1);
int ggl_ext_get_state(ggl_ctx *ctx, double *Lambda, double *X1);
int ggl_ext_admm_step(ggl_ctx *ctx, double rho, const double *lambda1K, double lambda2, int latent,
                      const double *mu1, double out_norms[5]);
int ggl_ext_kkt_residual(ggl_ctx *ctx, double rho, const double *lambda1K, double lambda2, int latent,
                         const double *mu1, double *out);
int ggl_ext_setup_batch(ggl_ctx *ctx, int nprob, const int *pk, const int *G, int L);
int ggl_ext_batch_step(ggl_ctx *ctx, double rho, const double *lambda1K, const double *lambda2G, int latent,
                       const double *mu1, double *out_norms);

int ggl_snapshot_k(ggl_ctx *ctx, int k);
int ggl_snapshot_from(ggl_ctx *ctx, int kd, ggl_ctx *src, int ks);
int ggl_selection_stats(ggl_ctx *ctx, double *out);
int ggl_threshold_scan(ggl_ctx *ctx, const double *tau, int ntau, double *out, int *n_eig);
int ggl_selection_rank(ggl_ctx *ctx, double rel_tol, double *out);
int ggl_finalize_L(ggl_ctx *ctx, int which, int *rank_out);
int ggl_debug_poison(int on);
int ggl_set_odd_dl(int on);
int ggl_failed_instances(ggl_ctx *ctx, int *out);
int ggl_failed_reason(ggl_ctx *ctx, int k, double out[2]);
int ggl_reset_instance(ggl_ctx *ctx, int k);
int ggl_ctx_create_subset(ggl_ctx *src, const int *idx, int m, ggl_ctx **out);
int ggl_get_snapshot_k(ggl_ctx *ctx, int k, double *Theta, double *L);
int ggl_get_snapshot_state_k(ggl_ctx *ctx, int k, double *Omega, double *X);
int ggl_objective(ggl_ctx *ctx, double lambda1, double lambda2, int reg, double out[3]);

int ggl_kkt_residual(ggl_ctx *ctx, double rho, double lambda1, double lambda2, int reg, int latent,
                     const double *mu1, const double *nk, double *out);

#define GGL_PH_FORM_W 0
#define GGL_PH_EIG_OMEGA 1
#define GGL_PH_RECON_OMEGA 2
#define GGL_PH_THETA 3
#define GGL_PH_EIG_L 4
#define GGL_PH_RECON_L 5
#define GGL_PH_DUAL 6
#define GGL_PH_REDUCE 7
#define GGL_PH_EIG_OMEGA2 8
#define GGL_PH_BOUND 9
#define GGL_PH_ALLREDUCE_GROUPSQ 10
#define GGL_PH_ALLREDUCE_NORMS 11
#define GGL_NPHASE 12
int ggl_profile_enable(ggl_ctx *ctx, int on);
int ggl_profile_read(ggl_ctx *ctx, double ms[GGL_NPHASE], long long count[GGL_NPHASE], int reset);
int ggl_ns_stats(ggl_ctx *ctx, long long out[16]);
int ggl_lds_stats(ggl_ctx *ctx, long long out[4]);
int ggl_group_stats(ggl_ctx *ctx, long long out[11], double *units_sum);
int ggl_omega_poly_stats(ggl_ctx *ctx, long long out[3]);
int ggl_spectral_bounds(ggl_ctx *ctx, double *c_out, double *beta_out);
int ggl_pipeline_stats(ggl_ctx *ctx, long long out[10]);
int ggl_rank_stats(ggl_ctx *ctx, long long out[4]);
int ggl_deflate_stats(ggl_ctx *ctx, long long out[2]);
int ggl_finalize_stats(ggl_ctx *ctx, long long out[2]);
int ggl_last_dispatch(ggl_ctx *ctx, long long out[4]);
int ggl_fsgl_stats(ggl_ctx *ctx, long long out[4]);
int ggl_trace_start(ggl_ctx *ctx, int max_events);
int ggl_trace_read(ggl_ctx *ctx, double *out, int cap);
int ggl_eig_info(ggl_ctx *ctx, int *out);

int ggl_dev_symm(int K, int p, const double *A, const double *B, const double *E, const double *coef5K,
                 double *C, double *C2, int variant);
int ggl_dev_symm_bench(int K, int p, int variant, int iters, double *ms_out);
int ggl_dev_omega_lds(int K, int p, const double *Theta, const double *L, const double *X, const double *S, const double *beta,
                      double tol, int degrees, double *Omega, double *cbound, int iters, double *out);
int ggl_dev_symm_bounds(int K, int p, const double *A, const double *B, int variant, double *C,
                        double *rowsum_out, double *fro2_out, double *bound_out);
int ggl_dev_ns_schedule(double l, int degrees, int max_steps, int *deg_out, double *coef_out, int *units_out);
int ggl_dev_ns_schedule_tol(double l, int degrees, double tol, int max_steps, int *deg_out, double *coef_out,
                            int *units_out);
int ggl_dev_group_partition(const int *units, int K, int p, int max_groups, int *len_out);
int ggl_dev_ns_units(double l, int degrees, double tol);
int ggl_dev_omega_poly_plan(double a, double tol, int degrees, int *deg, double *out, int *units);
#ifdef GGL_DEV
int ggl_dev_i8_stages(int n);
int ggl_dev_symm_i8(int K, int p, int S, int dmax, const double *A, const double *B, double scaleA, double scaleB, double *C,
                    int iters, double *ms_out);
int ggl_dev_omega_i8(int K, int p, const double *W, const double *beta, const double *cbound, const int *cfg5, double tol,
                     double *Omega, int iters, double *ms_out);
int ggl_dev_mfma_f64_peak(double *tflops_out);
int ggl_dev_coissue_probe(double *out12);
int ggl_dev_mfma_lds_probe(double *out6);
int ggl_dev_chain_run(int K, int p, int nprod, int iters, double *out);
int ggl_dev_switch_bench(int K, int p, int variant, int iters, int mode, double *ms_out);
int ggl_dev_vendor_bench(int K, int p, int mode, int iters, double *ms_out);
int ggl_dev_fill_copy_probe(int reps, int K, int p, int slices, int gap_us, long long out[2]);
int ggl_dev_symm_timeline(int K, int p, long long *out, int max_blocks, int *nblocks_out);
int ggl_dev_chain_probe(int K, int p, int variant, int nprod, int iters, int two_level, double *out);
#endif

int ggl_eigh_batched(int K, int p, const double *A, double *D, double *Q, int eig_method);
int ggl_phiplus(int K, int p, const double *beta, const double *D, const double *Q, double *out);
int ggl_prox_rank_norm(int K, int p, const double *beta, const double *D, const double *Q, double *out);
int ggl_phiplus_matrix(int K, int p, const double *beta, const double *W, double *out, int eig_method);
int ggl_rank_matrix(int K, int p, const double *beta, const double *C, double *out, int eig_method);
int ggl_rank_matrix_ex(int K, int p, const double *beta, const double *C, double *out, int eig_method, double l0_coarse,
                       long long stats[6]);
int ggl_rank_matrix_deflate(int K, int p, const double *beta, const double *C, double *out, int eig_method, double l0_deflate,
                            long long stats[8]);
int ggl_prox_od_1norm(int p, const double *A, double lam, const double *lam_pp, double *out);
int ggl_prox_sum_frob(int p, int M, const double *X, double l, double *out);
int ggl_frob_norm_per_block(int p, int M, const double *S, int off_diag, double *out);
int ggl_prox_p(int K, int p, const double *X, double l1, double l2, int reg, double *out);
int ggl_prox_tv(int n, int K, const double *Y, double lam, double *out);
int ggl_prox_2norm(int n, int K, const double *Y, double lam, double *out);
int ggl_prox_phi(int n, int K, const double *Y, double l1, double l2, int reg, double *out);

#ifdef __cplusplus
}
#endif
#endif
```

Measured before the change: 1475.

## Schedule per-instance polynomial degrees so short instances skip a matrix product

Adds per-instance scheduling for the direct polynomial Omega step. When instance degrees differ by exactly one digit, instances needing fewer terms are given an index list and skip one batched product. The product kernels gain an instance-index indirection, so split launches can cover subsets of instances. This is meant to cut wasted matrix products for well-conditioned instances, at the cost of extra launches and more complex coefficient layout.

```diff
diff --git a/gglasso_amd/_lib.py b/gglasso_amd/_lib.py
--- a/gglasso_amd/_lib.py
+++ b/gglasso_amd/_lib.py
@@ -11,7 +11,7 @@
 EIG_AUTO, EIG_JACOBI, EIG_ROCSOLVER, EIG_NEWTON_SCHULZ = 0, 1, 2, 3
 CTX_STREAM_GIVEN = 1 << 16
 OPTIONS = {"speculate": 1, "spec_factor": 2, "ns_mode": 3, "ns_degrees": 4, "theta_flat": 5, "rank_eig": 6, "parts": 7,
-           "parts_max_tiles": 8, "symm_variant": 9, "spin_wait": 10, "fused_bounds": 11, "pipeline": 12, "fused_start": 13, "parts_small": 14, "ns_tol": 15, "cw_warm": 16, "chain": 17, "rank_l0_coarse": 18, "isolate": 19, "rank_deflate": 20, "rank_l0_deflate": 21, "fused_cw": 22, "omega_lds": 23, "early_part": 24, "part_priority": 25, "fused_w": 26, "rank_cw": 27, "bound_side": 28, "lds_pinned": 29, "join_flag": 30, "cw_rider": 31, "copy_rider": 32, "reduce_rider": 33, "parts_bias": 34, "parts_order": 35, "download_threads": 36, "group_sched": 37, "omega_poly": 38}
+           "parts_max_tiles": 8, "symm_variant": 9, "spin_wait": 10, "fused_bounds": 11, "pipeline": 12, "fused_start": 13, "parts_small": 14, "ns_tol": 15, "cw_warm": 16, "chain": 17, "rank_l0_coarse": 18, "isolate": 19, "rank_deflate": 20, "rank_l0_deflate": 21, "fused_cw": 22, "omega_lds": 23, "early_part": 24, "part_priority": 25, "fused_w": 26, "rank_cw": 27, "bound_side": 28, "lds_pinned": 29, "join_flag": 30, "cw_rider": 31, "copy_rider": 32, "reduce_rider": 33, "parts_bias": 34, "parts_order": 35, "download_threads": 36, "group_sched": 37, "omega_poly": 38, "inst_sched": 39}
 
 
 def eig_flags(method=EIG_AUTO, ns_mode=0, ns_degrees=0):
@@ -124,6 +124,9 @@
     "ggl_dev_ns_units": ([_d, _i, _d], _i),
     "ggl_dev_omega_poly_plan": ([_d, _d, _i, ctypes.POINTER(_i), _dp, ctypes.POINTER(_i)], _i),
     "ggl_omega_poly_stats": ([_vp, ctypes.POINTER(ctypes.c_longlong)], _i),
+    "ggl_inst_sched_stats": ([_vp, ctypes.POINTER(ctypes.c_longlong)], _i),
+    "ggl_dev_symm_inst": ([_i, _i, _dp, _dp, _dp, _dp, _dp, _ip, _i, _i, _dp, _dp, _dp, _dp], _i),
+    "ggl_dev_inst_plan": ([_i, _dp, _dp, _d, _i, _i, _i, _ip, _ip, _ip], _i),
     "ggl_ns_stats": ([_vp, ctypes.POINTER(ctypes.c_longlong)], _i),
     "ggl_rank_stats": ([_vp, ctypes.POINTER(ctypes.c_longlong)], _i),
     "ggl_deflate_stats": ([_vp, ctypes.POINTER(ctypes.c_longlong)], _i),
diff --git a/gglasso_amd/csrc/capi_batch.hip b/gglasso_amd/csrc/capi_batch.hip
--- a/gglasso_amd/csrc/capi_batch.hip
+++ b/gglasso_amd/csrc/capi_batch.hip
@@ -509,7 +509,7 @@
     c->symm_variant = src->symm_variant; c->spin_wait = src->spin_wait; c->fused_bounds = src->fused_bounds;
     c->pipeline = src->pipeline; c->fused_start = src->fused_start; c->parts_small = src->parts_small; c->download_threads = src->download_threads; c->ns_tol = src->ns_tol;
     c->cw_warm = src->cw_warm; c->rank_l0 = src->rank_l0; c->rank_l0_coarse = src->rank_l0_coarse;
-    c->group_sched = src->group_sched; c->omega_poly = src->omega_poly;
+    c->group_sched = src->group_sched; c->omega_poly = src->omega_poly; c->inst_sched = src->inst_sched;
     c->isolate = src->isolate; c->lds_omega = src->lds_omega; c->lds_waves = src->lds_waves; c->early_part = src->early_part; c->rank_deflate = src->rank_deflate; c->rank_l0_deflate = src->rank_l0_deflate;
     int* didx = nullptr;
     hipError_t e = hipMalloc(&didx, m * sizeof(int));
diff --git a/gglasso_amd/csrc/capi_ctx.hip b/gglasso_amd/csrc/capi_ctx.hip
--- a/gglasso_amd/csrc/capi_ctx.hip
+++ b/gglasso_amd/csrc/capi_ctx.hip
@@ -354,6 +354,10 @@
             if (v != 0.0 && v != 1.0) return fail(GGL_E_ARG, "bad argument: GGL_OPT_OMEGA_POLY is 0 or 1");
             c->omega_poly = (int)v;
             break;
+        case GGL_OPT_INST_SCHED:
+            if (v != 0.0 && v != 1.0 && v != 2.0) return fail(GGL_E_ARG, "bad argument: GGL_OPT_INST_SCHED is 0, 1 or 2");
+            c->inst_sched = (int)v;
+            break;
 #ifdef GGL_DEV
         case GGL_OPT_PARTS_BIAS: c->parts_bias = (int)v; break;
         case GGL_OPT_PARTS_ORDER: c->parts_order = (int)v; break;
@@ -446,6 +450,7 @@
         case GGL_OPT_PARTS_SMALL: *value = c->parts_small; break;
         case GGL_OPT_GROUP_SCHED: *value = c->group_sched; break;
         case GGL_OPT_OMEGA_POLY: *value = c->omega_poly; break;
+        case GGL_OPT_INST_SCHED: *value = c->inst_sched; break;
         case GGL_OPT_PARTS_BIAS: *value = c->parts_bias; break;
         case GGL_OPT_PARTS_ORDER: *value = c->parts_order; break;
         case GGL_OPT_DOWNLOAD_THREADS: *value = c->download_threads; break;
diff --git a/gglasso_amd/csrc/capi_internal.hpp b/gglasso_amd/csrc/capi_internal.hpp
--- a/gglasso_amd/csrc/capi_internal.hpp
+++ b/gglasso_amd/csrc/capi_internal.hpp
@@ -136,6 +136,9 @@
     int omega_poly = 1;
     long long poly_seqs = 0, poly_seqs_total = 0;
     int poly_last_deg = 0;
+    int inst_sched = 1;
+    long long inst_seqs = 0, inst_skipped = 0;
+    long long inst_products = 0;
     int parts_small = 8;
     bool fused_start = true;
     bool fused_bounds = true;
diff --git a/gglasso_amd/csrc/capi_omega.hip b/gglasso_amd/csrc/capi_omega.hip
--- a/gglasso_amd/csrc/capi_omega.hip
+++ b/gglasso_amd/csrc/capi_omega.hip
@@ -237,6 +237,16 @@
     if (pl.direct) { c->poly_seqs += 1; c->poly_last_deg = pl.direct; }
 }
 
+static void note_sequence(ggl_ctx* c, const NsPlan& pl, int Kr)
+{
+    const double frac = (double)Kr / c->K;
+    c->ns_launches_total += pl.products + (pl.n_short ? 1 : 0);
+    c->ns_units_frac += frac * pl.units - (double)pl.n_short / c->K;
+    c->ns_steps_frac += frac * pl.steps;
+    c->inst_products += (long long)Kr * pl.units - pl.n_short;
+    if (pl.n_short) { c->inst_seqs += 1; c->inst_skipped += pl.n_short; }
+}
+
 static int omega_groups(const ggl_ctx* c, const double* cb, const double* beta_h, int K, int* Kh, int* k0h, int* gunits)
 {
     if (!c->group_sched || K < 2 || c->ns_force == 2 || c->chain_mode || c->comm) return 1;
@@ -357,6 +367,7 @@
         c->last_variant = symm_effective_variant(var_parts >= 0 ? var_parts : symm_auto_variant(Kh[0], c->p), c->p);
         const size_t region = (size_t)(NS_MAX_LAUNCHES - 4) / nh * NS_SLOT(K);
         NsPlan plans[ggl_ctx::MAX_PARTS];
+        auto inst_on = [&](int var) { return (!c->chain_mode && !(var >= 41 && var <= 50)) ? c->inst_sched : 0; };
         double* start_base_h = c->coef_h + (size_t)(NS_MAX_LAUNCHES - 3) * NS_SLOT(K);
         double* start_base_d = c->coef + (size_t)(NS_MAX_LAUNCHES - 3) * NS_SLOT(K);
         double* fused[ggl_ctx::MAX_PARTS] = {};
@@ -516,7 +527,8 @@
             for (int h = 0; spec && h < nh; ++h) {
                 const int k0 = k0h[h];
                 const int prc = ns_plan(c->cuse_h + k0, c->par_h + k0, Kh[h], c->coef_h + h * region,
-                                        start_base_h + 5 * k0, &plans[h], c->ns_force, c->ns_degrees, c->ns_tol, c->omega_poly);
+                                        start_base_h + 5 * k0, &plans[h], c->ns_force, c->ns_degrees, c->ns_tol, c->omega_poly,
+                                        inst_on(var_parts));
                 spec = (prc == 0) && !plans[h].stable;
                 for (int k = k0; spec && c->fused_start && k < k0 + Kh[h]; ++k) {
                     fused[h] = ns_fused_start(plans[h], start_base_h + 5 * (size_t)k, c->nsYP[1] + k0 * pp, c->nsT + k0 * pp,
@@ -668,11 +680,8 @@
                        c->nsYP[1] + k0 * pp, c->nsT + k0 * pp, c->Om[nxt] + k0 * pp, Kh[h], c->p,
                        var_parts, nh > 1 ? c->n : 0, fused[h] != nullptr, bfree);
                 symm_flush_rider(sh);
-                c->ns_launches_total += plans[h].products;
                 note_family(c, plans[h]);
-                const double frac = (double)Kh[h] / K;
-                c->ns_units_frac += frac * plans[h].units;
-                c->ns_steps_frac += frac * plans[h].steps;
+                note_sequence(c, plans[h], Kh[h]);
             }
             if (h == 0 && !spec) PE(c, GGL_PH_EIG_OMEGA);
         }
@@ -736,7 +745,8 @@
         for (int h = 0; h < nh; ++h) {
             const int k0 = k0h[h];
             const int prc = ns_plan(c->bounds_h + k0, c->par_h + k0, Kh[h], c->coef_h + h * region_b, start_base_h + 5 * k0,
-                                    &plans[h], c->ns_force, c->ns_degrees, c->ns_tol, c->omega_poly);
+                                    &plans[h], c->ns_force, c->ns_degrees, c->ns_tol, c->omega_poly,
+                                    inst_on(nh > 1 ? var_b : c->symm_variant));
             if (prc == -1) return fail(GGL_E_SOLVER, "Newton-Schulz Omega-step: non-finite W (diverged iterate?)");
             if (prc == -2) {
                 c->ns_eigh_fallbacks += 1;
@@ -775,11 +785,8 @@
                    c->p,
                    nrun > 1 ? var_b : c->symm_variant, nrun > 1 ? c->n : 0);
             c->ns_stable_calls += plans[h].stable ? 1 : 0;
-            c->ns_launches_total += plans[h].products;
             note_family(c, plans[h]);
-            const double frac = (double)Kr / K;
-            c->ns_units_frac += frac * plans[h].units;
-            c->ns_steps_frac += frac * plans[h].steps;
+            note_sequence(c, plans[h], Kr);
         }
         for (int h = 1; h < nrun; ++h) {
             HIPCHK(hipEventRecord(c->ev_join[h - 1], c->streamx[h - 1]));
diff --git a/gglasso_amd/csrc/capi_ops.hip b/gglasso_amd/csrc/capi_ops.hip
--- a/gglasso_amd/csrc/capi_ops.hip
+++ b/gglasso_amd/csrc/capi_ops.hip
@@ -90,6 +90,47 @@
     DOWN(C, dC.p, n);
     if (C2) DOWN(C2, dC2.p, n);
     return GGL_OK;
+}
+
+extern "C" int ggl_dev_symm_inst(int K, int p, const double* A, const double* B, const double* E, const double* E2,
+                                 const double* coef8K, const int* inst, int nact, int variant, double* C, double* C2,
+                                 double* rowpart, double* fropart)
+{
+    ARGCHK(K >= 1 && p >= 1 && A && B && coef8K && C, "arguments");
+    ARGCHK(variant < 0 || symm_variant_built(variant), "product-kernel variant not in this build");
+    ARGCHK(!inst || (nact >= 1 && nact <= K), "1 <= nact <= K");
+    for (int i = 0; inst && i < nact; ++i) {
+        ARGCHK(inst[i] >= 0 && inst[i] < K, "inst[i] outside [0, K)");
+        for (int j = 0; j < i; ++j) ARGCHK(inst[j] != inst[i], "an instance listed twice");
+    }
+    if (variant < 0) variant = symm_auto_variant(K, p);
+    const int tile = (rowpart && fropart) ? symm_bounds_tile(K, p, variant) : 0;
+    const int T = tile ? (p + tile - 1) / tile : 0, ntile = T * (T + 1) / 2;
+    const size_t n = (size_t)K * p * p;
+    DevBuf dA, dB, dE, dE2, dC, dC2, dcoef, drow, dfro;
+    int* dinst = nullptr;
+    struct FreeI { int** q; ~FreeI() { if (*q) (void)hipFree(*q); } } freei{&dinst};
+    HIPCHK(dA.alloc(n)); HIPCHK(dB.alloc(n)); HIPCHK(dC.alloc(n)); HIPCHK(dcoef.alloc((size_t)K * NS_NCOEF));
+    UP(dA.p, A, n); UP(dB.p, B, n); UP(dC.p, C, n); UP(dcoef.p, coef8K, (size_t)K * NS_NCOEF);
+    if (E) { HIPCHK(dE.alloc(n)); UP(dE.p, E, n); }
+    if (E2) { HIPCHK(dE2.alloc(n)); UP(dE2.p, E2, n); }
+    if (C2) { HIPCHK(dC2.alloc(n)); UP(dC2.p, C2, n); }
+    if (tile) {
+        HIPCHK(drow.alloc((size_t)K * T * p)); HIPCHK(dfro.alloc((size_t)K * ntile));
+        UP(drow.p, rowpart, (size_t)K * T * p); UP(dfro.p, fropart, (size_t)K * ntile);
+    }
+    if (inst) {
+        HIPCHK(hipMalloc(&dinst, nact * sizeof(int)));
+        HIPCHK(hipMemcpy(dinst, inst, nact * sizeof(int), hipMemcpyHostToDevice));
+    }
+    launch_symm(nullptr, dA.p, dB.p, dC.p, C2 ? dC2.p : nullptr, E ? dE.p : nullptr, dcoef.p, inst ? nact : K, p, variant, nullptr,
+                tile ? drow.p : nullptr, tile ? dfro.p : nullptr, E2 ? dE2.p : nullptr, dinst);
+    HIPCHK(hipGetLastError());
+    HIPCHK(hipDeviceSynchronize());
+    DOWN(C, dC.p, n);
+    if (C2) DOWN(C2, dC2.p, n);
+    if (tile) { DOWN(rowpart, drow.p, (size_t)K * T * p); DOWN(fropart, dfro.p, (size_t)K * ntile); }
+    return tile;
 }
 
 extern "C" int ggl_dev_symm_bounds(int K, int p, const double* A, const double* B, int variant, double* C,
@@ -748,6 +789,23 @@
     return ns_poly_query(std::sqrt(a), degrees, tol, deg, out, units, out + 16, out + 17);
 }
 
+extern "C" int ggl_dev_inst_plan(int K, const double* cbound, const double* beta, double tol, int degrees, int poly, int inst_sched,
+                                 int* units_out, int* list_out, int* info_out)
+{
+    ARGCHK(K >= 1 && cbound && beta && units_out && list_out && info_out, "arguments");
+    std::vector<double> coef((size_t)NS_MAX_LAUNCHES * NS_SLOT(K), 0.0), start((size_t)K * 5, 0.0);
+    NsPlan pl;
+    const int rc = ns_plan(cbound, beta, K, coef.data(), start.data(), &pl, 0, degrees, tol, poly, inst_sched);
+    if (rc != 0) return fail(GGL_E_ARG, "ns_plan: %d (non-finite bounds, or a condition number beyond the matrix-function route)", rc);
+    const int* lst = reinterpret_cast<const int*>(coef.data() + (size_t)K * NS_NCOEF);
+    const int nl = pl.n_short ? K - pl.n_short : 0;
+    for (int k = 0; k < K; ++k) units_out[k] = pl.units;
+    for (int i = 0; i < nl; ++i) list_out[i] = lst[i];
+    for (int i = 0; i < pl.n_short; ++i) units_out[lst[nl + i]] = pl.units - 1;
+    info_out[0] = pl.direct; info_out[1] = nl; info_out[2] = pl.units; info_out[3] = pl.products + (pl.n_short ? 1 : 0);
+    return GGL_OK;
+}
+
 extern "C" int ggl_dev_ns_schedule_tol(double l, int degrees, double tol, int max_steps, int* deg_out, double* coef_out,
                                        int* units_out)
 {
diff --git a/gglasso_amd/csrc/capi_stats.hip b/gglasso_amd/csrc/capi_stats.hip
--- a/gglasso_amd/csrc/capi_stats.hip
+++ b/gglasso_amd/csrc/capi_stats.hip
@@ -57,6 +57,15 @@
     return GGL_OK;
 }
 
+extern "C" int ggl_inst_sched_stats(ggl_ctx* c, long long out[3])
+{
+    ARGCHK(c && out, "ctx, out");
+    out[0] = c->inst_seqs;
+    out[1] = c->inst_skipped;
+    out[2] = c->inst_products;
+    return GGL_OK;
+}
+
 extern "C" int ggl_group_stats(ggl_ctx* c, long long out[11], double* units_sum)
 {
     ARGCHK(c && out, "ctx, out");
diff --git a/gglasso_amd/csrc/gemm_sym.hip b/gglasso_amd/csrc/gemm_sym.hip
--- a/gglasso_amd/csrc/gemm_sym.hip
+++ b/gglasso_amd/csrc/gemm_sym.hip
@@ -83,7 +83,7 @@
     const double* __restrict__ A, const double* __restrict__ B, double* __restrict__ C, double* __restrict__ C2,
     const double* __restrict__ E, const double* __restrict__ coef, int K, int p, const double* __restrict__ A1,
     const double* __restrict__ B1, double* __restrict__ C1, int K1, double* __restrict__ maxdev,
-    const double* __restrict__ E2)
+    const double* __restrict__ E2, const int* __restrict__ inst)
 {
     using Cfg = SymCfg<BM, BK, WM, WN, LM>;
     __shared__ __attribute__((aligned(16))) double smem[Cfg::LDS_DOUBLES];
@@ -93,6 +93,7 @@
     int k, b;
     if (!decode_block_xcd(T * (T + 1) / 2, K + K1, k, b)) return;
     const bool second = k >= K;
+    if (inst) k = inst[k];
     const int kk = second ? k - K : k;
     int I = 0;
     while (b >= T - I) { b -= T - I; ++I; }
@@ -271,12 +272,13 @@
 template <int BM, int BK, int WM, int WN, bool LM>
 static void launch_cfg(hipStream_t st, const double* A, const double* B, double* C, double* C2, const double* E,
                        const double* coef, int K, int p, const double* A1 = nullptr, const double* B1 = nullptr,
-                       double* C1 = nullptr, int K1 = 0, double* maxdev = nullptr, const double* E2 = nullptr)
+                       double* C1 = nullptr, int K1 = 0, double* maxdev = nullptr, const double* E2 = nullptr,
+                       const int* inst = nullptr)
 {
     using Cfg = SymCfg<BM, BK, WM, WN, LM>;
     const int T = (p + BM - 1) / BM;
     hipLaunchKernelGGL((k_symm_tn<BM, BK, WM, WN, LM>), dim3(xcd_grid(T * (T + 1) / 2, K + K1)), dim3(Cfg::NT), 0, st, A,
-                       B, C, C2, E, coef, K, p, A1, B1, C1, K1, maxdev, E2);
+                       B, C, C2, E, coef, K, p, A1, B1, C1, K1, maxdev, E2, inst);
 }
 
 typedef __attribute__((address_space(1))) const void* gptr_t;
@@ -823,7 +825,7 @@
                                                  int p, const double* __restrict__ A1, const double* __restrict__ B1,
                                                  double* __restrict__ C1, int K1, double* __restrict__ maxdev,
                                                  double* __restrict__ rowpart, double* __restrict__ fropart, const CwRider rider,
-                                                 const CopySegs cps, const RedRider red)
+                                                 const CopySegs cps, const RedRider red, const int* __restrict__ inst)
 {
     __shared__ __attribute__((aligned(16))) double smem[NSTG * 2 * BK * BM];
     const int T = (p + BM - 1) / BM;
@@ -863,7 +865,9 @@
     }
     int k, b;
     if (!decode_block_xcd(T * (T + 1) / 2, K + K1, k, b, bid)) return;
-    symm_dl_tile<BK, NSTG, ABL, BM, NW>(A, B, C, C2, E, E2, coef, K, p, A1, B1, C1, K1, maxdev, rowpart, fropart, k, b, smem);
+    if (inst) k = inst[k];
+    symm_dl_tile<BK, NSTG, ABL, BM, NW>(A, B, C, C2, E, E2, coef, inst ? 0x7fffffff : K, p, A1, B1, C1, K1, maxdev, rowpart,
+                                        fropart, k, b, smem);
 }
 
 #ifdef GGL_DEV
@@ -1391,7 +1395,7 @@
 static void launch_dl(hipStream_t st, const double* A, const double* B, double* C, double* C2, const double* E,
                       const double* coef, int K, int p, const double* A1, const double* B1, double* C1, int K1,
                       double* maxdev, int dl_cfg = 0, double* rowpart = nullptr, double* fropart = nullptr,
-                      const double* E2 = nullptr)
+                      const double* E2 = nullptr, const int* inst = nullptr)
 {
     const bool eight = dl_cfg == 6 || dl_cfg == 7;
     const CwRider rider = (g_rider.K > 0 && !eight) ? g_rider : CwRider{};
@@ -1403,7 +1407,7 @@
     int ncopy = red.nblk > 0 ? NXCD : 0;
     for (int i = 0; i < cps.n; ++i) ncopy += (int)((cps.words[i] + 1023u) / 1024u);
     const int nride = rider.K * rider.nbx + ncopy;
-#define GGL_DL(...) hipLaunchKernelGGL((k_symm_dl<__VA_ARGS__>), grid, dim3(256), 0, st, A, B, C, C2, E, E2, coef, K, p, A1, B1, C1, K1, maxdev, rowpart, fropart, rider, cps, red)
+#define GGL_DL(...) hipLaunchKernelGGL((k_symm_dl<__VA_ARGS__>), grid, dim3(256), 0, st, A, B, C, C2, E, E2, coef, K, p, A1, B1, C1, K1, maxdev, rowpart, fropart, rider, cps, red, inst)
     if (dl_cfg == 4 || (dl_cfg >= 8 && dl_cfg <= 13) || (dl_cfg >= 18 && dl_cfg <= 21)) {
         const int T32 = (p + 31) / 32;
         const dim3 grid(xcd_grid(T32 * (T32 + 1) / 2, K + K1) + nride);
@@ -1426,7 +1430,7 @@
     const dim3 grid(xcd_grid(T * (T + 1) / 2, K + K1) + nride);
 #ifdef GGL_DEV
     if (dl_cfg == 6 || dl_cfg == 7) {
-#define GGL_DL8(...) hipLaunchKernelGGL((k_symm_dl<__VA_ARGS__>), grid, dim3(512), 0, st, A, B, C, C2, E, E2, coef, K, p, A1, B1, C1, K1, maxdev, rowpart, fropart, rider, cps, red)
+#define GGL_DL8(...) hipLaunchKernelGGL((k_symm_dl<__VA_ARGS__>), grid, dim3(512), 0, st, A, B, C, C2, E, E2, coef, K, p, A1, B1, C1, K1, maxdev, rowpart, fropart, rider, cps, red, inst)
         if (dl_cfg == 6) GGL_DL8(16, 4, 0, 64, 8);
         else GGL_DL8(32, 3, 0, 64, 8);
 #undef GGL_DL8
@@ -1788,14 +1792,14 @@
 
 void launch_symm(hipStream_t st, const double* A, const double* B, double* C, double* C2, const double* E,
                  const double* coef, int K, int p, int variant, double* maxdev, double* rowpart, double* fropart,
-                 const double* E2)
+                 const double* E2, const int* inst)
 {
     SymmHookAtExit hook{st, 0};
     if (variant < 0) variant = symm_auto_variant(K, p);
 #define GGL_TN(BM, BK, WM, WN, LM) \
-    launch_cfg<BM, BK, WM, WN, LM>(st, A, B, C, C2, E, coef, K, p, nullptr, nullptr, nullptr, 0, maxdev, E2)
-#ifdef GGL_DEV
-    if (E2 && variant >= 41 && variant <= 50) variant = 20;
+    launch_cfg<BM, BK, WM, WN, LM>(st, A, B, C, C2, E, coef, K, p, nullptr, nullptr, nullptr, 0, maxdev, E2, inst)
+#ifdef GGL_DEV
+    if ((E2 || inst) && variant >= 41 && variant <= 50) variant = 20;
     if (variant >= 41 && variant <= 50) {
         if ((p & 1) == 0 && p >= 2) { launch_sk(st, A, B, C, C2, E, coef, K, p, maxdev, rowpart, fropart, variant); return; }
         variant = 9;
@@ -1804,7 +1808,7 @@
     switch (variant) {
         case 16: case 17: case 18: case 19: case 20: case 21: case 22: case 23: case 24: case 25: case 26: case 27: case 28: case 29: case 30: case 31: case 32: case 33: case 34: case 35: case 36: case 37: case 38: case 39:
             if (symm_dl_serves(p)) {
-                launch_dl(st, A, B, C, C2, E, coef, K, p, nullptr, nullptr, nullptr, 0, maxdev, variant - 16, rowpart, fropart, E2);
+                launch_dl(st, A, B, C, C2, E, coef, K, p, nullptr, nullptr, nullptr, 0, maxdev, variant - 16, rowpart, fropart, E2, inst);
                 break;
             }
             if (variant == 20 || variant >= 24) GGL_TN(32, 32, 16, 16, true);
@@ -1825,7 +1829,7 @@
             const int T = (p + 63) / 64;
             const dim3 grid(xcd_grid(T * (T + 1) / 2, K));
             double* md = (variant == 10) ? maxdev : nullptr;
-#define GGL_ABL(N) hipLaunchKernelGGL((k_symm_tn<64, 16, 32, 32, true, N>), grid, dim3(256), 0, st, A, B, C, C2, E, coef, K, p, nullptr, nullptr, nullptr, 0, md, E2)
+#define GGL_ABL(N) hipLaunchKernelGGL((k_symm_tn<64, 16, 32, 32, true, N>), grid, dim3(256), 0, st, A, B, C, C2, E, coef, K, p, nullptr, nullptr, nullptr, 0, md, E2, inst)
             if (variant == 6) GGL_ABL(1); else if (variant == 7) GGL_ABL(2); else if (variant == 10) GGL_ABL(3);
             else if (variant == 14) GGL_ABL(4); else GGL_ABL(5);
 #undef GGL_ABL
diff --git a/gglasso_amd/csrc/kernels.hpp b/gglasso_amd/csrc/kernels.hpp
--- a/gglasso_amd/csrc/kernels.hpp
+++ b/gglasso_amd/csrc/kernels.hpp
@@ -196,7 +196,7 @@
 int symm_auto_variant(int nprod, int p);
 void launch_symm(hipStream_t st, const double* A, const double* B, double* C, double* C2, const double* E,
                  const double* coef, int K, int p, int variant, double* maxdev = nullptr, double* rowpart = nullptr,
-                 double* fropart = nullptr, const double* E2 = nullptr);
+                 double* fropart = nullptr, const double* E2 = nullptr, const int* inst = nullptr);
 int symm_bounds_tile(int K, int p, int variant);
 void symm_release_workspace(hipStream_t st);
 
@@ -275,7 +275,7 @@
 static constexpr double NS_SYM_KAPPA_MAX = 300.0;
 static constexpr double NS_KAPPA_LIMIT = 1e12;
 struct NsPlan {
-    int steps = 0; int products = 0; bool stable = false; double kappa = 0.0; int units = 0; int direct = 0;
+    int steps = 0; int products = 0; bool stable = false; double kappa = 0.0; int units = 0; int direct = 0; int n_short = 0;
     double check = 5e-5;
     unsigned char deg[NS_RANK_MAX_STEPS] = {};
 };
@@ -283,7 +283,7 @@
 void launch_form_W_sym(hipStream_t st, double* W, const double* Theta, const double* L, const double* X,
                        const double* S, const double* betaK, int K, int p);
 int ns_plan(const double* cbound_h, const double* beta_h, int K, double* coef_h, double* start_h, NsPlan* plan,
-            int force_mode, int degrees = 9, double tol = NS_TOL_EXACT, int poly = 0);
+            int force_mode, int degrees = 9, double tol = NS_TOL_EXACT, int poly = 0, int inst_sched = 0);
 int ns_poly_query(double l, int degrees, double tol, int* deg, double* coef, int* units, double* a_out, double* err_out);
 int ns_schedule_query(double l, int degrees, int max_steps, int* deg, double* coef, int* units, double tol = NS_TOL_EXACT);
 int ns_units_query(double l, int degrees, double tol);
diff --git a/gglasso_amd/csrc/newton_schulz.hip b/gglasso_amd/csrc/newton_schulz.hip
--- a/gglasso_amd/csrc/newton_schulz.hip
+++ b/gglasso_amd/csrc/newton_schulz.hip
@@ -599,7 +599,7 @@
 }
 
 int ns_plan(const double* cbound_h, const double* beta_h, int K, double* coef_h, double* start_h, NsPlan* plan,
-            int force_mode, int degrees, double tol, int poly)
+            int force_mode, int degrees, double tol, int poly, int inst_sched)
 {
     std::vector<double> c(K);
     double kappa = 1.0;
@@ -615,43 +615,78 @@
     plan->stable = stable;
     plan->kappa = kappa;
     plan->direct = 0;
+    plan->n_short = 0;
     auto put = [&](int g, int k, double cI, double cAcc, double cE, double dI = 0.0, double dC = 0.0, double dE = 0.0,
                    double cE2 = 0.0, double dE2 = 0.0) {
         double* o = coef_h + (size_t)g * NS_SLOT(K) + (size_t)k * NS_NCOEF;
         o[0] = cI; o[1] = cAcc; o[2] = cE; o[3] = dI; o[4] = dC; o[5] = dE; o[6] = cE2; o[7] = dE2;
     };
+    auto direct_rows = [&](int k, const NsPoly& pp, int Jk, int J) {
+        const double a = pp.a, m = 0.5 * (1.0 + a), h = 0.5 * (1.0 - a), u = 1.0 / (h * h * h);
+        const double ck = c[k], hc = 0.5 * std::sqrt(ck);
+        auto digit = [&](int j, double* o3) {
+            const double a0 = pp.co[3 * j], a1 = pp.co[3 * j + 1], a2 = pp.co[3 * j + 2];
+            o3[0] = a0 - a1 * (m / h) + a2 * (m / h) * (m / h);
+            o3[1] = a1 / (ck * h) - 2.0 * a2 * m / (ck * h * h);
+            o3[2] = a2 / (ck * ck * h * h);
+        };
+        double dg[3];
+        digit(0, dg);
+        double* s = start_h + (size_t)k * 5;
+        s[0] = hc * dg[1]; s[1] = hc * dg[2]; s[2] = hc * dg[0]; s[3] = 0.0; s[4] = 0.0;
+        digit(Jk - 1, dg);
+        put(0, k, -m * m * m * u, u / (ck * ck * ck), -3.0 * m * u / (ck * ck), dg[0], pp.co[3 * Jk], dg[2],
+            3.0 * m * m * u / ck, dg[1]);
+        for (int j = J - 2; j >= 1; --j) {
+            if (j > Jk - 2) { put(J - 1 - j, k, 0.0, 0.0, 0.0); continue; }
+            digit(j, dg);
+            put(J - 1 - j, k, dg[0], 1.0, dg[2], 0.0, 0.0, 0.0, dg[1]);
+        }
+        put(J - 1, k, 0.0, hc, 1.0);
+    };
+    if (inst_sched && !stable && poly && K > 1) {
+        int useq = 1 << 30;
+        if (inst_sched >= 2 && kappa <= NS_SYM_KAPPA_MAX) {
+            const int pds = ns_poly_choice(lmin, degrees, tol);
+            const NsSeq& sq = ns_mixed_schedule(lmin, degrees, tol);
+            useq = pds ? pds / 3 + 2 : ((sq.n < 1 || sq.n > NS_MAX_STEPS || sq.cost >= (1 << 29)) ? (1 << 30) : 2 + sq.cost);
+        }
+        std::vector<int> pdk(K);
+        int dlo = 1 << 30, dhi = 0;
+        for (int k = 0; k < K; ++k) {
+            const double lk = 1.0 / std::sqrt(c[k] / (4.0 * beta_h[k]));
+            pdk[k] = inst_sched >= 2 ? (kappa <= NS_SYM_KAPPA_MAX ? ns_poly_plan(lk, tol).deg : 0) : ns_poly_choice(lk, degrees, tol);
+            dlo = std::min(dlo, pdk[k]);
+            dhi = std::max(dhi, pdk[k]);
+        }
+        if (dlo > 0 && dhi == dlo + 3 && (inst_sched < 2 || dhi / 3 + 2 <= useq)) {
+            const int J = dhi / 3;
+            int* lst = reinterpret_cast<int*>(coef_h + (size_t)K * NS_NCOEF);
+            int nl = 0, nsh = 0;
+            for (int k = 0; k < K; ++k) nl += pdk[k] == dhi ? 1 : 0;
+            for (int k = 0, il = 0; k < K; ++k) {
+                direct_rows(k, ns_poly_plan(1.0 / std::sqrt(c[k] / (4.0 * beta_h[k])), tol, pdk[k]), pdk[k] / 3, J);
+                if (pdk[k] == dhi) lst[il++] = k; else lst[nl + nsh++] = k;
+            }
+            plan->direct = dhi;
+            plan->n_short = nsh;
+            plan->steps = 1;
+            plan->deg[0] = 0;
+            plan->units = J + 2;
+            plan->products = J + 2;
+            return 0;
+        }
+    }
     const int pd = (!stable && poly) ? ns_poly_choice(lmin, degrees, tol) : 0;
     if (pd) {
         const NsPoly pp = ns_poly_plan(lmin, tol, pd);
         const int J = pd / 3;
-        const double a = pp.a, m = 0.5 * (1.0 + a), h = 0.5 * (1.0 - a), u = 1.0 / (h * h * h);
         plan->direct = pd;
         plan->steps = 1;
         plan->deg[0] = 0;
         plan->units = pp.units;
         plan->products = J + 2;
-        for (int k = 0; k < K; ++k) {
-            const double ck = c[k], hc = 0.5 * std::sqrt(ck);
-            auto digit = [&](int j, double* o3) {
-                const double a0 = pp.co[3 * j], a1 = pp.co[3 * j + 1], a2 = pp.co[3 * j + 2];
-                o3[0] = a0 - a1 * (m / h) + a2 * (m / h) * (m / h);
-                o3[1] = a1 / (ck * h) - 2.0 * a2 * m / (ck * h * h);
-                o3[2] = a2 / (ck * ck * h * h);
-            };
-            double dg[3];
-            digit(0, dg);
-            double* s = start_h + (size_t)k * 5;
-            s[0] = hc * dg[1]; s[1] = hc * dg[2]; s[2] = hc * dg[0]; s[3] = 0.0; s[4] = 0.0;
-            int g = 0;
-            digit(J - 1, dg);
-            put(g++, k, -m * m * m * u, u / (ck * ck * ck), -3.0 * m * u / (ck * ck), dg[0], pp.co[3 * J], dg[2],
-                3.0 * m * m * u / ck, dg[1]);
-            for (int j = J - 2; j >= 1; --j) {
-                digit(j, dg);
-                put(g++, k, dg[0], 1.0, dg[2], 0.0, 0.0, 0.0, dg[1]);
-            }
-            put(g++, k, 0.0, hc, 1.0);
-        }
+        for (int k = 0; k < K; ++k) direct_rows(k, pp, J, J);
         return 0;
     }
     if (!stable) {
@@ -779,6 +814,21 @@
         if (!fused_start) launch_ns_start(st, Tb, nullptr, AB, AB + n1, W, start_d, K, p, 4);
         const int J = plan.direct / 3;
         auto hbuf = [&](int j) { return (j & 1) ? YP + n1 : out; };
+        if (plan.n_short) {
+            const int nl = K - plan.n_short;
+            const int* lst = reinterpret_cast<const int*>(coef_d + (size_t)K * NS_NCOEF);
+            if (variant < 0) variant = symm_auto_variant(K, p);
+            launch_symm(st, AB, AB + n1, YP, hbuf(J - 1), AB + n1, coef_d, nl, p, variant, nullptr, nullptr, nullptr, AB, lst);
+            launch_symm(st, AB, AB + n1, YP, hbuf(J - 2), AB + n1, coef_d, plan.n_short, p, variant, nullptr, nullptr, nullptr, AB,
+                        lst + nl);
+            launch_symm(st, hbuf(J - 1), YP, hbuf(J - 2), nullptr, AB + n1, coef_d + cs, nl, p, variant, nullptr, nullptr, nullptr,
+                        AB, lst);
+            for (int j = J - 3; j >= 1; --j)
+                launch_symm(st, hbuf(j + 1), YP, hbuf(j), nullptr, AB + n1, coef_d + cs * (J - 1 - j), K, p, variant, nullptr,
+                            nullptr, nullptr, AB);
+            launch_symm(st, hbuf(1), YP, out, nullptr, Tb, coef_d + cs * (J - 1), K, p, variant);
+            return;
+        }
         launch_symm(st, AB, AB + n1, YP, hbuf(J - 1), AB + n1, coef_d + cs * g++, K, p, variant, nullptr, nullptr, nullptr, AB);
         for (int j = J - 2; j >= 1; --j)
             launch_symm(st, hbuf(j + 1), YP, hbuf(j), nullptr, AB + n1, coef_d + cs * g++, K, p, variant, nullptr, nullptr,
diff --git a/gglasso_amd/solver.py b/gglasso_amd/solver.py
--- a/gglasso_amd/solver.py
+++ b/gglasso_amd/solver.py
@@ -427,6 +427,12 @@
         out = (ctypes.c_longlong * 3)()
         check(self.lib.ggl_omega_poly_stats(self.h, out))
         return dict(zip(("seqs", "seqs_total", "last_deg"), (int(v) for v in out)))
+
+    def inst_stats(self):
+        import ctypes
+        out = (ctypes.c_longlong * 3)()
+        check(self.lib.ggl_inst_sched_stats(self.h, out))
+        return dict(zip(("seqs", "skipped", "products"), (int(v) for v in out)))
 
     def rank_stats(self):
         import ctypes
diff --git a/include/ggl_hip.h b/include/ggl_hip.h
--- a/include/ggl_hip.h
+++ b/include/ggl_hip.h
@@ -84,6 +84,7 @@
 #define GGL_OPT_DOWNLOAD_THREADS 36
 #define GGL_OPT_GROUP_SCHED 37
 #define GGL_OPT_OMEGA_POLY 38
+#define GGL_OPT_INST_SCHED 39
 #define GGL_OPT_PART_PRIORITY 25
 #define GGL_OPT_ISOLATE 19
 #define GGL_OPT_RANK_L0_COARSE 18
@@ -203,6 +204,7 @@
 int ggl_lds_stats(ggl_ctx *ctx, long long out[4]);
 int ggl_group_stats(ggl_ctx *ctx, long long out[11], double *units_sum);
 int ggl_omega_poly_stats(ggl_ctx *ctx, long long out[3]);
+int ggl_inst_sched_stats(ggl_ctx *ctx, long long out[3]);
 int ggl_spectral_bounds(ggl_ctx *ctx, double *c_out, double *beta_out);
 int ggl_pipeline_stats(ggl_ctx *ctx, long long out[10]);
 int ggl_rank_stats(ggl_ctx *ctx, long long out[4]);
@@ -227,6 +229,10 @@
 int ggl_dev_group_partition(const int *units, int K, int p, int max_groups, int *len_out);
 int ggl_dev_ns_units(double l, int degrees, double tol);
 int ggl_dev_omega_poly_plan(double a, double tol, int degrees, int *deg, double *out, int *units);
+int ggl_dev_symm_inst(int K, int p, const double *A, const double *B, const double *E, const double *E2, const double *coef8K,
+                      const int *inst, int nact, int variant, double *C, double *C2, double *rowpart, double *fropart);
+int ggl_dev_inst_plan(int K, const double *cbound, const double *beta, double tol, int degrees, int poly, int inst_sched,
+                      int *units_out, int *list_out, int *info_out);
 #ifdef GGL_DEV
 int ggl_dev_i8_stages(int n);
 int ggl_dev_symm_i8(int K, int p, int S, int dmax, const double *A, const double *B, double scaleA, double scaleB, double *C,
```

After: 1473. About the same (-0.2%).
